# levi106/kvedge

Measured on AMD Instinct MI355X. Metric: images/sec ResNet-50 edge module at 1/2/4/8 MI355X; VM boot-to-ready sec, higher is better.
Workload: dtype bf16; 1 GPU; model=resnet50, global_batch=1280, per_gpu_batch=1280, image_size=224, parallelism=dp1, backend=none, hip_graph=True, streams=2, microbatch=0, mb_blocks=3

## Files before the change

### csrc/bindings/ops.cpp

```cpp
#include <ATen/ATen.h>
#include <c10/core/DeviceGuard.h>
#include <c10/hip/HIPStream.h>
#include <torch/library.h>

#include "../kernels/kvedge_kernels.h"

namespace {

hipStream_t cur_stream(const at::Tensor& t) {
  return c10::hip::getCurrentHIPStream(t.device().index()).stream();
}

void check_dev(const at::Tensor& t, const char* name) {
  TORCH_CHECK(t.is_cuda(), "kvedge: ", name, " must be a GPU tensor");
  TORCH_CHECK(t.is_contiguous(), "kvedge: ", name, " must be contiguous");
}

void check_bf16(const at::Tensor& t, const char* name) {
  check_dev(t, name);
  TORCH_CHECK(t.scalar_type() == at::kBFloat16, "kvedge: ", name, " must be bf16");
}

void set_splitk_ws(KvConvParams& p, const at::Tensor& ws) {
  p.ws = ws.data_ptr<float>();
  p.ws_elems = ws.numel();
}

void conv(const at::Tensor& x, const at::Tensor& w, const c10::optional<at::Tensor>& bias,
          const c10::optional<at::Tensor>& res, at::Tensor& y, int64_t N, int64_t H, int64_t W,
          int64_t Cin, int64_t ldx, int64_t x_coff, int64_t Ho, int64_t Wo, int64_t Cout,
          int64_t KH, int64_t KW, int64_t stride, int64_t pad, int64_t K, int64_t ldy,
          int64_t y_coff, int64_t ldr, int64_t r_coff, int64_t act, int64_t mode,
          int64_t tile, const c10::optional<at::Tensor>& ws) {
  check_bf16(x, "x");
  check_bf16(w, "w");
  check_bf16(y, "y");
  const c10::DeviceGuard g(x.device());
  KvConvParams p{};
  if (ws.has_value() && ws->defined()) {
    check_dev(*ws, "ws");
    TORCH_CHECK(ws->scalar_type() == at::kFloat, "kvedge: split-K workspace fp32");
    set_splitk_ws(p, *ws);
  }
  p.x = x.data_ptr();
  p.w = w.data_ptr();
  p.bias = nullptr;
  if (bias.has_value() && bias->defined()) {
    check_dev(*bias, "bias");
    TORCH_CHECK(bias->scalar_type() == at::kFloat && bias->numel() >= Cout, "kvedge: bias fp32[Cout]");
    p.bias = bias->data_ptr<float>();
  }
  p.res = nullptr;
  if (res.has_value() && res->defined()) {
    check_bf16(*res, "res");
    p.res = res->data_ptr();
  }
  p.y = y.data_ptr();
  p.N = (int)N; p.H = (int)H; p.W = (int)W; p.Cin = (int)Cin;
  p.ldx = (int)ldx; p.x_coff = (int)x_coff;
  p.Ho = (int)Ho; p.Wo = (int)Wo; p.Cout = (int)Cout;
  p.KH = (int)KH; p.KW = (int)KW; p.stride = (int)stride; p.pad = (int)pad;
  p.K = (int)K;
  TORCH_CHECK(w.dim() == 2 && w.size(0) == Cout, "kvedge: packed weight must be [Cout, Kpad]");
  p.Kpad = (int)w.size(1);
  p.M = (int)(N * Ho * Wo);
  p.ldy = (int)ldy; p.y_coff = (int)y_coff; p.ldr = (int)ldr; p.r_coff = (int)r_coff;
  p.act = (int)act; p.mode = (int)mode;
  TORCH_CHECK(N > 0 && H * W * ldx * 2 < (1ll << 31) && Ho * Wo * ldy * 2 < (1ll << 31),
              "kvedge: one image's activations exceed 2 GiB");
  TORCH_CHECK(x.numel() >= N * H * W * ldx, "kvedge: x smaller than N*H*W*ldx");
  TORCH_CHECK(x_coff >= 0 && x_coff + Cin <= ldx, "kvedge: x channel slice out of range");
  TORCH_CHECK(y.numel() >= (int64_t)p.M * ldy && y_coff + Cout <= ldy, "kvedge: y too small");
  if (p.res) TORCH_CHECK(res->numel() >= (int64_t)p.M * ldr && r_coff + Cout <= ldr, "kvedge: residual too small");
  const int rc = kv_conv2d(&p, (int)tile, cur_stream(x));
  TORCH_CHECK(rc == 0, "kvedge: kv_conv2d failed rc=", rc);
}

void conv_pair(const at::Tensor& x, const at::Tensor& w, const at::Tensor& bias,
               const at::Tensor& w2, const at::Tensor& b2, at::Tensor& z, int64_t Cin,
               int64_t x_coff, int64_t z_coff, int64_t act, int64_t tile) {
  check_bf16(x, "x");
  check_bf16(w, "w");
  check_bf16(w2, "w2");
  check_bf16(z, "z");
  check_dev(bias, "bias");
  check_dev(b2, "b2");
  TORCH_CHECK(x.dim() == 4 && z.dim() == 4 && w.dim() == 2 && w2.dim() == 2, "kvedge: conv_pair shapes");
  const int64_t N = x.size(0), H = x.size(1), W = x.size(2), ldx = x.size(3);
  const int64_t Cout = w.size(0), C2 = w2.size(0);
  TORCH_CHECK(w2.size(1) == Cout, "kvedge: conv_pair w2 must be [C2, Cout]");
  TORCH_CHECK(z.size(0) == N && z.size(1) == H && z.size(2) == W && z_coff + C2 <= z.size(3),
              "kvedge: conv_pair z [N, H, W, >= z_coff + C2]");
  TORCH_CHECK(x_coff + Cin <= ldx && w.size(1) == (9 * Cin + 63) / 64 * 64, "kvedge: conv_pair x / w");
  TORCH_CHECK(x_coff >= 0 && z_coff >= 0, "kvedge: conv_pair channel offsets must be >= 0");
  TORCH_CHECK(z_coff % 4 == 0 && z.size(3) % 4 == 0,
              "kvedge: conv_pair z_coff and the z row pitch must be multiples of 4 channels");
  TORCH_CHECK(bias.scalar_type() == at::kFloat && bias.numel() >= Cout && b2.scalar_type() == at::kFloat &&
              b2.numel() >= C2, "kvedge: conv_pair biases fp32");
  TORCH_CHECK(N * H * W * ldx * 2 < (1ll << 31) && N * H * W * z.size(3) * 2 < (1ll << 31),
              "kvedge: conv_pair operands exceed 2 GiB");
  const c10::DeviceGuard g(x.device());
  KvConvParams p{};
  p.x = x.data_ptr();
  p.w = w.data_ptr();
  p.bias = bias.data_ptr<float>();
  p.N = (int)N; p.H = (int)H; p.W = (int)W; p.Cin = (int)Cin;
  p.ldx = (int)ldx; p.x_coff = (int)x_coff;
  p.Ho = (int)H; p.Wo = (int)W; p.Cout = (int)Cout;
  p.KH = 3; p.KW = 3; p.stride = 1; p.pad = 1;
  p.K = (int)(9 * Cin); p.Kpad = (int)w.size(1);
  p.M = (int)(N * H * W);
  p.act = (int)act; p.mode = 0;
  p.w_t = w2.data_ptr(); p.bias_t = b2.data_ptr<float>(); p.z = z.data_ptr();
  p.n_t = (int)C2; p.ldz = (int)z.size(3); p.z_coff = (int)z_coff;
  p.pair_1x1 = 1;
  const int rc = kv_conv_pair(&p, (int)tile, cur_stream(x));
  TORCH_CHECK(rc == 0, "kvedge: conv_pair failed rc=", rc);
}

void conv_dual(const at::Tensor& x1, const at::Tensor& x2, const at::Tensor& w,
               const c10::optional<at::Tensor>& bias, at::Tensor& y, int64_t stride2,
               int64_t act, int64_t tile, const c10::optional<at::Tensor>& ws) {
  check_bf16(x1, "x1");
  check_bf16(x2, "x2");
  check_bf16(w, "w");
  check_bf16(y, "y");
  TORCH_CHECK(x1.dim() == 4 && x2.dim() == 4 && y.dim() == 4, "kvedge: NHWC tensors");
  const int64_t N = x1.size(0), Ho = x1.size(1), Wo = x1.size(2), K1 = x1.size(3);
  const int64_t K2 = x2.size(3), Cout = y.size(3);
  TORCH_CHECK(x2.size(0) == N && (x2.size(1) + stride2 - 1) / stride2 == Ho &&
                  (x2.size(2) + stride2 - 1) / stride2 == Wo, "kvedge: x2 geometry vs stride");
  TORCH_CHECK(y.size(0) == N && y.size(1) == Ho && y.size(2) == Wo, "kvedge: y shape");
  TORCH_CHECK(w.dim() == 2 && w.size(0) == Cout && w.size(1) == K1 + K2, "kvedge: w [Cout, K1+K2]");
  TORCH_CHECK(K1 % 64 == 0 && K2 % 64 == 0, "kvedge: K1, K2 multiples of 64");
  const c10::DeviceGuard g(x1.device());
  KvConvParams p{};
  p.x = x1.data_ptr();
  p.w = w.data_ptr();
  p.bias = nullptr;
  if (bias.has_value() && bias->defined()) {
    check_dev(*bias, "bias");
    TORCH_CHECK(bias->scalar_type() == at::kFloat && bias->numel() >= Cout, "kvedge: bias fp32[Cout]");
    p.bias = bias->data_ptr<float>();
  }
  p.res = nullptr;
  p.y = y.data_ptr();
  p.N = (int)N; p.H = (int)Ho; p.W = (int)Wo; p.Cin = (int)K1; p.ldx = (int)K1; p.x_coff = 0;
  p.Ho = (int)Ho; p.Wo = (int)Wo; p.Cout = (int)Cout;
  p.KH = 1; p.KW = 1; p.stride = 1; p.pad = 0;
  p.K = (int)(K1 + K2); p.Kpad = (int)(K1 + K2);
  p.M = (int)(N * Ho * Wo);
  p.ldy = (int)Cout; p.y_coff = 0; p.ldr = 0; p.r_coff = 0;
  p.act = (int)act; p.mode = 4;
  p.x2 = x2.data_ptr(); p.K1 = (int)K1; p.H2 = (int)x2.size(1); p.W2 = (int)x2.size(2);
  p.ldx2 = (int)K2; p.stride2 = (int)stride2;
  if (ws.has_value() && ws->defined()) {
    check_dev(*ws, "ws");
    TORCH_CHECK(ws->scalar_type() == at::kFloat, "kvedge: split-K workspace fp32");
    set_splitk_ws(p, *ws);
  }
  const int rc = kv_conv2d(&p, (int)tile, cur_stream(x1));
  TORCH_CHECK(rc == 0, "kvedge: conv_dual failed rc=", rc);
}

void conv_dual2(const at::Tensor& x, int64_t x_coff, int64_t K1, const at::Tensor& x2,
                int64_t x2_coff, const at::Tensor& w, const c10::optional<at::Tensor>& bias,
                at::Tensor& y, int64_t y_coff, int64_t stride2, int64_t up2, int64_t act,
                int64_t tile, const c10::optional<at::Tensor>& ws) {
  check_bf16(x, "x");
  check_bf16(x2, "x2");
  check_bf16(w, "w");
  check_bf16(y, "y");
  TORCH_CHECK(x.dim() == 4 && x2.dim() == 4 && y.dim() == 4 && w.dim() == 2, "kvedge: NHWC tensors");
  const int64_t N = x.size(0), Ho = x.size(1), Wo = x.size(2);
  const int64_t Cout = w.size(0), K2 = w.size(1) - K1;
  TORCH_CHECK(K1 > 0 && K2 > 0 && K1 % 64 == 0 && K2 % 64 == 0, "kvedge: K1, K2 multiples of 64");
  TORCH_CHECK(x_coff >= 0 && x_coff % 8 == 0 && x_coff + K1 <= x.size(3), "kvedge: x slice");
  TORCH_CHECK(x2_coff >= 0 && x2_coff % 8 == 0 && x2_coff + K2 <= x2.size(3), "kvedge: x2 slice");
  TORCH_CHECK(y_coff >= 0 && y_coff % 8 == 0 && y_coff + Cout <= y.size(3), "kvedge: y slice");
  TORCH_CHECK(x.size(3) % 8 == 0 && x2.size(3) % 8 == 0 && y.size(3) % 8 == 0, "kvedge: pitches");
  TORCH_CHECK(y.size(0) == N && y.size(1) == Ho && y.size(2) == Wo && x2.size(0) == N, "kvedge: y shape");
  if (up2) {
    TORCH_CHECK(x2.size(1) * 2 == Ho && x2.size(2) * 2 == Wo, "kvedge: up2 needs x2 at half size");
  } else {
    TORCH_CHECK(stride2 >= 1 && (x2.size(1) + stride2 - 1) / stride2 == Ho &&
                    (x2.size(2) + stride2 - 1) / stride2 == Wo,
                "kvedge: x2 geometry vs stride");
  }
  const c10::DeviceGuard g(x.device());
  KvConvParams p{};
  p.x = x.data_ptr();
  p.w = w.data_ptr();
  p.bias = nullptr;
  if (bias.has_value() && bias->defined()) {
    check_dev(*bias, "bias");
    TORCH_CHECK(bias->scalar_type() == at::kFloat && bias->numel() >= Cout, "kvedge: bias fp32[Cout]");
    p.bias = bias->data_ptr<float>();
  }
  p.y = y.data_ptr();
  p.N = (int)N; p.H = (int)Ho; p.W = (int)Wo; p.Cin = (int)K1; p.ldx = (int)x.size(3);
  p.x_coff = (int)x_coff;
  p.Ho = (int)Ho; p.Wo = (int)Wo; p.Cout = (int)Cout;
  p.KH = 1; p.KW = 1; p.stride = 1; p.pad = 0;
  p.K = (int)(K1 + K2); p.Kpad = (int)(K1 + K2);
  p.M = (int)(N * Ho * Wo);
  p.ldy = (int)y.size(3); p.y_coff = (int)y_coff; p.ldr = 0; p.r_coff = 0;
  p.act = (int)act; p.mode = 4;
  p.x2 = x2.data_ptr(); p.K1 = (int)K1; p.H2 = (int)x2.size(1); p.W2 = (int)x2.size(2);
  p.ldx2 = (int)x2.size(3); p.stride2 = (int)stride2; p.x2_coff = (int)x2_coff; p.up2 = (int)up2;
  if (ws.has_value() && ws->defined()) {
    check_dev(*ws, "ws");
    TORCH_CHECK(ws->scalar_type() == at::kFloat, "kvedge: split-K workspace fp32");
    set_splitk_ws(p, *ws);
  }
  const int rc = kv_conv2d(&p, (int)tile, cur_stream(x));
  TORCH_CHECK(rc == 0, "kvedge: conv_dual2 failed rc=", rc);
}

void conv_tail(const at::Tensor& x, const c10::optional<at::Tensor>& x2, const at::Tensor& w,
               const c10::optional<at::Tensor>& bias, const c10::optional<at::Tensor>& res,
               at::Tensor& y, const at::Tensor& w1, const c10::optional<at::Tensor>& b1,
               at::Tensor& z, int64_t stride2, int64_t act, int64_t tile) {
  check_bf16(x, "x");
  check_bf16(w, "w");
  check_bf16(y, "y");
  check_bf16(w1, "w1");
  check_bf16(z, "z");
  TORCH_CHECK(x.dim() == 4 && y.dim() == 4 && z.dim() == 4, "kvedge: NHWC tensors");
  const int64_t N = x.size(0), H = x.size(1), W = x.size(2), K1 = x.size(3);
  const int64_t Cout = y.size(3), Nt = w1.size(0);
  TORCH_CHECK(y.size(0) == N && y.size(1) == H && y.size(2) == W, "kvedge: y shape");
  TORCH_CHECK(z.size(0) == N && z.size(1) == H && z.size(2) == W && z.size(3) == Nt,
              "kvedge: z shape");
  TORCH_CHECK(w1.dim() == 2 && w1.size(1) == Cout, "kvedge: w1 must be [n_t, Cout]");
  TORCH_CHECK(K1 % 64 == 0, "kvedge: conv_tail K1 multiple of 64");
  const c10::DeviceGuard g(x.device());
  KvConvParams p{};
  p.x = x.data_ptr();
  p.w = w.data_ptr();
  p.bias = nullptr;
  if (bias.has_value() && bias->defined()) {
    check_dev(*bias, "bias");
    TORCH_CHECK(bias->scalar_type() == at::kFloat && bias->numel() >= Cout, "kvedge: bias fp32[Cout]");
    p.bias = bias->data_ptr<float>();
  }
  p.y = y.data_ptr();
  p.N = (int)N; p.H = (int)H; p.W = (int)W; p.Cin = (int)K1; p.ldx = (int)K1; p.x_coff = 0;
  p.Ho = (int)H; p.Wo = (int)W; p.Cout = (int)Cout;
  p.KH = 1; p.KW = 1; p.stride = 1; p.pad = 0;
  p.M = (int)(N * H * W);
  p.ldy = (int)Cout; p.y_coff = 0; p.r_coff = 0;
  p.act = (int)act;
  if (x2.has_value() && x2->defined()) {
    check_bf16(*x2, "x2");
    TORCH_CHECK(!(res.has_value() && res->defined()), "kvedge: conv_tail dual form takes no res");
    const int64_t K2 = x2->size(3);
    TORCH_CHECK(x2->dim() == 4 && x2->size(0) == N && (x2->size(1) + stride2 - 1) / stride2 == H &&
                    (x2->size(2) + stride2 - 1) / stride2 == W && K2 % 64 == 0,
                "kvedge: x2 geometry vs stride");
    TORCH_CHECK(w.dim() == 2 && w.size(0) == Cout && w.size(1) == K1 + K2, "kvedge: w [Cout, K1+K2]");
    p.mode = 4; p.K = (int)(K1 + K2); p.Kpad = (int)(K1 + K2);
    p.x2 = x2->data_ptr(); p.K1 = (int)K1; p.H2 = (int)x2->size(1); p.W2 = (int)x2->size(2);
    p.ldx2 = (int)K2; p.stride2 = (int)stride2;
    p.res = nullptr; p.ldr = 0;
  } else {
    TORCH_CHECK(res.has_value() && res->defined(), "kvedge: conv_tail plain form needs res");
    check_bf16(*res, "res");
    TORCH_CHECK(res->sizes() == y.sizes(), "kvedge: res shape");
    TORCH_CHECK(w.dim() == 2 && w.size(0) == Cout && w.size(1) == K1, "kvedge: w [Cout, K1]");
    p.mode = 1; p.K = (int)K1; p.Kpad = (int)K1;
    p.res = res->data_ptr(); p.ldr = (int)Cout;
  }
  p.w_t = w1.data_ptr();
  p.bias_t = nullptr;
  if (b1.has_value() && b1->defined()) {
    check_dev(*b1, "b1");
    TORCH_CHECK(b1->scalar_type() == at::kFloat && b1->numel() >= Nt, "kvedge: b1 fp32[n_t]");
    p.bias_t = b1->data_ptr<float>();
  }
  p.z = z.data_ptr(); p.n_t = (int)Nt; p.ldz = (int)Nt; p.z_coff = 0; p.act_t = 1;
  const int rc = kv_conv2d(&p, (int)tile, cur_stream(x));
  TORCH_CHECK(rc == 0, "kvedge: conv_tail failed rc=", rc);
}

void conv_frames_s2d(const at::Tensor& frames, const at::Tensor& w,
                     const c10::optional<at::Tensor>& bias, at::Tensor& y, int64_t act,
                     int64_t tile) {
  check_dev(frames, "frames");
  TORCH_CHECK(frames.scalar_type() == at::kByte && frames.dim() == 4 && frames.size(3) == 3 &&
                  frames.size(1) % 2 == 0 && frames.size(2) % 2 == 0,
              "kvedge: frames must be uint8 [N, H, W, 3] with even H, W");
  check_bf16(w, "w");
  check_bf16(y, "y");
  const int64_t N = frames.size(0), H = frames.size(1) / 2, W = frames.size(2) / 2;
  const int64_t Cout = w.size(0);
  TORCH_CHECK(w.dim() == 2 && w.size(1) == 64, "kvedge: s2d stem weight must be [Cout, 64]");
  TORCH_CHECK(y.dim() == 4 && y.size(0) == N && y.size(1) == H && y.size(2) == W &&
                  y.size(3) == Cout, "kvedge: y must be [N, H/2, W/2, Cout]");
  const c10::DeviceGuard g(frames.device());
  KvConvParams p{};
  p.x = frames.data_ptr();
  p.w = w.data_ptr();
  p.bias = nullptr;
  if (bias.has_value() && bias->defined()) {
    check_dev(*bias, "bias");
    TORCH_CHECK(bias->scalar_type() == at::kFloat && bias->numel() >= Cout, "kvedge: bias fp32[Cout]");
    p.bias = bias->data_ptr<float>();
  }
  p.res = nullptr;
  p.y = y.data_ptr();
  p.N = (int)N; p.H = (int)H; p.W = (int)W; p.Cin = 16; p.ldx = 16; p.x_coff = 0;
  p.Ho = (int)H; p.Wo = (int)W; p.Cout = (int)Cout;
  p.KH = 2; p.KW = 2; p.stride = 1; p.pad = 1; p.K = 64; p.Kpad = 64;
  p.M = (int)(N * H * W);
  p.ldy = (int)Cout; p.y_coff = 0; p.ldr = 0; p.r_coff = 0;
  p.act = (int)act; p.mode = 0; p.in_u8 = 1;
  const int rc = kv_conv2d(&p, (int)tile, cur_stream(frames));
  TORCH_CHECK(rc == 0, "kvedge: conv_frames_s2d failed rc=", rc);
}

void maxpool2d(const at::Tensor& x, at::Tensor& y, int64_t N, int64_t H, int64_t W, int64_t C,
               int64_t ldx, int64_t x_coff, int64_t ldy, int64_t y_coff, int64_t k, int64_t stride, int64_t pad,
               int64_t Ho, int64_t Wo) {
  check_bf16(x, "x");
  check_bf16(y, "y");
  TORCH_CHECK(x.numel() >= N * H * W * ldx && y.numel() >= N * Ho * Wo * ldy, "kvedge: maxpool sizes");
  const c10::DeviceGuard g(x.device());
  const int rc = kv_maxpool2d(x.data_ptr(), y.data_ptr(), (int)N, (int)H, (int)W, (int)C, (int)ldx,
                              (int)x_coff, (int)ldy, (int)y_coff, (int)k, (int)stride, (int)pad, (int)Ho,
                              (int)Wo, cur_stream(x));
  TORCH_CHECK(rc == 0, "kvedge: maxpool2d failed rc=", rc);
}

void stem_pool(const at::Tensor& x, const at::Tensor& w, const at::Tensor& bias, at::Tensor& y,
               int64_t y_coff) {
  check_bf16(x, "x");
  check_bf16(w, "w");
  check_bf16(y, "y");
  TORCH_CHECK(x.dim() == 4 && x.size(3) == 16, "kvedge: stem_pool x must be [N,H,W,16] (s2d)");
  TORCH_CHECK(w.numel() == 64 * 256, "kvedge: stem_pool w must be [64][256]");
  TORCH_CHECK(bias.is_cuda() && bias.scalar_type() == at::kFloat && bias.numel() == 64 &&
                  bias.is_contiguous(), "kvedge: stem_pool bias");
  const int64_t N = x.size(0), H = x.size(1), W = x.size(2);
  TORCH_CHECK(y.dim() == 4 && y.size(0) == N && y.size(1) == (H - 1) / 2 + 1 &&
                  y.size(2) == (W - 1) / 2 + 1 && y.size(3) >= y_coff + 64,
              "kvedge: stem_pool y shape");
  const c10::DeviceGuard g(x.device());
  const int rc = kv_stem_pool(x.data_ptr(), w.data_ptr(), bias.data_ptr<float>(), y.data_ptr(),
                              (int)N, (int)H, (int)W, (int)y.size(3), (int)y_coff, cur_stream(x));
  TORCH_CHECK(rc == 0, "kvedge: stem_pool failed rc=", rc);
}

void sppf_pool(at::Tensor& buf, int64_t N, int64_t H, int64_t W, int64_t C) {
  check_bf16(buf, "buf");
  TORCH_CHECK(buf.numel() == N * H * W * 4 * C, "kvedge: sppf buffer must be [N,H,W,4C]");
  const c10::DeviceGuard g(buf.device());
  const int rc = kv_sppf_pool(buf.data_ptr(), (int)N, (int)H, (int)W, (int)C, cur_stream(buf));
  TORCH_CHECK(rc == 0, "kvedge: sppf failed rc=", rc);
}

void global_avgpool(const at::Tensor& x, at::Tensor& y, int64_t N, int64_t HW, int64_t C) {
  check_bf16(x, "x");
  check_bf16(y, "y");
  TORCH_CHECK(x.numel() == N * HW * C && y.numel() == N * C, "kvedge: avgpool sizes");
  const c10::DeviceGuard g(x.device());
  const int rc = kv_global_avgpool(x.data_ptr(), y.data_ptr(), (int)N, (int)HW, (int)C, cur_stream(x));
  TORCH_CHECK(rc == 0, "kvedge: avgpool failed rc=", rc);
}

void pooled_fc(const at::Tensor& x, const at::Tensor& w, const c10::optional<at::Tensor>& bias,
               at::Tensor& y) {
  check_bf16(x, "x");
  check_bf16(w, "w");
  check_bf16(y, "y");
  TORCH_CHECK(x.dim() == 4 && w.dim() == 2 && y.dim() == 2, "kvedge: pooled_fc shapes");
  const int64_t N = x.size(0), HW = x.size(1) * x.size(2), C = x.size(3), ncls = w.size(0);
  TORCH_CHECK(w.size(1) >= C && y.size(0) == N && y.size(1) == ncls, "kvedge: pooled_fc w / y");
  const float* bp = nullptr;
  if (bias.has_value() && bias->defined()) {
    check_dev(*bias, "bias");
    TORCH_CHECK(bias->scalar_type() == at::kFloat && bias->numel() >= ncls, "kvedge: pooled_fc bias");
    bp = bias->data_ptr<float>();
  }
  const c10::DeviceGuard g(x.device());
  const int rc = kv_pooled_fc(x.data_ptr(), (int)N, (int)HW, (int)C, w.data_ptr(), (int)w.size(1),
                              bp, y.data_ptr(), (int)ncls, cur_stream(x));
  TORCH_CHECK(rc == 0, "kvedge: pooled_fc failed rc=", rc);
}

void softmax_rows(const at::Tensor& x, at::Tensor& y, at::Tensor& argmax) {
  check_bf16(x, "x");
  check_dev(y, "y");
  check_dev(argmax, "argmax");
  TORCH_CHECK(x.dim() == 2 && y.sizes() == x.sizes() && y.scalar_type() == at::kFloat, "kvedge: softmax y");
  TORCH_CHECK(argmax.scalar_type() == at::kLong && argmax.numel() == x.size(0), "kvedge: argmax");
  const c10::DeviceGuard g(x.device());
  const int rc = kv_softmax_rows(x.data_ptr(), y.data_ptr<float>(), argmax.data_ptr<int64_t>(),
                                 (int)x.size(0), (int)x.size(1), cur_stream(x));
  TORCH_CHECK(rc == 0, "kvedge: softmax failed rc=", rc);
}

void upsample2x(const at::Tensor& x, at::Tensor& y, int64_t N, int64_t H, int64_t W, int64_t C,
                int64_t ldx, int64_t x_coff, int64_t ldy, int64_t y_coff) {
  check_bf16(x, "x");
  check_bf16(y, "y");
  TORCH_CHECK(x.numel() >= N * H * W * ldx && y.numel() >= N * 4 * H * W * ldy, "kvedge: upsample sizes");
  const c10::DeviceGuard g(x.device());
  const int rc = kv_upsample2x(x.data_ptr(), y.data_ptr(), (int)N, (int)H, (int)W, (int)C, (int)ldx,
                               (int)x_coff, (int)ldy, (int)y_coff, cur_stream(x));
  TORCH_CHECK(rc == 0, "kvedge: upsample2x failed rc=", rc);
}

void yolo_decode(const at::Tensor& f0, const at::Tensor& f1, const at::Tensor& f2, int64_t h0,
                 int64_t w0, int64_t h1, int64_t w1, int64_t h2, int64_t w2, int64_t s0,
                 int64_t s1, int64_t s2, int64_t nc, at::Tensor& boxes, at::Tensor& scores,
                 at::Tensor& cls) {
  check_bf16(f0, "f0");
  check_bf16(f1, "f1");
  check_bf16(f2, "f2");
  const int64_t N = f0.size(0);
  const int64_t A = h0 * w0 + h1 * w1 + h2 * w2;
  const int64_t ch = 64 + nc;
  TORCH_CHECK(f0.numel() == N * h0 * w0 * ch && f1.numel() == N * h1 * w1 * ch &&
                  f2.numel() == N * h2 * w2 * ch, "kvedge: decode feature sizes");
  TORCH_CHECK(boxes.numel() == N * A * 4 && boxes.scalar_type() == at::kFloat, "kvedge: boxes");
  TORCH_CHECK(scores.numel() == N * A && scores.scalar_type() == at::kFloat, "kvedge: scores");
  TORCH_CHECK(cls.numel() == N * A && cls.scalar_type() == at::kInt, "kvedge: cls");
  const c10::DeviceGuard g(f0.device());
  const int rc = kv_yolo_decode(f0.data_ptr(), f1.data_ptr(), f2.data_ptr(), (int)h0, (int)w0,
                                (int)h1, (int)w1, (int)h2, (int)w2, (int)s0, (int)s1, (int)s2,
                                (int)N, (int)nc, boxes.data_ptr<float>(), scores.data_ptr<float>(),
                                cls.data_ptr<int>(), cur_stream(f0));
  TORCH_CHECK(rc == 0, "kvedge: yolo_decode failed rc=", rc);
}

void nms(const at::Tensor& boxes, const at::Tensor& scores, const at::Tensor& cls, double conf,
         double iou, int64_t max_det, at::Tensor& out, at::Tensor& count) {
  check_dev(boxes, "boxes");
  check_dev(scores, "scores");
  check_dev(cls, "cls");
  TORCH_CHECK(scores.dim() == 2, "kvedge: scores [N, A]");
  const int64_t N = scores.size(0), A = scores.size(1);
  TORCH_CHECK(boxes.numel() == N * A * 4 && cls.numel() == N * A, "kvedge: nms inputs");
  TORCH_CHECK(out.numel() == N * max_det * 6 && out.scalar_type() == at::kFloat, "kvedge: nms out");
  TORCH_CHECK(count.numel() == N && count.scalar_type() == at::kInt, "kvedge: nms count");
  const c10::DeviceGuard g(scores.device());
  const int rc = kv_nms(boxes.data_ptr<float>(), scores.data_ptr<float>(), cls.data_ptr<int>(),
                        (int)N, (int)A, (float)conf, (float)iou, (int)max_det,
                        out.data_ptr<float>(), count.data_ptr<int>(), cur_stream(scores));
  TORCH_CHECK(rc == 0, "kvedge: nms failed rc=", rc);
}

void synth_frames(at::Tensor& y, int64_t seed, int64_t step) {
  check_dev(y, "y");
  TORCH_CHECK(y.scalar_type() == at::kByte && y.dim() == 4 && y.size(3) == 3, "kvedge: frames u8 [N,H,W,3]");
  const c10::DeviceGuard g(y.device());
  const int rc = kv_synth_frames(y.data_ptr<uint8_t>(), (int)y.size(0), (int)y.size(1),
                                 (int)y.size(2), (uint64_t)seed, (uint64_t)step, cur_stream(y));
  TORCH_CHECK(rc == 0, "kvedge: synth_frames failed rc=", rc);
}

void synth_frames_dev(at::Tensor& y, at::Tensor& step, int64_t seed) {
  check_dev(y, "y");
  check_dev(step, "step");
  TORCH_CHECK(y.scalar_type() == at::kByte && y.dim() == 4 && y.size(3) == 3, "kvedge: frames u8 [N,H,W,3]");
  TORCH_CHECK(step.scalar_type() == at::kLong && (step.numel() == 1 || step.numel() == 2),
              "kvedge: step int64[1] or int64[2]");
  const c10::DeviceGuard g(y.device());
  const int rc = kv_synth_frames_dev(y.data_ptr<uint8_t>(), (int)y.size(0), (int)y.size(1),
                                     (int)y.size(2), (uint64_t)seed,
                                     reinterpret_cast<uint64_t*>(step.data_ptr<int64_t>()),
                                     step.numel() == 2 ? 1 : 0, cur_stream(y));
  TORCH_CHECK(rc == 0, "kvedge: synth_frames_dev failed rc=", rc);
}

void stem12_pool_frames(const at::Tensor& x, const at::Tensor& w, const at::Tensor& bias,
                        at::Tensor& y, at::ArrayRef<double> mean, at::ArrayRef<double> stdv,
                        int64_t y_coff) {
  check_dev(x, "x");
  check_bf16(w, "w");
  check_bf16(y, "y");
  TORCH_CHECK(x.scalar_type() == at::kByte && x.dim() == 4 && x.size(3) == 3 && x.is_contiguous(),
              "kvedge: stem12_pool_frames x must be contiguous u8 [N,H,W,3]");
  TORCH_CHECK(x.size(1) % 2 == 0 && x.size(2) % 4 == 0, "kvedge: stem12_pool_frames H even, W % 4");
  TORCH_CHECK(w.numel() == 64 * 192 && w.is_contiguous(), "kvedge: stem12 w must be [64][192]");
  TORCH_CHECK(bias.is_cuda() && bias.scalar_type() == at::kFloat && bias.numel() == 64 &&
                  bias.is_contiguous(), "kvedge: stem12 bias");
  TORCH_CHECK(mean.size() == 3 && stdv.size() == 3, "kvedge: mean/std of 3");
  const int64_t N = x.size(0), H = x.size(1) / 2, W = x.size(2) / 2;
  TORCH_CHECK(y.dim() == 4 && y.size(0) == N && y.size(1) == (H - 1) / 2 + 1 &&
                  y.size(2) == (W - 1) / 2 + 1 && y.size(3) >= y_coff + 64 && y.is_contiguous(),
              "kvedge: stem12_pool_frames y shape");
  float m[3], is[3];
  for (int i = 0; i < 3; ++i) {
    m[i] = (float)mean[i];
    is[i] = (float)(1.0 / stdv[i]);
  }
  const c10::DeviceGuard g(x.device());
  const int rc = kv_stem12_pool_frames(x.data_ptr(), w.data_ptr(), bias.data_ptr<float>(),
                                       y.data_ptr(), (int)N, (int)x.size(1), (int)x.size(2), m, is,
                                       (int)y.size(3), (int)y_coff, cur_stream(x));
  TORCH_CHECK(rc == 0, "kvedge: stem12_pool_frames failed rc=", rc);
}

void yolo_stem2(const at::Tensor& x, const at::Tensor& w0, const at::Tensor& b0,
                const at::Tensor& w1, const at::Tensor& b1, at::Tensor& y) {
  check_dev(x, "x");
  check_bf16(w0, "w0");
  check_bf16(w1, "w1");
  check_bf16(y, "y");
  TORCH_CHECK(x.scalar_type() == at::kByte && x.dim() == 4 && x.size(3) == 3 && x.is_contiguous(),
              "kvedge: yolo_stem2 x must be contiguous u8 [N,H,W,3]");
  TORCH_CHECK(x.size(1) % 4 == 0 && x.size(2) % 32 == 0 && x.size(2) <= 640,
              "kvedge: yolo_stem2 needs H % 4 == 0, W % 32 == 0, W <= 640");
  TORCH_CHECK(w0.dim() == 2 && w0.size(0) == 16 && w0.size(1) == 64 && w0.is_contiguous(),
              "kvedge: yolo_stem2 w0 must be [16][64]");
  TORCH_CHECK(w1.dim() == 2 && w1.size(0) == 32 && w1.size(1) >= 144 && w1.size(1) % 8 == 0 &&
                  w1.is_contiguous(), "kvedge: yolo_stem2 w1 must be [32][>= 144]");
  for (const at::Tensor* b : {&b0, &b1}) {
    check_dev(*b, "bias");
    TORCH_CHECK(b->scalar_type() == at::kFloat && b->is_contiguous(), "kvedge: fp32 biases");
  }
  TORCH_CHECK(b0.numel() >= 16 && b1.numel() >= 32, "kvedge: bias sizes");
  const int64_t N = x.size(0), H0 = x.size(1), W0 = x.size(2);
  TORCH_CHECK(y.dim() == 4 && y.size(0) == N && y.size(1) == H0 / 4 && y.size(2) == W0 / 4 &&
                  y.size(3) == 32 && y.is_contiguous(), "kvedge: yolo_stem2 y must be [N,H/4,W/4,32]");
  const c10::DeviceGuard g(x.device());
  const int rc = kv_yolo_stem2(x.data_ptr(), w0.data_ptr(), b0.data_ptr<float>(), w1.data_ptr(),
                               (int)w1.size(1), b1.data_ptr<float>(), y.data_ptr(), (int)N,
                               (int)H0, (int)W0, cur_stream(x));
  TORCH_CHECK(rc == 0, "kvedge: yolo_stem2 failed rc=", rc);
}

void stem_pool_frames(const at::Tensor& x, const at::Tensor& w, const at::Tensor& bias,
                      at::Tensor& y, at::ArrayRef<double> mean, at::ArrayRef<double> stdv,
                      int64_t y_coff) {
  check_dev(x, "x");
  check_bf16(w, "w");
  check_bf16(y, "y");
  TORCH_CHECK(x.scalar_type() == at::kByte && x.dim() == 4 && x.size(3) == 3 && x.is_contiguous(),
              "kvedge: stem_pool_frames x must be contiguous u8 [N,H,W,3]");
  TORCH_CHECK(x.size(1) % 2 == 0 && x.size(2) % 4 == 0, "kvedge: stem_pool_frames H even, W % 4");
  TORCH_CHECK(w.numel() == 64 * 256, "kvedge: stem_pool w must be [64][256]");
  TORCH_CHECK(bias.is_cuda() && bias.scalar_type() == at::kFloat && bias.numel() == 64 &&
                  bias.is_contiguous(), "kvedge: stem_pool bias");
  TORCH_CHECK(mean.size() == 3 && stdv.size() == 3, "kvedge: mean/std of 3");
  const int64_t N = x.size(0), H = x.size(1) / 2, W = x.size(2) / 2;
  TORCH_CHECK(y.dim() == 4 && y.size(0) == N && y.size(1) == (H - 1) / 2 + 1 &&
                  y.size(2) == (W - 1) / 2 + 1 && y.size(3) >= y_coff + 64,
              "kvedge: stem_pool_frames y shape");
  float m[3], is[3];
  for (int i = 0; i < 3; ++i) {
    m[i] = (float)mean[i];
    is[i] = (float)(1.0 / stdv[i]);
  }
  const c10::DeviceGuard g(x.device());
  const int rc = kv_stem_pool_frames(x.data_ptr(), w.data_ptr(), bias.data_ptr<float>(),
                                     y.data_ptr(), (int)N, (int)x.size(1), (int)x.size(2), m, is,
                                     (int)y.size(3), (int)y_coff, cur_stream(x));
  TORCH_CHECK(rc == 0, "kvedge: stem_pool_frames failed rc=", rc);
}

void preprocess(const at::Tensor& x, at::Tensor& y, at::ArrayRef<double> mean,
                at::ArrayRef<double> stdv) {
  check_dev(x, "x");
  check_bf16(y, "y");
  TORCH_CHECK(x.scalar_type() == at::kByte && x.dim() == 4 && x.size(3) == 3, "kvedge: x u8 [N,H,W,3]");
  TORCH_CHECK(y.dim() == 4 && y.size(0) == x.size(0), "kvedge: y batch");
  const bool s2d = y.size(3) == 16;
  if (s2d) {
    TORCH_CHECK(y.size(1) * 2 == x.size(1) && y.size(2) * 2 == x.size(2), "kvedge: y bf16 [N,H/2,W/2,16]");
  } else {
    TORCH_CHECK(y.size(1) == x.size(1) && y.size(2) == x.size(2) && y.size(3) == 4,
                "kvedge: y bf16 [N,H,W,4] or [N,H/2,W/2,16]");
  }
  TORCH_CHECK(mean.size() == 3 && stdv.size() == 3, "kvedge: mean/std of 3");
  float m[3], is[3];
  for (int i = 0; i < 3; ++i) {
    m[i] = (float)mean[i];
    is[i] = (float)(1.0 / stdv[i]);
  }
  const c10::DeviceGuard g(x.device());
  const int rc = s2d ? kv_preprocess_s2d(x.data_ptr<uint8_t>(), y.data_ptr(), (int)x.size(0),
                                         (int)x.size(1), (int)x.size(2), m, is, cur_stream(x))
                     : kv_preprocess(x.data_ptr<uint8_t>(), y.data_ptr(), (int)x.size(0),
                                     (int)x.size(1), (int)x.size(2), m, is, cur_stream(x));
  TORCH_CHECK(rc == 0, "kvedge: preprocess failed rc=", rc);
}

void frame_resize(const at::Tensor& src, at::Tensor& dst, at::IntArrayRef axis_y,
                  at::IntArrayRef axis_x, int64_t pad) {
  check_dev(src, "src");
  check_dev(dst, "dst");
  TORCH_CHECK(src.scalar_type() == at::kByte && src.dim() == 4 && src.size(3) == 3,
              "kvedge: src u8 [N,Hs,Ws,3]");
  TORCH_CHECK(dst.scalar_type() == at::kByte && dst.dim() == 4 && dst.size(3) == 3 &&
                  dst.size(0) == src.size(0), "kvedge: dst u8 [N,Hd,Wd,3]");
  TORCH_CHECK(axis_y.size() == 5 && axis_x.size() == 5, "kvedge: axis_y / axis_x of 5 ints");
  TORCH_CHECK(src.size(1) <= 8192 && src.size(2) <= 8192 && dst.size(1) <= 8192 &&
                  dst.size(2) <= 8192, "kvedge: frame_resize extents are 1..8192");
  TORCH_CHECK(src.device() == dst.device(), "kvedge: src / dst on different devices");
  int ay[5], ax[5];
  for (int i = 0; i < 5; ++i) {
    TORCH_CHECK(axis_y[i] >= 0 && axis_y[i] <= 8192 && axis_x[i] >= 0 && axis_x[i] <= 8192,
                "kvedge: frame_resize axis values are 0..8192");
    ay[i] = (int)axis_y[i];
    ax[i] = (int)axis_x[i];
  }
  const c10::DeviceGuard g(src.device());
  const int rc = kv_frame_resize(src.data_ptr<uint8_t>(), dst.data_ptr<uint8_t>(), (int)src.size(0),
                                 (int)src.size(1), (int)src.size(2), (int)dst.size(1),
                                 (int)dst.size(2), ay, ax, (int)pad, cur_stream(src));
  TORCH_CHECK(rc == 0, "kvedge: frame_resize failed rc=", rc);
}

void det_to_source(at::Tensor& det, const at::Tensor& count, at::ArrayRef<double> map, int64_t Hs,
                   int64_t Ws) {
  check_dev(det, "det");
  check_dev(count, "count");
  TORCH_CHECK(det.scalar_type() == at::kFloat && det.dim() == 3 && det.size(2) == 6,
              "kvedge: det fp32 [N,max_det,6]");
  TORCH_CHECK(count.scalar_type() == at::kInt && count.numel() == det.size(0),
              "kvedge: count int32 [N]");
  TORCH_CHECK(map.size() == 4, "kvedge: map = {cy, sy, cx, sx}");
  TORCH_CHECK(Hs >= 1 && Ws >= 1 && Hs <= 8192 && Ws <= 8192, "kvedge: source size 1..8192");
  TORCH_CHECK(det.device() == count.device(), "kvedge: det / count on different devices");
  const c10::DeviceGuard g(det.device());
  const int rc = kv_det_to_source(det.data_ptr<float>(), count.data_ptr<int>(), (int)det.size(0),
                                  (int)det.size(1), (float)map[0], (float)map[1], (float)map[2],
                                  (float)map[3], (int)Hs, (int)Ws, cur_stream(det));
  TORCH_CHECK(rc == 0, "kvedge: det_to_source failed rc=", rc);
}

void roi_crop_band(const at::Tensor& src, const at::Tensor& det, const at::Tensor& count,
                   at::Tensor& dst, int64_t pad, int64_t band) {
  check_dev(src, "src");
  check_dev(det, "det");
  check_dev(count, "count");
  check_dev(dst, "dst");
  TORCH_CHECK(src.scalar_type() == at::kByte && src.dim() == 4 && src.size(3) == 3,
              "kvedge: src u8 [N,Hs,Ws,3]");
  TORCH_CHECK(det.scalar_type() == at::kFloat && det.dim() == 3 && det.size(2) == 6 &&
                  det.size(0) == src.size(0), "kvedge: det fp32 [N,max_det,6]");
  TORCH_CHECK(count.scalar_type() == at::kInt && count.dim() == 1 &&
                  count.size(0) == src.size(0), "kvedge: count int32 [N]");
  TORCH_CHECK(dst.scalar_type() == at::kByte && dst.dim() == 4 && dst.size(3) == 3 &&
                  dst.size(1) == dst.size(2), "kvedge: dst u8 [N*K,D,D,3]");
  const int64_t N = src.size(0);
  TORCH_CHECK(N ? dst.size(0) >= N && dst.size(0) % N == 0 : dst.size(0) == 0,
              "kvedge: dst holds N*K crops, K >= 1");
  const int64_t K = N ? dst.size(0) / N : 1;
  TORCH_CHECK(K <= det.size(1), "kvedge: roi_crop K ", K, " > max_det ", det.size(1));
  TORCH_CHECK(src.size(1) <= 8192 && src.size(2) <= 8192 && dst.size(1) <= 8192,
              "kvedge: roi_crop extents are 1..8192");
  TORCH_CHECK(N * det.size(1) < (1ll << 31) && dst.size(0) < (1ll << 31),
              "kvedge: roi_crop batch too large");
  TORCH_CHECK(src.device() == det.device() && src.device() == count.device() &&
                  src.device() == dst.device(), "kvedge: roi_crop operands on different devices");
  TORCH_CHECK(band >= 0 && band <= 32, "kvedge: roi_crop band is 0, 4, 8, 16 or 32");
  const c10::DeviceGuard g(src.device());
  const int rc = kv_roi_crop_band(src.data_ptr<uint8_t>(), det.data_ptr<float>(),
                                  count.data_ptr<int>(), dst.data_ptr<uint8_t>(), (int)N,
                                  (int)src.size(1), (int)src.size(2), (int)det.size(1), (int)K,
                                  (int)dst.size(1), (int)pad, (int)band, cur_stream(src));
  TORCH_CHECK(rc == 0, "kvedge: roi_crop failed rc=", rc);
}

void roi_crop(const at::Tensor& src, const at::Tensor& det, const at::Tensor& count,
              at::Tensor& dst, int64_t pad) {
  roi_crop_band(src, det, count, dst, pad, 0);
}

void batchnorm_nhwc(const at::Tensor& x, at::Tensor& y, const at::Tensor& scale,
                    const at::Tensor& shift, bool relu) {
  check_bf16(x, "x");
  check_bf16(y, "y");
  check_dev(scale, "scale");
  check_dev(shift, "shift");
  const int64_t C = x.size(-1);
  TORCH_CHECK(scale.numel() == C && shift.numel() == C && scale.scalar_type() == at::kFloat &&
                  shift.scalar_type() == at::kFloat, "kvedge: bn scale/shift fp32[C]");
  TORCH_CHECK(y.sizes() == x.sizes(), "kvedge: bn y shape");
  const c10::DeviceGuard g(x.device());
  const int rc = kv_batchnorm_nhwc(x.data_ptr(), y.data_ptr(), scale.data_ptr<float>(),
                                   shift.data_ptr<float>(), x.numel() / C, (int)C, relu ? 1 : 0,
                                   cur_stream(x));
  TORCH_CHECK(rc == 0, "kvedge: batchnorm failed rc=", rc);
}

int64_t conv_num_tiles() { return kv_conv_num_tiles(); }
int64_t conv_splitk_base() { return kv_conv_splitk_base(); }
int64_t conv_splitk_num_tiles() { return kv_conv_splitk_num_tiles(); }
int64_t nloop_sched_check() { return kv_nloop_sched_check(); }
int64_t conv_seam_num_tiles() { return kv_conv_seam_num_tiles(); }
int64_t set_conv_chunk_bytes(int64_t b) { return kv_set_conv_chunk_bytes(b); }

void c2f16_fused(const at::Tensor& x, int64_t x_coff, const at::Tensor& w1, const at::Tensor& b1,
                 const at::Tensor& wm1, const at::Tensor& bm1, const at::Tensor& wm2,
                 const at::Tensor& bm2, const at::Tensor& w2, const at::Tensor& b2, at::Tensor& y,
                 int64_t y_coff, int64_t S) {
  check_bf16(x, "x");
  check_bf16(y, "y");
  for (const at::Tensor* w : {&w1, &wm1, &wm2, &w2}) check_bf16(*w, "w");
  for (const at::Tensor* b : {&b1, &bm1, &bm2, &b2}) {
    check_dev(*b, "bias");
    TORCH_CHECK(b->scalar_type() == at::kFloat && b->is_contiguous(), "kvedge: c2f16 biases fp32");
  }
  TORCH_CHECK(x.dim() == 4 && y.dim() == 4 && x.size(0) == y.size(0) && x.size(1) == y.size(1) &&
                  x.size(2) == y.size(2), "kvedge: c2f16 x / y [N, H, W, C]");
  const int64_t N = x.size(0), H = x.size(1), W = x.size(2);
  TORCH_CHECK(x_coff >= 0 && x_coff + 32 <= x.size(3) && y_coff >= 0 && y_coff + 32 <= y.size(3),
              "kvedge: c2f16 channel slices");
  TORCH_CHECK(w1.dim() == 2 && w1.size(0) == 32 && w1.size(1) >= 32 && wm1.dim() == 2 &&
                  wm1.size(0) == 16 && wm1.size(1) >= 144 && wm2.sizes() == wm1.sizes() &&
                  w2.dim() == 2 && w2.size(0) == 32 && w2.size(1) >= 48,
              "kvedge: c2f16 weights w1 [32, >=32], wm [16, >=144], w2 [32, >=48]");
  TORCH_CHECK(b1.numel() == 32 && bm1.numel() == 16 && bm2.numel() == 16 && b2.numel() == 32,
              "kvedge: c2f16 bias sizes");
  TORCH_CHECK(kv_c2f16_supported((int)H, (int)W, (int)S), "kvedge: c2f16 has no form for H=", H,
              " W=", W, " S=", S);
  TORCH_CHECK(x.numel() * 2 < (1ll << 31) - (1 << 20) && y.numel() * 2 < (1ll << 31) - (1 << 20),
              "kvedge: c2f16 operands exceed 2 GiB");
  TORCH_CHECK(x.data_ptr() != y.data_ptr(), "kvedge: c2f16 cannot run in place");
  const c10::DeviceGuard g(x.device());
  KvC2fParams p{};
  p.x = x.data_ptr();
  p.y = y.data_ptr();
  p.w1 = w1.data_ptr();
  p.b1 = b1.data_ptr<float>();
  p.wm1 = wm1.data_ptr();
  p.bm1 = bm1.data_ptr<float>();
  p.wm2 = wm2.data_ptr();
  p.bm2 = bm2.data_ptr<float>();
  p.w2 = w2.data_ptr();
  p.b2 = b2.data_ptr<float>();
  p.N = (int)N; p.H = (int)H; p.W = (int)W;
  p.ldx = (int)x.size(3); p.x_coff = (int)x_coff;
  p.ldy = (int)y.size(3); p.y_coff = (int)y_coff;
  p.ldw1 = (int)w1.size(1); p.ldwm = (int)wm1.size(1); p.ldw2 = (int)w2.size(1);
  p.S = (int)S;
  const int rc = kv_c2f16_fused(&p, cur_stream(x));
  TORCH_CHECK(rc == 0, "kvedge: c2f16_fused failed rc=", rc);
}

int64_t c2f16_supported(int64_t H, int64_t W, int64_t S) {
  return kv_c2f16_supported((int)H, (int)W, (int)S);
}

}

TORCH_LIBRARY(kvedge, m) {
  m.def("conv(Tensor x, Tensor w, Tensor? bias, Tensor? res, Tensor(a!) y, int N, int H, int W, "
        "int Cin, int ldx, int x_coff, int Ho, int Wo, int Cout, int KH, int KW, int stride, "
        "int pad, int K, int ldy, int y_coff, int ldr, int r_coff, int act, int mode, int tile, "
        "Tensor(b!)? ws=None) -> ()");
  m.def("conv_pair(Tensor x, Tensor w, Tensor bias, Tensor w2, Tensor b2, Tensor(a!) z, int Cin, "
        "int x_coff, int z_coff, int act, int tile) -> ()");
  m.def("conv_dual(Tensor x1, Tensor x2, Tensor w, Tensor? bias, Tensor(a!) y, int stride2, int act, "
        "int tile, Tensor(b!)? ws=None) -> ()");
  m.def("conv_tail(Tensor x, Tensor? x2, Tensor w, Tensor? bias, Tensor? res, Tensor(a!) y, "
        "Tensor w1, Tensor? b1, Tensor(b!) z, int stride2, int act, int tile) -> ()");
  m.def("conv_frames_s2d(Tensor frames, Tensor w, Tensor? bias, Tensor(a!) y, int act, "
        "int tile) -> ()");
  m.def("stem_pool(Tensor x, Tensor w, Tensor bias, Tensor(a!) y, int y_coff) -> ()");
  m.def("maxpool2d(Tensor x, Tensor(a!) y, int N, int H, int W, int C, int ldx, int x_coff, int ldy, "
        "int y_coff, int k, int stride, int pad, int Ho, int Wo) -> ()");
  m.def("sppf_pool(Tensor(a!) buf, int N, int H, int W, int C) -> ()");
  m.def("global_avgpool(Tensor x, Tensor(a!) y, int N, int HW, int C) -> ()");
  m.def("softmax_rows(Tensor x, Tensor(a!) y, Tensor(b!) argmax) -> ()");
  m.def("pooled_fc(Tensor x, Tensor w, Tensor? bias, Tensor(a!) y) -> ()");
  m.def("upsample2x(Tensor x, Tensor(a!) y, int N, int H, int W, int C, int ldx, int x_coff, int ldy, "
        "int y_coff) -> ()");
  m.def("yolo_decode(Tensor f0, Tensor f1, Tensor f2, int h0, int w0, int h1, int w1, int h2, "
        "int w2, int s0, int s1, int s2, int nc, Tensor(a!) boxes, Tensor(b!) scores, "
        "Tensor(c!) cls) -> ()");
  m.def("nms(Tensor boxes, Tensor scores, Tensor cls, float conf, float iou, int max_det, "
        "Tensor(a!) out, Tensor(b!) count) -> ()");
  m.def("synth_frames(Tensor(a!) y, int seed, int step) -> ()");
  m.def("synth_frames_dev(Tensor(a!) y, Tensor(b!) step, int seed) -> ()");
  m.def("stem_pool_frames(Tensor x, Tensor w, Tensor bias, Tensor(a!) y, float[] mean, float[] std, int y_coff) -> ()");
  m.def("stem12_pool_frames(Tensor x, Tensor w, Tensor bias, Tensor(a!) y, float[] mean, float[] std, int y_coff) -> ()");
  m.def("yolo_stem2(Tensor x, Tensor w0, Tensor b0, Tensor w1, Tensor b1, Tensor(a!) y) -> ()");
  m.def("preprocess(Tensor x, Tensor(a!) y, float[] mean, float[] std) -> ()");
  m.def("frame_resize(Tensor src, Tensor(a!) dst, int[] axis_y, int[] axis_x, int pad) -> ()");
  m.def("det_to_source(Tensor(a!) det, Tensor count, float[] map, int Hs, int Ws) -> ()");
  m.def("roi_crop(Tensor src, Tensor det, Tensor count, Tensor(a!) dst, int pad) -> ()");
  m.def("roi_crop_band(Tensor src, Tensor det, Tensor count, Tensor(a!) dst, int pad, int band) -> ()");
  m.def("batchnorm_nhwc(Tensor x, Tensor(a!) y, Tensor scale, Tensor shift, bool relu) -> ()");
  m.def("conv_num_tiles() -> int", conv_num_tiles);
  m.def("conv_splitk_base() -> int", conv_splitk_base);
  m.def("conv_splitk_num_tiles() -> int", conv_splitk_num_tiles);
  m.def("nloop_sched_check() -> int", nloop_sched_check);
  m.def("conv_seam_num_tiles() -> int", conv_seam_num_tiles);
  m.def("c2f16_fused(Tensor x, int x_coff, Tensor w1, Tensor b1, Tensor wm1, Tensor bm1, "
        "Tensor wm2, Tensor bm2, Tensor w2, Tensor b2, Tensor(a!) y, int y_coff, int S) -> ()");
  m.def("c2f16_supported(int H, int W, int S) -> int", c2f16_supported);
  m.def("conv_dual2(Tensor x, int x_coff, int K1, Tensor x2, int x2_coff, Tensor w, Tensor? bias, "
        "Tensor(a!) y, int y_coff, int stride2, int up2, int act, int tile, Tensor(b!)? ws=None) -> ()");
  m.def("set_conv_chunk_bytes(int bytes) -> int", set_conv_chunk_bytes);
}

TORCH_LIBRARY_IMPL(kvedge, CUDA, m) {
  m.impl("conv", conv);
  m.impl("conv_dual", conv_dual);
  m.impl("maxpool2d", maxpool2d);
  m.impl("stem_pool", stem_pool);
  m.impl("conv_frames_s2d", conv_frames_s2d);
  m.impl("conv_tail", conv_tail);
  m.impl("conv_pair", conv_pair);
  m.impl("c2f16_fused", c2f16_fused);
  m.impl("conv_dual2", conv_dual2);
  m.impl("sppf_pool", sppf_pool);
  m.impl("global_avgpool", global_avgpool);
  m.impl("softmax_rows", softmax_rows);
  m.impl("pooled_fc", pooled_fc);
  m.impl("upsample2x", upsample2x);
  m.impl("yolo_decode", yolo_decode);
  m.impl("nms", nms);
  m.impl("synth_frames", synth_frames);
  m.impl("synth_frames_dev", synth_frames_dev);
  m.impl("preprocess", preprocess);
  m.impl("stem_pool_frames", stem_pool_frames);
  m.impl("stem12_pool_frames", stem12_pool_frames);
  m.impl("yolo_stem2", yolo_stem2);
  m.impl("frame_resize", frame_resize);
  m.impl("det_to_source", det_to_source);
  m.impl("roi_crop", roi_crop);
  m.impl("roi_crop_band", roi_crop_band);
  m.impl("batchnorm_nhwc", batchnorm_nhwc);
}
```

### csrc/kernels/conv_igemm.hip

```cpp
#include <algorithm>

#include "common.h"
#include "kvedge_kernels.h"

namespace kvedge {
namespace {

constexpr int BK = 64;

struct TileCfg {
  int bm, bn, wm, wn;
};

template <int BM, int BN, int WM, int WN, int MODE>
__global__ __launch_bounds__(256, 2) void conv_igemm_kernel(const KvConvParams p) {
  constexpr int WTM = BM / WM, WTN = BN / WN;
  constexpr int TM = WTM / 16, TN = WTN / 16;
  constexpr int AR = BM / 32;
  constexpr int BR = BN / 32;
  static_assert(WM * WN == 4, "4 waves per workgroup");
  static_assert(TM >= 1 && TN >= 1, "wave tile >= 16x16");

  __shared__ __attribute__((aligned(16))) bf16 smem[2 * (BM + BN) * BK];

  const int tid = threadIdx.x;
  const int lane = tid & 63;
  const int wv = tid >> 6;
  const int wm = wv / WN, wn = wv % WN;

  const int nbm = (p.M + BM - 1) / BM;
  const int nbn = (p.Cout + BN - 1) / BN;
  const int t = xcd_remap(blockIdx.x, nbm * nbn);
  const int m0 = (t / nbn) * BM;
  const int n0 = (t % nbn) * BN;
  static_assert(BN <= 256, "one bias value per thread");
  const float bias_r = (tid < BN && p.bias && n0 + tid < p.Cout) ? p.bias[n0 + tid] : 0.f;

  const bf16* __restrict__ X = reinterpret_cast<const bf16*>(p.x);
  const bf16* __restrict__ Wt = reinterpret_cast<const bf16*>(p.w);

  const int cc = tid & 7;
  const int rr = tid >> 3;

  int a_base[AR], a_h0[AR], a_w0[AR];
  const int HoWo = p.Ho * p.Wo;
#pragma unroll
  for (int i = 0; i < AR; ++i) {
    const int m = m0 + rr + 32 * i;
    if (m < p.M) {
      if (MODE == 1) {
        a_base[i] = m * p.ldx + p.x_coff;
        a_h0[i] = 0;
        a_w0[i] = 0;
      } else {
        const int img = m / HoWo;
        const int rem = m - img * HoWo;
        const int ho = rem / p.Wo;
        const int wo = rem - ho * p.Wo;
        a_base[i] = img * p.H * p.W * p.ldx + p.x_coff;
        a_h0[i] = ho * p.stride - p.pad;
        a_w0[i] = wo * p.stride - p.pad;
      }
    } else {
      a_base[i] = 0;
      a_h0[i] = -(1 << 28);
      a_w0[i] = -(1 << 28);
    }
  }

  int kr = 0, ksx = 0, kc = cc * 8;
  if (MODE == 0) {
    while (kc >= p.Cin) {
      kc -= p.Cin;
      if (++ksx == p.KW) { ksx = 0; ++kr; }
    }
  }
  const int kwp = (p.KW + 1) & ~1;
  const int kpr = kwp * 4;

  uint4 ra[AR], rb[BR];

  auto load_a = [&](int kt) {
#pragma unroll
    for (int i = 0; i < AR; ++i) {
      uint4 v = make_uint4(0, 0, 0, 0);
      if (MODE == 1) {
        const int k = kt * BK + cc * 8;
        if (a_h0[i] >= 0 && k < p.Cin)
          v = *reinterpret_cast<const uint4*>(X + a_base[i] + k);
      } else if (MODE == 0) {
        const int hi = a_h0[i] + kr, wi = a_w0[i] + ksx;
        if (kr < p.KH && (unsigned)hi < (unsigned)p.H && (unsigned)wi < (unsigned)p.W)
          v = *reinterpret_cast<const uint4*>(X + a_base[i] + (hi * p.W + wi) * p.ldx + kc);
      } else {
        const int k = kt * BK + cc * 8;
        const int r = k / kpr;
        const int s = ((k - r * kpr) >> 3) * 2;
        const int hi = a_h0[i] + r, wi = a_w0[i] + s;
        if (r < p.KH && (unsigned)hi < (unsigned)p.H) {
          const bf16* rowp = X + a_base[i] + hi * p.W * 4;
          uint2 lo = make_uint2(0, 0), hi2 = make_uint2(0, 0);
          if ((unsigned)wi < (unsigned)p.W) lo = *reinterpret_cast<const uint2*>(rowp + wi * 4);
          if ((unsigned)(wi + 1) < (unsigned)p.W)
            hi2 = *reinterpret_cast<const uint2*>(rowp + (wi + 1) * 4);
          v = make_uint4(lo.x, lo.y, hi2.x, hi2.y);
        }
      }
      ra[i] = v;
    }
  };
  auto advance_k = [&]() {
    if (MODE == 0) {
      kc += BK;
      while (kc >= p.Cin) {
        kc -= p.Cin;
        if (++ksx == p.KW) { ksx = 0; ++kr; }
      }
    }
  };
  auto load_b = [&](int kt) {
#pragma unroll
    for (int i = 0; i < BR; ++i) {
      const int n = n0 + rr + 32 * i;
      uint4 v = make_uint4(0, 0, 0, 0);
      if (n < p.Cout)
        v = *reinterpret_cast<const uint4*>(Wt + (size_t)n * p.Kpad + kt * BK + cc * 8);
      rb[i] = v;
    }
  };
  auto store_tiles = [&](int buf) {
    bf16* As = smem + buf * (BM + BN) * BK;
    bf16* Bs = As + BM * BK;
#pragma unroll
    for (int i = 0; i < AR; ++i) {
      const int row = rr + 32 * i;
      *reinterpret_cast<uint4*>(As + row * BK + ((cc ^ (row & 7)) << 3)) = ra[i];
    }
#pragma unroll
    for (int i = 0; i < BR; ++i) {
      const int row = rr + 32 * i;
      *reinterpret_cast<uint4*>(Bs + row * BK + ((cc ^ (row & 7)) << 3)) = rb[i];
    }
  };

  floatx4 acc[TN][TM];
#pragma unroll
  for (int a = 0; a < TN; ++a)
#pragma unroll
    for (int b = 0; b < TM; ++b) acc[a][b] = floatx4{0.f, 0.f, 0.f, 0.f};

  auto compute = [&](int buf) {
    const bf16* As = smem + buf * (BM + BN) * BK;
    const bf16* Bs = As + BM * BK;
    const int fr = lane & 15;
    const int sw = lane & 7;
#pragma unroll
    for (int ks = 0; ks < 2; ++ks) {
      const int q = ks * 4 + (lane >> 4);
      bf16x8 af[TM], bfg[TN];
#pragma unroll
      for (int tm = 0; tm < TM; ++tm) {
        const int row = wm * WTM + tm * 16 + fr;
        af[tm] = *reinterpret_cast<const bf16x8*>(As + row * BK + ((q ^ sw) << 3));
      }
#pragma unroll
      for (int tn = 0; tn < TN; ++tn) {
        const int row = wn * WTN + tn * 16 + fr;
        bfg[tn] = *reinterpret_cast<const bf16x8*>(Bs + row * BK + ((q ^ sw) << 3));
      }
#pragma unroll
      for (int tn = 0; tn < TN; ++tn)
#pragma unroll
        for (int tm = 0; tm < TM; ++tm)
          acc[tn][tm] = __builtin_amdgcn_mfma_f32_16x16x32_bf16(bfg[tn], af[tm], acc[tn][tm], 0, 0, 0);
    }
  };

  const int nk = p.Kpad / BK;
  load_a(0);
  load_b(0);
  store_tiles(0);
  __syncthreads();
  for (int kt = 0; kt < nk; ++kt) {
    const int cur = kt & 1;
    const bool more = kt + 1 < nk;
    if (more) {
      advance_k();
      load_a(kt + 1);
      load_b(kt + 1);
    }
    compute(cur);
    if (more) store_tiles(cur ^ 1);
    __syncthreads();
  }

  constexpr int CS = BN + 8;
  static_assert(BM * CS * 2 + BN * 4 <= 2 * (BM + BN) * BK * 2, "C tile + bias slot must fit");
  const bool has_res = p.res != nullptr;
  float* const lbias = reinterpret_cast<float*>(smem + 2 * (BM + BN) * BK) - BN;
  if (tid < BN) lbias[tid] = bias_r;
  __syncthreads();
  typedef unsigned int u32x4v __attribute__((ext_vector_type(4)));
  const __amdgpu_buffer_rsrc_t ry = __builtin_amdgcn_make_buffer_rsrc(p.y, (short)0, p.M * p.ldy * 2, 0x00020000);
  const __amdgpu_buffer_rsrc_t rres = __builtin_amdgcn_make_buffer_rsrc(
      const_cast<void*>(p.res), (short)0, has_res ? p.M * p.ldr * 2 : 0, 0x00020000);
  constexpr int kOOB1 = 0x7ffffff0;
  constexpr int CPR = BN / 8;
  constexpr int PER = BM * CPR / 256;
  dispatch_act(p.act, has_res, [&](auto A1, auto A2) __attribute__((always_inline)) {
    constexpr int act1 = decltype(A1)::value, act2 = decltype(A2)::value;
#pragma unroll
    for (int tn = 0; tn < TN; ++tn) {
      const int nl = wn * WTN + tn * 16 + (lane >> 4) * 4;
      const float4 bv = *reinterpret_cast<const float4*>(lbias + nl);
#pragma unroll
      for (int tm = 0; tm < TM; ++tm) {
        const int ml = wm * WTM + tm * 16 + (lane & 15);
        bf16x4 o;
        o[0] = f2bf(act_c<act1>(acc[tn][tm][0] + bv.x));
        o[1] = f2bf(act_c<act1>(acc[tn][tm][1] + bv.y));
        o[2] = f2bf(act_c<act1>(acc[tn][tm][2] + bv.z));
        o[3] = f2bf(act_c<act1>(acc[tn][tm][3] + bv.w));
        *reinterpret_cast<bf16x4*>(smem + ml * CS + nl) = o;
      }
    }
    u32x4v rv[PER];
    if (has_res) {
#pragma unroll
      for (int j = 0; j < PER; ++j) {
        const int idx = tid + 256 * j;
        const int m = m0 + idx / CPR, n = n0 + (idx % CPR) * 8;
        const int off = (m < p.M && n < p.Cout) ? (m * p.ldr + p.r_coff + n) * 2 : kOOB1;
        rv[j] = __builtin_amdgcn_raw_buffer_load_b128(rres, off, 0, 0);
      }
    }
    __syncthreads();
#pragma unroll
    for (int j = 0; j < PER; ++j) {
      const int idx = tid + 256 * j;
      const int ml = idx / CPR, ch = idx % CPR;
      const int m = m0 + ml, n = n0 + ch * 8;
      bf16x8 v = *reinterpret_cast<const bf16x8*>(smem + ml * CS + ch * 8);
      if (has_res) {
        const bf16x8 r8 = __builtin_bit_cast(bf16x8, rv[j]);
#pragma unroll
        for (int e = 0; e < 8; ++e) v[e] = f2bf(act_c<act2>((float)v[e] + (float)r8[e]));
      }
      const int off = (m < p.M && n < p.Cout) ? (m * p.ldy + p.y_coff + n) * 2 : kOOB1;
      __builtin_amdgcn_raw_buffer_store_b128(__builtin_bit_cast(u32x4v, v), ry, off, 0, 0);
    }
  });
}

typedef void (*ConvKernelFn)(const KvConvParams);

template <int BM, int BN, int WM, int WN>
struct TileInst {
  static ConvKernelFn get(int mode) {
    switch (mode) {
      case 0: return conv_igemm_kernel<BM, BN, WM, WN, 0>;
      case 1: return conv_igemm_kernel<BM, BN, WM, WN, 1>;
      default: return conv_igemm_kernel<BM, BN, WM, WN, 2>;
    }
  }
};

struct TileEntry {
  TileCfg cfg;
  ConvKernelFn (*get)(int);
};

const TileEntry kTiles[] = {
    {{128, 128, 2, 2}, &TileInst<128, 128, 2, 2>::get},
    {{128, 64, 2, 2}, &TileInst<128, 64, 2, 2>::get},
    {{64, 64, 2, 2}, &TileInst<64, 64, 2, 2>::get},
    {{256, 64, 4, 1}, &TileInst<256, 64, 4, 1>::get},
    {{64, 128, 2, 2}, &TileInst<64, 128, 2, 2>::get},
    {{256, 128, 2, 2}, &TileInst<256, 128, 2, 2>::get},
};
constexpr int kNumTiles = sizeof(kTiles) / sizeof(kTiles[0]);

}
}

using namespace kvedge;

namespace kvedge {
int glds_num_tiles();
int glds_launch(const KvConvParams* p, int tile, hipStream_t stream);
int glds_tile_bm(int tile);
int glds_tile_bn(int tile);
int stream_num_tiles();
int stream_launch(const KvConvParams* p, int tile, hipStream_t stream);
int stream_tail_tile(int n_t);
int direct_num_tiles();
int direct_launch(const KvConvParams* p, int tile, hipStream_t stream);
int nloop_num_tiles();
int nloop_launch(const KvConvParams* p, int tile, hipStream_t stream);
int nloop_sched_check();
int xp_num_tiles();
int xp_launch(const KvConvParams* p, int tile, hipStream_t stream);
int sk_num_tiles();
int sk_launch(const KvConvParams* p, int tile, hipStream_t stream);
int direct_de_num_tiles();
int direct_de_launch(const KvConvParams* p, int tile, hipStream_t stream);
int skinny_num_tiles();
int skinny_launch(const KvConvParams* p, int tile, hipStream_t stream);
int pp_num_tiles();
int pp_launch(const KvConvParams* p, int tile, hipStream_t stream);
int seam_num_tiles();
int seam_pick_tile(const KvConvParams* p);
int seam_launch(const KvConvParams* p, int tile, hipStream_t stream);
}

extern "C" int kv_conv_seam_num_tiles(void) { return kvedge::seam_num_tiles(); }

extern "C" int kv_nloop_sched_check(void) { return kvedge::nloop_sched_check(); }

extern "C" int kv_conv_num_tiles(void) {
  return kNumTiles + glds_num_tiles() + stream_num_tiles() + direct_num_tiles() +
         nloop_num_tiles() + xp_num_tiles() + sk_num_tiles() + direct_de_num_tiles() +
         skinny_num_tiles() + pp_num_tiles();
}

extern "C" int kv_conv_splitk_base(void) {
  return kNumTiles + glds_num_tiles() + stream_num_tiles() + direct_num_tiles() +
         nloop_num_tiles() + xp_num_tiles();
}
extern "C" int kv_conv_splitk_num_tiles(void) { return sk_num_tiles(); }

extern "C" int kv_conv_pick_tile(const KvConvParams* p) {
  const long long M = p->M, N = p->Cout;
  auto nwg = [&](int bm, int bn) { return ((M + bm - 1) / bm) * ((N + bn - 1) / bn); };
  if (N <= 64) {
    if (nwg(256, 64) >= 1024) return 3;
    if (nwg(128, 64) >= 512) return 1;
    return 2;
  }
  if (nwg(256, 128) >= 2048) return 5;
  if (nwg(128, 128) >= 512) return 0;
  if (nwg(64, 128) >= 256) return 4;
  return 2;
}

#ifdef KVEDGE_CHECKS
static bool kv_in_alloc(const void* ptr, long long bytes) {
  if (!ptr || bytes <= 0) return true;
  hipDeviceptr_t base = nullptr;
  size_t size = 0;
  if (hipMemGetAddressRange(&base, &size, (hipDeviceptr_t)ptr) != hipSuccess) {
    (void)hipGetLastError();
    return false;
  }
  const char* b = static_cast<const char*>(base);
  const char* q = static_cast<const char*>(ptr);
  return q >= b && q + bytes <= b + size;
}

static int kv_conv_check_extents(const KvConvParams* p) {
  const long long M = (long long)p->N * p->Ho * p->Wo;
  if (!kv_in_alloc(p->x, p->in_u8 ? (long long)p->N * p->H * p->W * 12
                                    : (long long)p->N * p->H * p->W * p->ldx * 2)) return -20;
  if (!kv_in_alloc(p->w, (long long)p->Cout * p->Kpad * 2)) return -21;
  if (!kv_in_alloc(p->bias, (long long)p->Cout * 4)) return -22;
  if (!kv_in_alloc(p->y, M * p->ldy * 2)) return -23;
  if (p->res && !kv_in_alloc(p->res, M * p->ldr * 2)) return -24;
  if (p->n_t && (!kv_in_alloc(p->z, M * p->ldz * 2) ||
                 !kv_in_alloc(p->w_t, (long long)p->n_t * p->Cout * 2) ||
                 !kv_in_alloc(p->bias_t, (long long)p->n_t * 4)))
    return -28;
  if (p->mode == 4 && !kv_in_alloc(p->x2, (long long)p->N * p->H2 * p->W2 * p->ldx2 * 2)) return -25;
  if (p->x_coff + p->Cin > p->ldx || p->y_coff + p->Cout > p->ldy) return -26;
  if (p->res && p->r_coff + p->Cout > p->ldr) return -27;
  return 0;
}
#endif

static int kv_conv2d_one(const KvConvParams* p, int tile, hipStream_t stream);

static long long kv_conv_max_image_bytes(const KvConvParams* p) {
  const long long hw = (long long)p->H * p->W, ohw = (long long)p->Ho * p->Wo;
  long long m = p->in_u8 ? hw * 12 : hw * p->ldx * 2;
  m = std::max(m, ohw * p->ldy * 2);
  if (p->res) m = std::max(m, ohw * p->ldr * 2);
  if (p->mode == 4) m = std::max(m, (long long)p->H2 * p->W2 * p->ldx2 * 2);
  if (p->n_t) m = std::max(m, ohw * p->ldz * 2);
  return m;
}

static long long g_chunk_bytes = 0x7f000000LL;

extern "C" long long kv_set_conv_chunk_bytes(long long bytes) {
  g_chunk_bytes = bytes > 0 ? std::min(bytes, 0x7f000000LL) : 0x7f000000LL;
  return g_chunk_bytes;
}

extern "C" int kv_conv2d(const KvConvParams* p, int tile, hipStream_t stream) {
#ifdef KVEDGE_CHECKS
  if (const int rc = kv_conv_check_extents(p)) return rc;
#endif
  const long long kChunkBytes = g_chunk_bytes;
  const long long per = kv_conv_max_image_bytes(p);
  if (per <= 0 || per >= kChunkBytes) return per <= 0 ? -1 : -9;
  const long long cap = kChunkBytes / per;
  if (p->N <= cap) return kv_conv2d_one(p, tile, stream);
  const long long hw = (long long)p->H * p->W, ohw = (long long)p->Ho * p->Wo;
  for (int n0 = 0; n0 < p->N; n0 += (int)cap) {
    KvConvParams q = *p;
    q.N = (int)std::min<long long>(cap, p->N - n0);
    q.M = (int)(q.N * ohw);
    auto adv = [&](const void* b, long long bytes_per_image) -> const char* {
      return b ? static_cast<const char*>(b) + (long long)n0 * bytes_per_image : nullptr;
    };
    q.x = adv(p->x, p->in_u8 ? hw * 12 : hw * p->ldx * 2);
    q.y = const_cast<char*>(adv(p->y, ohw * p->ldy * 2));
    if (p->res) q.res = adv(p->res, ohw * p->ldr * 2);
    if (p->mode == 4) q.x2 = adv(p->x2, (long long)p->H2 * p->W2 * p->ldx2 * 2);
    if (p->n_t) q.z = const_cast<char*>(adv(p->z, ohw * p->ldz * 2));
    if (const int rc = kv_conv2d_one(&q, tile, stream)) return rc;
  }
  return 0;
}

static int kv_conv2d_one(const KvConvParams* p, int tile, hipStream_t stream) {
  if (p->Kpad % BK != 0 || p->Cout % 8 != 0) return -1;
  if (p->n_t) {
    const int v3 = kNumTiles + glds_num_tiles();
    const int v9 = kv_conv_num_tiles();
    if (tile < 0) {
      if (p->Cout == 256) {
        tile = v3 + stream_tail_tile(p->n_t);
      } else {
        const int s = seam_pick_tile(p);
        if (s < 0) return -8;
        tile = v9 + s;
      }
    }
    if (tile >= v9) return seam_launch(p, tile - v9, stream);
    if (tile < v3 || tile >= v3 + stream_num_tiles()) return -8;
    return stream_launch(p, tile - v3, stream);
  }
  if (p->in_u8) {
    const int v4 = kNumTiles + glds_num_tiles() + stream_num_tiles();
    if (tile >= 0 && tile < v4) return -8;
    return direct_launch(p, tile < 0 ? 0 : tile - v4, stream);
  }
  if (p->mode == 2 && (p->Cin != 4 || p->ldx != 4)) return -2;
  if (p->mode != 2 && (p->Cin % 8 != 0 || p->ldx % 8 != 0 || p->x_coff % 8 != 0)) return -3;
  if (p->mode == 1 && (p->KH != 1 || p->KW != 1 || p->stride != 1 || p->pad != 0)) return -4;
  if ((p->ldy % 8) || (p->y_coff % 8) || (p->res && ((p->ldr % 8) || (p->r_coff % 8)))) return -5;
  if (p->mode == 4) {
    if (tile < 0) {
      const long long nwg128 = ((p->M + 127) / 128) * ((p->Cout + 127) / 128);
      tile = kNumTiles + (nwg128 >= 512 ? 0 : 4);
    }
    if (tile < kNumTiles) return -8;
  }
  if (tile < 0) tile = kv_conv_pick_tile(p);
  const int v3 = kNumTiles + glds_num_tiles();
  const int v4 = v3 + stream_num_tiles();
  const int v6 = v4 + direct_num_tiles();
  const int v7 = v6 + nloop_num_tiles();
  const int v8 = v7 + xp_num_tiles();
  const int v10 = v8 + sk_num_tiles();
  const int v12 = v10 + direct_de_num_tiles();
  const int v14 = v12 + skinny_num_tiles();
  if (tile >= v14 + pp_num_tiles()) return -6;
  if (tile >= v14) return pp_launch(p, tile - v14, stream);
  if (tile >= v12) return skinny_launch(p, tile - v12, stream);
  if (tile >= v10) return direct_de_launch(p, tile - v10, stream);
  if (tile >= v8) return sk_launch(p, tile - v8, stream);
  if (tile >= v7) return xp_launch(p, tile - v7, stream);
  if (tile >= v6) return nloop_launch(p, tile - v6, stream);
  if (tile >= v4) return direct_launch(p, tile - v4, stream);
  if (tile >= v3) return stream_launch(p, tile - v3, stream);
  if (tile >= kNumTiles) return glds_launch(p, tile - kNumTiles, stream);
  const TileEntry& e = kTiles[tile];
  const long long nwg = (long long)((p->M + e.cfg.bm - 1) / e.cfg.bm) *
                        ((p->Cout + e.cfg.bn - 1) / e.cfg.bn);
  if (nwg <= 0) return 0;
  ConvKernelFn fn = e.get(p->mode);
  hipLaunchKernelGGL(fn, dim3((unsigned)nwg), dim3(256), 0, stream, *p);
  return hipGetLastError() == hipSuccess ? 0 : -7;
}
```

### csrc/kernels/conv_seam.hip

```cpp
#include "common.h"
#include "kvedge_kernels.h"

namespace kvedge {
namespace {

constexpr int kSmOOB = 0x7ffffff0;
constexpr int kSmLdsMax = 160 * 1024;

template <int I>
struct SmIC {
  static constexpr int value = I;
};
template <int N, int I = 0, class F>
__device__ __forceinline__ void sm_static_for(F&& f) {
  if constexpr (I < N) {
    f(SmIC<I>{});
    sm_static_for<N, I + 1>(f);
  }
}

template <int N>
__device__ __forceinline__ void sm_wait_vm() {
  static_assert(N >= 0 && N <= 63, "vmcnt field");
  asm volatile("s_waitcnt vmcnt(%0)" ::"n"(N) : "memory");
}

template <int SY, int SZ, int D, int RD, int KB, int NA>
struct SmSched {
  static constexpr int SPT = SY + SZ;
  static constexpr int kB = KB, kR = 2, kS = 2, kA = NA;
  static constexpr int kFar = 12;
  static constexpr int kTiles = kFar + 2;
  static constexpr int wait(int kind, int idx) {
    long endB[kTiles * SPT + D + 2] = {};
    long endR[kTiles + RD + 2] = {};
    long pos = kA;
    for (int t = 0; t < RD - 1; ++t) endR[t] = (pos += kR);
    for (int s = 0; s < D - 1; ++s) endB[s] = (pos += kB);
    for (int t = 0; t < kTiles; ++t) {
      for (int j = 0; j < SPT; ++j) {
        const int s = t * SPT + j;
        if (j == SY) {
          if (kind == 1 && idx == t) return (int)(pos - endR[t]);
          pos += kS;
        }
        if (kind == 0 && idx == s) return (int)(pos - endB[s]);
        if (kind == 2 && idx == s) return D >= 3 ? (int)(pos - endB[s + 1]) : -1;
        endB[s + D - 1] = (pos += kB);
        if (j == 0) endR[t + RD - 1] = (pos += kR);
      }
    }
    return -1;
  }
  static constexpr int wB(int t, int j) { return wait(0, t * SPT + j); }
  static constexpr int wE(int t) { return wait(1, t); }
  static constexpr int wXB(int t, int j) { return wait(2, t * SPT + j); }
  static constexpr int steady_from() {
    int t0 = 0;
    for (int t = 0; t < kFar; ++t) {
      bool same = wE(t) == wE(kFar);
      for (int j = 0; j < SPT; ++j)
        same = same && wB(t, j) == wB(kFar, j) && wXB(t, j) == wXB(kFar, j);
      if (!same) t0 = t + 1;
    }
    return t0;
  }
  static constexpr int kSteady = steady_from();
  static constexpr int safe_B(int j) {
    int m = wB(kFar, j);
    for (int t = 0; t <= kSteady; ++t) m = wB(t, j) < m ? wB(t, j) : m;
    return m;
  }
  static constexpr int safe_XB(int j) {
    int m = wXB(kFar, j);
    for (int t = 0; t <= kSteady; ++t) m = wXB(t, j) < m ? wXB(t, j) : m;
    return m;
  }
  static constexpr int safe_E() {
    int m = wE(kFar);
    for (int t = 0; t <= kSteady; ++t) m = wE(t) < m ? wE(t) : m;
    return m;
  }
  static constexpr bool ok(bool xp = false) {
    for (int t = 0; t <= kFar; ++t) {
      if (wE(t) < 0 || wE(t) > 63) return false;
      for (int j = 0; j < SPT; ++j) {
        if (wB(t, j) < 0 || wB(t, j) > 63) return false;
        if (xp && (wXB(t, j) < 0 || wXB(t, j) > 63)) return false;
      }
    }
    return kSteady < kFar;
  }
};

__device__ __forceinline__ int sm_sw(int r) { return (r >> 1) & 7; }

__device__ __forceinline__ void sm_lds_barrier() {
  asm volatile("s_waitcnt lgkmcnt(0)" ::: "memory");
  __builtin_amdgcn_s_barrier();
  asm volatile("" ::: "memory");
}

template <int NC3, int NZC, int D, int RD, int NW = 8, int KS2 = 1, bool AREG = false,
          bool XP = false>
__global__ __launch_bounds__(64 * NW, NW == 4 ? 2 : 1) void conv_seam_kernel(const KvConvParams p, int ntiles) {
  static_assert(NW == 4 || NW == 8, "waves");
  static_assert(NC3 % KS2 == 0 && NZC % KS2 == 0, "whole chunks per ring stage");
  constexpr int SY = NC3 / KS2, SZ = NZC / KS2, BPW = 8 / NW;
  using S = SmSched<SY, SZ, D, RD, KS2 * BPW, AREG ? 0 : 2 * NC3>;
  static_assert(S::ok(XP), "counted-wait schedule out of range or not periodic");
  constexpr int SPT = S::SPT, BM = 16 * NW, NT = 64 * NW;
  static_assert(!XP || (AREG && D >= 3 && SPT % 2 == 0),
                "XP: A in VGPRs, stage s + 1 issued before step s, register sets by step parity");
  constexpr int A_BYTES = AREG ? 0 : NC3 * BM * 128, B_CHUNK = 64 * 128, B_STAGE = KS2 * B_CHUNK;
  constexpr int R_SLOT = BM * 64 * 2;
  constexpr int B_OFF = A_BYTES, R_OFF = B_OFF + D * B_STAGE, BIAS_OFF = R_OFF + RD * R_SLOT;
  constexpr int BIAS_ROUND = NW * 1024;
  extern __shared__ __attribute__((aligned(16))) char sm_smem[];
  char* const lds = sm_smem;

  const int tid = threadIdx.x, lane = tid & 63;
  const int wv = __builtin_amdgcn_readfirstlane(tid >> 6);
  const int wm = wv >> 1, wn = wv & 1;
  const int nbm = (p.M + BM - 1) / BM;
  const int m0 = xcd_remap(blockIdx.x, nbm) * BM;
  const int Cout = p.Cout, N1 = p.n_t;
  const int b1_off = BIAS_OFF + ((Cout * 4 + BIAS_ROUND - 1) / BIAS_ROUND) * BIAS_ROUND;

  const kv_i32x4 rx = kv_rsrc4(p.x, p.M * p.ldx * 2);
  const kv_i32x4 rw3 = kv_rsrc4(p.w, Cout * p.Kpad * 2);
  const kv_i32x4 rw1 = kv_rsrc4(p.w_t, N1 * Cout * 2);
  const kv_i32x4 rr = kv_rsrc4(p.res, p.M * p.ldr * 2);
  const kv_i32x4 rb3 = kv_rsrc4(p.bias, Cout * 4);
  const kv_i32x4 rb1 = kv_rsrc4(p.bias_t, N1 * 4);
  const __amdgpu_buffer_rsrc_t ry =
      __builtin_amdgcn_make_buffer_rsrc(p.y, (short)0, p.M * p.ldy * 2, 0x00020000);
  const __amdgpu_buffer_rsrc_t rz =
      __builtin_amdgcn_make_buffer_rsrc(p.z, (short)0, p.M * p.ldz * 2, 0x00020000);

  const int lrow = lane >> 3, pch = lane & 7;
  int arow_off[2], r_src[2], lc8[2];
#pragma unroll
  for (int i = 0; i < 2; ++i) {
    const int row = (wv * 2 + i) * 8 + lrow;
    const int lc = pch ^ sm_sw(row);
    lc8[i] = lc * 8;
    const int m = m0 + row;
    arow_off[i] = m < p.M ? (m * p.ldx + p.x_coff + lc * 8) * 2 : kSmOOB;
    r_src[i] = m < p.M ? (m * p.ldr + p.r_coff + lc * 8) * 2 : kSmOOB;
  }
  int w3_src[BPW], w1_src[BPW], brow[BPW];
#pragma unroll
  for (int i = 0; i < BPW; ++i) {
    brow[i] = (wv * BPW + i) * 8 + lrow;
    const int bch = (pch ^ sm_sw(brow[i])) * 8;
    w3_src[i] = (brow[i] * p.Kpad + bch) * 2;
    w1_src[i] = (brow[i] * Cout + bch) * 2;
  }

  auto issue_B = [&](int tt, auto JJ) __attribute__((always_inline)) {
    constexpr int jj = decltype(JJ)::value;
    const int s = tt * SPT + jj;
    char* dst = lds + B_OFF + (s % D) * B_STAGE;
#pragma unroll
    for (int c = 0; c < KS2; ++c)
#pragma unroll
      for (int i = 0; i < BPW; ++i) {
        char* d = dst + c * B_CHUNK + (wv * BPW + i) * 1024;
        if constexpr (jj < SY) {
          const int n = tt * 64 + brow[i];
          const int v = (tt < ntiles && n < Cout) ? w3_src[i] + (tt * 64 * p.Kpad + (jj * KS2 + c) * 64) * 2 : kSmOOB;
          kv_lds_dma16(rw3, d, v);
        } else {
          const int zc = (jj - SY) * KS2 + c;
          const int zr = zc * 64 + brow[i];
          const int v = (tt < ntiles && zr < N1) ? w1_src[i] + (zc * 64 * Cout + tt * 64) * 2 : kSmOOB;
          kv_lds_dma16(rw1, d, v);
        }
      }
  };
  auto issue_R = [&](int tt) __attribute__((always_inline)) {
    char* dst = lds + R_OFF + (tt % RD) * R_SLOT;
#pragma unroll
    for (int i = 0; i < 2; ++i) {
      const int n = tt * 64 + lc8[i];
      const int v = (tt < ntiles && n < Cout && r_src[i] != kSmOOB) ? r_src[i] + tt * 128 : kSmOOB;
      kv_lds_dma16_nt(rr, dst + (wv * 2 + i) * 1024, v);
    }
  };

  for (int i = 0; i < (Cout * 4 + BIAS_ROUND - 1) / BIAS_ROUND; ++i) {
    const int off = (i * NW + wv) * 1024;
    kv_lds_dma16(rb3, lds + BIAS_OFF + off, off + lane * 16);
  }
  for (int i = 0; i < (N1 * 4 + BIAS_ROUND - 1) / BIAS_ROUND; ++i) {
    const int off = (i * NW + wv) * 1024;
    kv_lds_dma16(rb1, lds + b1_off + off, off + lane * 16);
  }
  typedef unsigned int sm_u32x4 __attribute__((ext_vector_type(4)));
  sm_u32x4 araw[AREG ? NC3 : 1][2][2];
  const int fr = lane & 15, fh = lane >> 4;
  if constexpr (AREG) {
#pragma unroll
    for (int kc = 0; kc < NC3; ++kc)
#pragma unroll
      for (int ks = 0; ks < 2; ++ks)
#pragma unroll
        for (int tm = 0; tm < 2; ++tm) {
          const int m = m0 + wm * 32 + tm * 16 + fr;
          const int k = kc * 64 + ks * 32 + fh * 8;
          const int off = (m < p.M && k < p.Cin) ? (m * p.ldx + p.x_coff + k) * 2 : kSmOOB;
          asm volatile("buffer_load_dwordx4 %0, %1, %2, 0 offen"
                       : "=v"(araw[kc][ks][tm]) : "v"(off), "s"(rx) : "memory");
        }
  }
  if constexpr (!AREG) {
#pragma unroll
    for (int kc = 0; kc < NC3; ++kc)
#pragma unroll
      for (int i = 0; i < 2; ++i) {
        char* dst = lds + kc * (BM * 128) + (wv * 2 + i) * 1024;
        const int v = (arow_off[i] != kSmOOB && kc * 64 + lc8[i] < p.Cin) ? arow_off[i] + kc * 128 : kSmOOB;
        kv_lds_dma16_nt(rx, dst, v);
      }
  }
#pragma unroll
  for (int t = 0; t < RD - 1; ++t) issue_R(t);
  sm_static_for<D - 1>([&](auto JJ) __attribute__((always_inline)) {
    constexpr int s = decltype(JJ)::value;
    issue_B(s / SPT, SmIC<s % SPT>{});
  });
  bf16x8 areg[AREG ? NC3 : 1][2][2];
  if constexpr (AREG) {
    sm_wait_vm<(RD - 1) * S::kR + (D - 1) * S::kB>();
#pragma unroll
    for (int kc = 0; kc < NC3; ++kc)
#pragma unroll
      for (int ks = 0; ks < 2; ++ks)
#pragma unroll
        for (int tm = 0; tm < 2; ++tm) {
          asm volatile("" : "+v"(araw[kc][ks][tm]));
          areg[kc][ks][tm] = __builtin_bit_cast(bf16x8, araw[kc][ks][tm]);
        }
  }

  floatx4 acc[2][2];
  floatx4 accz[NZC][2][2];
#pragma unroll
  for (int zc = 0; zc < NZC; ++zc)
#pragma unroll
    for (int a = 0; a < 2; ++a)
#pragma unroll
      for (int b = 0; b < 2; ++b) accz[zc][a][b] = floatx4{0.f, 0.f, 0.f, 0.f};

  auto mma64 = [&](const char* As, const char* Bs, floatx4 (&c)[2][2]) __attribute__((always_inline)) {
#pragma unroll
    for (int ks = 0; ks < 2; ++ks) {
      const int q = ks * 4 + fh;
      bf16x8 af[2], bfg[2];
#pragma unroll
      for (int tm = 0; tm < 2; ++tm) {
        const int row = wm * 32 + tm * 16 + fr;
        af[tm] = *reinterpret_cast<const bf16x8*>(As + row * 128 + ((q ^ sm_sw(row)) << 4));
      }
#pragma unroll
      for (int tn = 0; tn < 2; ++tn) {
        const int row = wn * 32 + tn * 16 + fr;
        bfg[tn] = *reinterpret_cast<const bf16x8*>(Bs + row * 128 + ((q ^ sm_sw(row)) << 4));
      }
#pragma unroll
      for (int tn = 0; tn < 2; ++tn)
#pragma unroll
        for (int tm = 0; tm < 2; ++tm)
          c[tn][tm] = __builtin_amdgcn_mfma_f32_16x16x32_bf16(bfg[tn], af[tm], c[tn][tm], 0, 0, 0);
    }
  };

  auto mma64r = [&](int kc_unused, const bf16x8 (&a)[2][2], const char* Bs, floatx4 (&c)[2][2])
      __attribute__((always_inline)) {
#pragma unroll
    for (int ks = 0; ks < 2; ++ks) {
      const int q = ks * 4 + fh;
      bf16x8 bfg[2];
#pragma unroll
      for (int tn = 0; tn < 2; ++tn) {
        const int row = wn * 32 + tn * 16 + fr;
        bfg[tn] = *reinterpret_cast<const bf16x8*>(Bs + row * 128 + ((q ^ sm_sw(row)) << 4));
      }
#pragma unroll
      for (int tn = 0; tn < 2; ++tn)
#pragma unroll
        for (int tm = 0; tm < 2; ++tm)
          c[tn][tm] = __builtin_amdgcn_mfma_f32_16x16x32_bf16(bfg[tn], a[ks][tm], c[tn][tm], 0, 0, 0);
    }
  };

  bf16x8 bset[XP ? 2 : 1][XP ? KS2 : 1][2][2];
  auto read_B = [&](bf16x8 (&dst)[XP ? KS2 : 1][2][2], const char* Bs) __attribute__((always_inline)) {
#pragma unroll
    for (int c = 0; c < (XP ? KS2 : 1); ++c)
#pragma unroll
      for (int ks = 0; ks < 2; ++ks)
#pragma unroll
        for (int tn = 0; tn < 2; ++tn) {
          const int row = wn * 32 + tn * 16 + fr, q = ks * 4 + fh;
          dst[c][ks][tn] =
              *reinterpret_cast<const bf16x8*>(Bs + c * B_CHUNK + row * 128 + ((q ^ sm_sw(row)) << 4));
        }
  };
  auto mma_xr = [&](const bf16x8 (&b)[2][2], const bf16x8 (&a)[2][2], floatx4 (&c)[2][2])
      __attribute__((always_inline)) {
#pragma unroll
    for (int ks = 0; ks < 2; ++ks)
#pragma unroll
      for (int tn = 0; tn < 2; ++tn)
#pragma unroll
        for (int tm = 0; tm < 2; ++tm)
          c[tn][tm] = __builtin_amdgcn_mfma_f32_16x16x32_bf16(b[ks][tn], a[ks][tm], c[tn][tm], 0, 0, 0);
  };
  auto mma_xl = [&](const bf16x8 (&b)[2][2], const char* As, floatx4 (&c)[2][2])
      __attribute__((always_inline)) {
#pragma unroll
    for (int ks = 0; ks < 2; ++ks) {
      const int q = ks * 4 + fh;
      bf16x8 af[2];
#pragma unroll
      for (int tm = 0; tm < 2; ++tm) {
        const int row = wm * 32 + tm * 16 + fr;
        af[tm] = *reinterpret_cast<const bf16x8*>(As + row * 128 + ((q ^ sm_sw(row)) << 4));
      }
#pragma unroll
      for (int tn = 0; tn < 2; ++tn)
#pragma unroll
        for (int tm = 0; tm < 2; ++tm)
          c[tn][tm] = __builtin_amdgcn_mfma_f32_16x16x32_bf16(b[ks][tn], af[tm], c[tn][tm], 0, 0, 0);
    }
  };

  dispatch_act(p.act, true, [&](auto A1, auto A2) __attribute__((always_inline)) {
    constexpr int act1 = decltype(A1)::value, act2 = decltype(A2)::value;
    for (int t = 0; t < ntiles; ++t) {
      const bool warm = t < S::kSteady;
      char* Rs = lds + R_OFF + (t % RD) * R_SLOT;
      sm_static_for<SPT>([&](auto JC) __attribute__((always_inline)) {
        constexpr int j = decltype(JC)::value;
        const int s = t * SPT + j;
        if constexpr (j == SY) {
          if (warm) sm_wait_vm<S::safe_E()>();
          else sm_wait_vm<S::wE(S::kFar)>();
          sm_lds_barrier();
          const float* bias_t = reinterpret_cast<const float*>(lds + BIAS_OFF) + t * 64;
#pragma unroll
          for (int tn = 0; tn < 2; ++tn) {
            const int c0 = wn * 32 + tn * 16 + fh * 4;
            const float4 bv = *reinterpret_cast<const float4*>(bias_t + c0);
#pragma unroll
            for (int tm = 0; tm < 2; ++tm) {
              const int row = wm * 32 + tm * 16 + fr;
              bf16x4* ptr = reinterpret_cast<bf16x4*>(Rs + row * 128 + (((c0 >> 3) ^ sm_sw(row)) << 4) +
                                                      (c0 & 7) * 2);
              const bf16x4 rv = *ptr;
              bf16x4 o;
              o[0] = f2bf(act_c<act2>(act_c<act1>(acc[tn][tm][0] + bv.x) + (float)rv[0]));
              o[1] = f2bf(act_c<act2>(act_c<act1>(acc[tn][tm][1] + bv.y) + (float)rv[1]));
              o[2] = f2bf(act_c<act2>(act_c<act1>(acc[tn][tm][2] + bv.z) + (float)rv[2]));
              o[3] = f2bf(act_c<act2>(act_c<act1>(acc[tn][tm][3] + bv.w) + (float)rv[3]));
              *ptr = o;
            }
          }
          sm_lds_barrier();
#pragma unroll
          for (int i = 0; i < 2; ++i) {
            const int idx = tid + NT * i;
            const int row = idx >> 3, c = idx & 7;
            const bf16x8 v = *reinterpret_cast<const bf16x8*>(Rs + row * 128 + ((c ^ sm_sw(row)) << 4));
            const int m = m0 + row, n = t * 64 + c * 8;
            const int off = (m < p.M && n < Cout) ? (m * p.ldy + p.y_coff + n) * 2 : kSmOOB;
            __builtin_amdgcn_raw_buffer_store_b128(__builtin_bit_cast(kv_i32x4, v), ry, off, 0, 2);
          }
        }
        if constexpr (j == 0) {
#pragma unroll
          for (int a = 0; a < 2; ++a)
#pragma unroll
            for (int b = 0; b < 2; ++b) acc[a][b] = floatx4{0.f, 0.f, 0.f, 0.f};
        }
        if constexpr (XP) {
          if (warm) sm_wait_vm<S::safe_XB(j)>();
          else sm_wait_vm<S::wXB(S::kFar, j)>();
        } else {
          if (warm) sm_wait_vm<S::safe_B(j)>();
          else sm_wait_vm<S::wB(S::kFar, j)>();
        }
        sm_lds_barrier();
        constexpr int jn = (j + D - 1) % SPT, tadv = (j + D - 1) / SPT;
        issue_B(t + tadv, SmIC<jn>{});
        if constexpr (j == 0) issue_R(t + RD - 1);
        const char* Bs = lds + B_OFF + (s % D) * B_STAGE;
        if constexpr (XP) {
          constexpr int cur = j & 1, nxt = cur ^ 1;
          if constexpr (j == 0) {
            if (t == 0) read_B(bset[cur], Bs);
          }
          read_B(bset[nxt], lds + B_OFF + ((s + 1) % D) * B_STAGE);
#pragma unroll
          for (int c = 0; c < KS2; ++c) {
            if constexpr (j < SY) mma_xr(bset[cur][c], areg[j * KS2 + c], acc);
            else mma_xl(bset[cur][c], Rs, accz[(j - SY) * KS2 + c]);
          }
        } else {
#pragma unroll
          for (int c = 0; c < KS2; ++c) {
            if constexpr (j < SY && AREG) mma64r(0, areg[j * KS2 + c], Bs + c * B_CHUNK, acc);
            else if constexpr (j < SY) mma64(lds + (j * KS2 + c) * (BM * 128), Bs + c * B_CHUNK, acc);
            else mma64(Rs, Bs + c * B_CHUNK, accz[(j - SY) * KS2 + c]);
          }
        }
      });
    }
  });

  asm volatile("s_waitcnt vmcnt(0)" ::: "memory");
  __syncthreads();
  const float* b1 = reinterpret_cast<const float*>(lds + b1_off);
  const bool relu_z = p.act_t == 1;
  sm_static_for<NZC>([&](auto ZC) __attribute__((always_inline)) {
    constexpr int zc = decltype(ZC)::value;
    char* Zs = lds + R_OFF + (zc % RD) * R_SLOT;
    if constexpr (zc > 0 && zc % RD == 0) __syncthreads();
#pragma unroll
    for (int tn = 0; tn < 2; ++tn) {
      const int c0 = wn * 32 + tn * 16 + fh * 4;
      const float4 bv = *reinterpret_cast<const float4*>(b1 + zc * 64 + c0);
#pragma unroll
      for (int tm = 0; tm < 2; ++tm) {
        const int row = wm * 32 + tm * 16 + fr;
        float v0 = accz[zc][tn][tm][0] + bv.x, v1 = accz[zc][tn][tm][1] + bv.y;
        float v2 = accz[zc][tn][tm][2] + bv.z, v3 = accz[zc][tn][tm][3] + bv.w;
        if (relu_z) {
          v0 = fmaxf(v0, 0.f); v1 = fmaxf(v1, 0.f); v2 = fmaxf(v2, 0.f); v3 = fmaxf(v3, 0.f);
        }
        bf16x4 o;
        o[0] = f2bf(v0); o[1] = f2bf(v1); o[2] = f2bf(v2); o[3] = f2bf(v3);
        *reinterpret_cast<bf16x4*>(Zs + row * 128 + (((c0 >> 3) ^ sm_sw(row)) << 4) + (c0 & 7) * 2) = o;
      }
    }
    if constexpr (zc % RD == RD - 1 || zc == NZC - 1) {
      __syncthreads();
      constexpr int z0 = zc - zc % RD;
#pragma unroll
      for (int g = z0; g <= zc; ++g) {
        const char* Zg = lds + R_OFF + (g % RD) * R_SLOT;
#pragma unroll
        for (int i = 0; i < 2; ++i) {
          const int idx = tid + NT * i;
          const int row = idx >> 3, c = idx & 7;
          const bf16x8 v = *reinterpret_cast<const bf16x8*>(Zg + row * 128 + ((c ^ sm_sw(row)) << 4));
          const int m = m0 + row, n = g * 64 + c * 8;
          const int off = (m < p.M && n < N1) ? (m * p.ldz + p.z_coff + n) * 2 : kSmOOB;
          __builtin_amdgcn_raw_buffer_store_b128(__builtin_bit_cast(kv_i32x4, v), rz, off, 0, 0);
        }
      }
    }
  });
}

typedef void (*SmFn)(const KvConvParams, int);

struct SmTile {
  int nc3, nzc, d, rd, nw, ks2, areg;
  SmFn fn;
};

template <int NC3, int NZC, int D, int RD, int NW = 8, int KS2 = 1, bool AREG = false,
          bool XP = false>
constexpr SmTile sm_tile() {
  return SmTile{NC3, NZC, D, RD, NW, KS2, AREG ? 1 : 0,
                &conv_seam_kernel<NC3, NZC, D, RD, NW, KS2, AREG, XP>};
}

static const SmTile kSmTiles[] = {
    sm_tile<2, 2, 4, 3, 4>(),
    sm_tile<2, 2, 6, 3>(),
    sm_tile<2, 2, 4, 3, 8, 2>(),
    sm_tile<2, 2, 6, 3, 4, 1, true>(),
    sm_tile<2, 2, 6, 3, 8, 2, true>(),
    sm_tile<2, 4, 6, 3, 8, 2, true>(),
    sm_tile<2, 4, 6, 3>(),
    sm_tile<4, 4, 4, 4, 8, 2, true, true>(),
    sm_tile<4, 4, 4, 4, 8, 2, true>(),
    sm_tile<4, 4, 3, 2, 8, 2>(),
    sm_tile<4, 4, 5, 2>(),
    sm_tile<4, 4, 3, 2, 4>(),
    sm_tile<4, 4, 6, 2, 8, 2, true>(),
    sm_tile<4, 4, 8, 3, 8, 1, true>(),
    sm_tile<4, 4, 3, 5, 8, 2, true>(),
    sm_tile<4, 8, 4, 3>(),
};

int sm_lds_bytes(const SmTile& e, int cout, int n1) {
  const int bm = 16 * e.nw, round = e.nw * 1024;
  return (e.areg ? 0 : e.nc3 * bm * 128) + e.d * e.ks2 * 64 * 128 + e.rd * bm * 128 +
         ((cout * 4 + round - 1) / round) * round + ((n1 * 4 + round - 1) / round) * round;
}

}

int seam_num_tiles() { return (int)(sizeof(kSmTiles) / sizeof(kSmTiles[0])); }

int seam_pick_tile(const KvConvParams* p) {
  for (int i = 0; i < seam_num_tiles(); ++i) {
    const SmTile& e = kSmTiles[i];
    if (p->Kpad == e.nc3 * 64 && p->n_t == e.nzc * 64 && sm_lds_bytes(e, p->Cout, p->n_t) <= kSmLdsMax)
      return i;
  }
  return -1;
}

int seam_launch(const KvConvParams* p, int tile, hipStream_t stream) {
  if (tile < 0 || tile >= seam_num_tiles()) return -6;
  const SmTile& e = kSmTiles[tile];
  if (p->mode != 1 || !p->res || p->x2 || !p->w_t || !p->z || p->in_u8 || p->pair_1x1) return -8;
  if (p->Kpad != e.nc3 * 64 || p->Cin > p->Kpad || p->n_t != e.nzc * 64 || p->Cout % 64) return -8;
  if (p->ldx % 8 || p->x_coff % 8 || p->ldy % 8 || p->y_coff % 8 || p->ldr % 8 || p->r_coff % 8 ||
      p->ldz % 8 || p->z_coff % 8 || p->x_coff + p->Cin > p->ldx || p->y_coff + p->Cout > p->ldy ||
      p->r_coff + p->Cout > p->ldr || p->z_coff + p->n_t > p->ldz)
    return -8;
  if ((long long)p->M * p->ldy * 2 >= kSmOOB || (long long)p->M * p->ldr * 2 >= kSmOOB ||
      (long long)p->M * p->ldx * 2 >= kSmOOB || (long long)p->M * p->ldz * 2 >= kSmOOB ||
      (long long)p->Cout * p->Kpad * 2 >= kSmOOB || (long long)p->n_t * p->Cout * 2 >= kSmOOB)
    return -9;
  const int lds = sm_lds_bytes(e, p->Cout, p->n_t);
  if (lds > kSmLdsMax) return -11;
  const int nbm = (p->M + 16 * e.nw - 1) / (16 * e.nw), ntiles = p->Cout / 64;
  if (nbm <= 0 || ntiles <= 0) return 0;
  if (hipFuncSetAttribute(reinterpret_cast<const void*>(e.fn),
                          hipFuncAttributeMaxDynamicSharedMemorySize, lds) != hipSuccess)
    return -7;
  hipLaunchKernelGGL(e.fn, dim3((unsigned)nbm), dim3(64 * e.nw), (unsigned)lds, stream, *p, ntiles);
  return hipGetLastError() == hipSuccess ? 0 : -7;
}

}
```

### csrc/kernels/conv_stream.hip

```cpp
#include "common.h"
#include "kvedge_kernels.h"

#include <cstdlib>

typedef float floatx16 __attribute__((ext_vector_type(16)));
typedef float floatx4 __attribute__((ext_vector_type(4)));
typedef unsigned int u32x4 __attribute__((ext_vector_type(4)));

template <int MF>
struct SAccOf { typedef floatx16 type; static constexpr int n = 16; };
template <>
struct SAccOf<16> { typedef floatx4 type; static constexpr int n = 4; };

namespace kvedge {
namespace {

constexpr int BK = 64;
constexpr int kOOB = 0x7ffffff0;
constexpr int kLdsMax = 160 * 1024;

__device__ __forceinline__ __amdgpu_buffer_rsrc_t mk_rsrc(const void* base, int bytes) {
  return __builtin_amdgcn_make_buffer_rsrc(const_cast<void*>(base), (short)0, bytes, 0x00020000);
}

template <int AUX = 0>
__device__ __forceinline__ void dma16(__amdgpu_buffer_rsrc_t rs, bf16* lds, int voff, int soff) {
  __builtin_amdgcn_raw_ptr_buffer_load_lds(
      rs, (__attribute__((address_space(3))) void*)lds, 16, voff, soff, 0, AUX);
}

template <int N, int I = 0, class F>
__device__ __forceinline__ void static_for(F&& f) {
  if constexpr (I < N) {
    f(IC<I>{});
    static_for<N, I + 1>(f);
  }
}

template <int N>
__device__ __forceinline__ void wait_vm() {
  asm volatile("s_waitcnt vmcnt(%0)" ::"n"(N < 63 ? N : 63) : "memory");
}

__host__ __device__ constexpr int stream_lds_bytes(int bm, int bn, int d, bool res, bool bres,
                                                   int kpad, int nt1 = 0) {
  return 2 * (d * (bm * BK + (bres ? 0 : bn * BK)) + (bres ? bn * kpad : 0) + bm * (bn + 8) +
              nt1 * bn);
}

template <int BM, int BN, int D, int MODE, bool RES, bool BRES, int POL, int NT1 = 0, int MF = 32>
__global__ __launch_bounds__(256, (NT1 || (BM * BN >= 128 * 128 && BRES)) ? 1 : 2)
void conv_stream_kernel(const KvConvParams p) {
  constexpr int WM = 2, WN = 2;
  constexpr int WTM = BM / WM, WTN = BN / WN;
  constexpr int TM = WTM / MF, TN = WTN / MF;
  using Acc = typename SAccOf<MF>::type;
  constexpr int NACC = SAccOf<MF>::n;
  constexpr int A_INS = BM / 32, B_INS = BN / 32;
  constexpr int CS = BN + 8;
  constexpr int CPR = BN / 8;
  constexpr int PER = BM * CPR / 256;
  constexpr int SA = BM * BK, SB = BRES ? 0 : BN * BK;
  constexpr int SLOT = SA + SB;
  constexpr int SI = A_INS + (BRES ? 0 : B_INS) + (RES ? PER : 0);
  constexpr int PERZ = NT1 ? BM * NT1 / 8 / 256 : 0;
  constexpr int EPI = PER + PERZ;
  static_assert(NT1 == 0 || (BM == 64 && BRES && NT1 % 64 == 0 && PERZ >= 1), "tail tile");
  constexpr int SP = POL;
  constexpr int YP = NT1 > 0 ? 2 : SP;
  static_assert(TM >= 1 && TN >= 1 && PER >= 1 && D >= 2 && D <= 6, "tile");
  extern __shared__ __attribute__((aligned(16))) bf16 smem[];
  const int nk = p.Kpad / BK;
  bf16* const Bres = smem + D * SLOT;
  bf16* const Cs = Bres + (BRES ? BN * p.Kpad : 0);
  bf16* const W1s = Cs + BM * CS;

  const int tid = threadIdx.x, lane = tid & 63;
  const int wv = __builtin_amdgcn_readfirstlane(tid >> 6);
  const int wm = wv / WN, wn = wv % WN;
  const int nbm = (p.M + BM - 1) / BM, nbn = (p.Cout + BN - 1) / BN;
  const int logical = xcd_remap(blockIdx.x, gridDim.x);
  const int nb = logical % nbn;
  const int n0 = nb * BN;
  const int mstep = gridDim.x / nbn;
  const int mfirst = logical / nbn;
  const int ntiles = mfirst < nbm ? (nbm - 1 - mfirst) / mstep + 1 : 0;
  const int nstages = ntiles * nk;
  if (nstages == 0) return;

  const __amdgpu_buffer_rsrc_t rx = mk_rsrc(p.x, p.N * p.H * p.W * p.ldx * 2);
  const __amdgpu_buffer_rsrc_t rw = mk_rsrc(p.w, p.Cout * p.Kpad * 2);
  const __amdgpu_buffer_rsrc_t rx2 =
      mk_rsrc(MODE == 4 ? p.x2 : p.x, MODE == 4 ? p.N * p.H2 * p.W2 * p.ldx2 * 2 : 0);
  const __amdgpu_buffer_rsrc_t rr = mk_rsrc(RES ? p.res : p.x, RES ? p.M * p.ldr * 2 : 0);
  const __amdgpu_buffer_rsrc_t ry = mk_rsrc(p.y, p.M * p.ldy * 2);

  const int lrow = lane >> 3, pch = lane & 7;
  int b_off[B_INS];
#pragma unroll
  for (int i = 0; i < B_INS; ++i) {
    const int row = (wv * B_INS + i) * 8 + lrow;
    const int n = n0 + row;
    b_off[i] = n < p.Cout ? (n * p.Kpad + (pch ^ ((row >> 1) & 7)) * 8) * 2 : kOOB;
  }
  int a_lc[A_INS];
#pragma unroll
  for (int i = 0; i < A_INS; ++i) {
    const int row = (wv * A_INS + i) * 8 + lrow;
    a_lc[i] = pch ^ ((row >> 1) & 7);
  }
  const int HoWo = p.Ho * p.Wo;

  typedef u32x4 ResRegs[RES ? PER : 1];
  auto issue = [&](int s, int slot, ResRegs& rdst) __attribute__((always_inline)) {
    const int ti = s / nk, kt = s - ti * nk;
    const bool tv = ti < ntiles;
    const int m0 = (mfirst + ti * mstep) * BM;
    bf16* As = smem + slot * SLOT;
    const int kbase = kt * BK;
    if (MODE == 4 && kbase >= p.K1) {
#pragma unroll
      for (int i = 0; i < A_INS; ++i) {
        const int m = m0 + (wv * A_INS + i) * 8 + lrow;
        int v = kOOB;
        if (tv && m < p.M) {
          const int img = m / HoWo, rem = m - img * HoWo;
          const int ho = rem / p.Wo, wo = rem - ho * p.Wo;
          v = (((img * p.H2 + ho * p.stride2) * p.W2 + wo * p.stride2) * p.ldx2 + a_lc[i] * 8) * 2;
        }
        dma16<YP>(rx2, As + (wv * A_INS + i) * 512, v, (kbase - p.K1) * 2);
      }
    } else {
#pragma unroll
      for (int i = 0; i < A_INS; ++i) {
        const int m = m0 + (wv * A_INS + i) * 8 + lrow;
        const bool ok = tv && m < p.M && (MODE == 4 || kbase + a_lc[i] * 8 < p.Cin);
        const int v = ok ? (m * p.ldx + p.x_coff + a_lc[i] * 8) * 2 : kOOB;
        dma16<YP>(rx, As + (wv * A_INS + i) * 512, v, kbase * 2);
      }
    }
    if (!BRES) {
      bf16* Bs = As + SA;
#pragma unroll
      for (int i = 0; i < B_INS; ++i)
        dma16(rw, Bs + (wv * B_INS + i) * 512, tv ? b_off[i] : kOOB, kbase * 2);
    }
    if (RES) {
      const bool last = kt == nk - 1 && tv;
#pragma unroll
      for (int j = 0; j < PER; ++j) {
        const int idx = tid + 256 * j;
        const int m = m0 + idx / CPR, n = n0 + (idx % CPR) * 8;
        const int off = (last && m < p.M && n < p.Cout) ? (m * p.ldr + p.r_coff + n) * 2 : kOOB;
        rdst[j] = __builtin_amdgcn_raw_buffer_load_b128(rr, off, 0, YP);
      }
    }
  };

  Acc acc[TN][TM];
  auto zero_acc = [&]() __attribute__((always_inline)) {
#pragma unroll
    for (int a = 0; a < TN; ++a)
#pragma unroll
      for (int b = 0; b < TM; ++b)
#pragma unroll
        for (int e = 0; e < NACC; ++e) acc[a][b][e] = 0.f;
  };

  const int fr = lane & (MF - 1), fh = lane / MF;
  const int fr32 = lane & 31, fh32 = lane >> 5;
  auto compute = [&](int slot, int kt) __attribute__((always_inline)) {
    const bf16* As = smem + slot * SLOT;
    const bf16* Bs = BRES ? Bres + kt * BN * BK : As + SA;
    bf16x8 af[2][TM], bfg[2][TN];
    constexpr int KS = BK / (MF == 32 ? 16 : 32);
    auto load = [&](int buf, int ks) __attribute__((always_inline)) {
      const int q = ks * (64 / MF) + fh;
#pragma unroll
      for (int tm = 0; tm < TM; ++tm) {
        const int row = wm * WTM + tm * MF + fr;
        af[buf][tm] = *reinterpret_cast<const bf16x8*>(As + row * BK + ((q ^ ((row >> 1) & 7)) << 3));
      }
#pragma unroll
      for (int tn = 0; tn < TN; ++tn) {
        const int row = wn * WTN + tn * MF + fr;
        bfg[buf][tn] = *reinterpret_cast<const bf16x8*>(Bs + row * BK + ((q ^ ((row >> 1) & 7)) << 3));
      }
    };
    load(0, 0);
#pragma unroll
    for (int ks = 0; ks < KS; ++ks) {
      if (ks < KS - 1) load((ks + 1) & 1, ks + 1);
#pragma unroll
      for (int tn = 0; tn < TN; ++tn)
#pragma unroll
        for (int tm = 0; tm < TM; ++tm) {
          if constexpr (MF == 32)
            acc[tn][tm] = __builtin_amdgcn_mfma_f32_32x32x16_bf16(bfg[ks & 1][tn], af[ks & 1][tm],
                                                                  acc[tn][tm], 0, 0, 0);
          else
            acc[tn][tm] = __builtin_amdgcn_mfma_f32_16x16x32_bf16(bfg[ks & 1][tn], af[ks & 1][tm],
                                                                  acc[tn][tm], 0, 0, 0);
        }
    }
    __builtin_amdgcn_sched_group_barrier(0x100, TM + TN, 0);
#pragma unroll
    for (int ks = 0; ks < KS; ++ks) {
      if (ks < KS - 1) __builtin_amdgcn_sched_group_barrier(0x100, TM + TN, 0);
      __builtin_amdgcn_sched_group_barrier(0x008, TM * TN, 0);
    }
  };


  float4 bias_r[TN][NACC / 4];
#pragma unroll
  for (int tn = 0; tn < TN; ++tn)
#pragma unroll
    for (int g = 0; g < NACC / 4; ++g) {
      const int n = n0 + wn * WTN + tn * MF + g * 8 + fh * 4;
      bias_r[tn][g] = (p.bias && n < p.Cout) ? *reinterpret_cast<const float4*>(p.bias + n)
                                             : make_float4(0.f, 0.f, 0.f, 0.f);
    }

  constexpr int TN1 = NT1 ? NT1 / 64 : 1;
  float4 bias1_r[TN1][4];
  const __amdgpu_buffer_rsrc_t rz = mk_rsrc(NT1 ? p.z : p.y, NT1 ? p.M * p.ldz * 2 : 0);
  if constexpr (NT1 > 0) {
#pragma unroll
    for (int tn = 0; tn < TN1; ++tn)
#pragma unroll
      for (int g = 0; g < 4; ++g) {
        const int n = (wv & 1) * (NT1 / 2) + tn * 32 + g * 8 + fh32 * 4;
        bias1_r[tn][g] = p.bias_t ? *reinterpret_cast<const float4*>(p.bias_t + n)
                                  : make_float4(0.f, 0.f, 0.f, 0.f);
      }
  }

  auto tail = [&](int m0) __attribute__((always_inline)) {
    asm volatile("s_waitcnt lgkmcnt(0)" ::: "memory");
    __builtin_amdgcn_s_barrier();
    asm volatile("" ::: "memory");
    const int wm2 = wv >> 1, wn2 = wv & 1;
    floatx16 acc2[TN1];
#pragma unroll
    for (int tn = 0; tn < TN1; ++tn)
#pragma unroll
      for (int g = 0; g < 4; ++g) {
        acc2[tn][4 * g + 0] = bias1_r[tn][g].x;
        acc2[tn][4 * g + 1] = bias1_r[tn][g].y;
        acc2[tn][4 * g + 2] = bias1_r[tn][g].z;
        acc2[tn][4 * g + 3] = bias1_r[tn][g].w;
      }
#pragma unroll
    for (int kk = 0; kk < BN / 16; ++kk) {
      const bf16x8 a = *reinterpret_cast<const bf16x8*>(Cs + (wm2 * 32 + fr32) * CS + kk * 16 + fh32 * 8);
      const int kt = kk >> 2, q = (kk & 3) * 2 + fh32;
#pragma unroll
      for (int tn = 0; tn < TN1; ++tn) {
        const int row = wn2 * (NT1 / 2) + tn * 32 + fr32;
        const bf16x8 b = *reinterpret_cast<const bf16x8*>(
            W1s + kt * NT1 * BK + row * BK + ((q ^ ((row >> 1) & 7)) << 3));
        acc2[tn] = __builtin_amdgcn_mfma_f32_32x32x16_bf16(b, a, acc2[tn], 0, 0, 0);
      }
    }
    asm volatile("s_waitcnt lgkmcnt(0)" ::: "memory");
    __builtin_amdgcn_s_barrier();
    asm volatile("" ::: "memory");
    constexpr int CZ = NT1 + 8;
#pragma unroll
    for (int tn = 0; tn < TN1; ++tn)
#pragma unroll
      for (int g = 0; g < 4; ++g) {
        const int nl = wn2 * (NT1 / 2) + tn * 32 + g * 8 + fh32 * 4;
        bf16x4 o;
        o[0] = f2bf(fmaxf(acc2[tn][4 * g + 0], 0.f));
        o[1] = f2bf(fmaxf(acc2[tn][4 * g + 1], 0.f));
        o[2] = f2bf(fmaxf(acc2[tn][4 * g + 2], 0.f));
        o[3] = f2bf(fmaxf(acc2[tn][4 * g + 3], 0.f));
        *reinterpret_cast<bf16x4*>(Cs + (wm2 * 32 + fr32) * CZ + nl) = o;
      }
    asm volatile("s_waitcnt lgkmcnt(0)" ::: "memory");
    __builtin_amdgcn_s_barrier();
    asm volatile("" ::: "memory");
    constexpr int ZPR = NT1 ? NT1 / 8 : 1;
#pragma unroll
    for (int j = 0; j < PERZ; ++j) {
      const int idx = tid + 256 * j;
      const int ml = idx / ZPR, ch = idx % ZPR;
      const int m = m0 + ml;
      const bf16x8 v = *reinterpret_cast<const bf16x8*>(Cs + ml * CZ + ch * 8);
      const int off = m < p.M ? (m * p.ldz + p.z_coff + ch * 8) * 2 : kOOB;
      __builtin_amdgcn_raw_buffer_store_b128(__builtin_bit_cast(u32x4, v), rz, off, 0, SP);
    }
  };

  auto epilogue = [&](int ti, const ResRegs& rres, auto A1, auto A2) __attribute__((always_inline)) {
    constexpr int act1 = decltype(A1)::value, act2 = decltype(A2)::value;
    const int m0 = (mfirst + ti * mstep) * BM;
#pragma unroll
    for (int tn = 0; tn < TN; ++tn) {
#pragma unroll
      for (int g = 0; g < NACC / 4; ++g) {
        const int nl = wn * WTN + tn * MF + g * 8 + fh * 4;
        const float4 bv = bias_r[tn][g];
#pragma unroll
        for (int tm = 0; tm < TM; ++tm) {
          const int ml = wm * WTM + tm * MF + fr;
          bf16x4 o;
          o[0] = f2bf(act_c<act1>(acc[tn][tm][4 * g + 0] + bv.x));
          o[1] = f2bf(act_c<act1>(acc[tn][tm][4 * g + 1] + bv.y));
          o[2] = f2bf(act_c<act1>(acc[tn][tm][4 * g + 2] + bv.z));
          o[3] = f2bf(act_c<act1>(acc[tn][tm][4 * g + 3] + bv.w));
          *reinterpret_cast<bf16x4*>(Cs + ml * CS + nl) = o;
        }
      }
    }
    asm volatile("s_waitcnt lgkmcnt(0)" ::: "memory");
    __builtin_amdgcn_s_barrier();
    asm volatile("" ::: "memory");
#pragma unroll
    for (int j = 0; j < PER; ++j) {
      const int idx = tid + 256 * j;
      const int ml = idx / CPR, ch = idx % CPR;
      const int m = m0 + ml, n = n0 + ch * 8;
      bf16x8 v = *reinterpret_cast<const bf16x8*>(Cs + ml * CS + ch * 8);
      if (RES) {
        const bf16x8 rv = __builtin_bit_cast(bf16x8, rres[j]);
#pragma unroll
        for (int e = 0; e < 8; ++e) v[e] = f2bf(act_c<act2>((float)v[e] + (float)rv[e]));
      }
      const int off = (m < p.M && n < p.Cout) ? (m * p.ldy + p.y_coff + n) * 2 : kOOB;
      __builtin_amdgcn_raw_buffer_store_b128(__builtin_bit_cast(u32x4, v), ry, off, 0, YP);
      if constexpr (NT1 > 0) *reinterpret_cast<bf16x8*>(Cs + ml * CS + ch * 8) = v;
    }
    if constexpr (NT1 > 0) tail(m0);
  };

  if (BRES) {
    for (int kt = 0; kt < nk; ++kt)
#pragma unroll
      for (int i = 0; i < B_INS; ++i)
        dma16(rw, Bres + kt * BN * BK + (wv * B_INS + i) * 512, b_off[i], kt * BK * 2);
  }
  if constexpr (NT1 > 0) {
    const __amdgpu_buffer_rsrc_t rw1 = mk_rsrc(p.w_t, p.n_t * p.Cout * 2);
    constexpr int B1 = NT1 / 32;
#pragma unroll
    for (int kt = 0; kt < BN / BK; ++kt)
#pragma unroll
      for (int i = 0; i < B1; ++i) {
        const int row = (wv * B1 + i) * 8 + lrow;
        const int off = row < p.n_t ? (row * p.Cout + (pch ^ ((row >> 1) & 7)) * 8) * 2 : kOOB;
        dma16(rw1, W1s + kt * NT1 * BK + (wv * B1 + i) * 512, off, kt * BK * 2);
      }
  }
  ResRegs rres[D];
  static_for<D - 1>([&](auto S) __attribute__((always_inline)) {
    constexpr int i = decltype(S)::value;
    issue(i, i, rres[i]);
  });
  zero_acc();
  const int nround = (nstages + D - 1) / D * D;
  dispatch_act(p.act, RES, [&](auto A1, auto A2) __attribute__((always_inline)) {
  for (int j0 = 0; j0 < nround; j0 += D) {
    static_for<D>([&](auto U) __attribute__((always_inline)) {
      constexpr int u = decltype(U)::value;
      const int j = j0 + u;
      const int ti = j / nk, kt = j - ti * nk;
      const int lo = j - D + 1 > 0 ? j - D + 1 : 0;
      const int e = j / nk - lo / nk;
      if (e <= 0) wait_vm<(D - 2) * SI>();
      else if (e == 1) wait_vm<(D - 2) * SI + EPI>();
      else if (e == 2) wait_vm<(D - 2) * SI + 2 * EPI>();
      else if (e == 3) wait_vm<(D - 2) * SI + 3 * EPI>();
      else if (e == 4) wait_vm<(D - 2) * SI + 4 * EPI>();
      else wait_vm<(D - 2) * SI + 5 * EPI>();
      asm volatile("s_waitcnt lgkmcnt(0)" ::: "memory");
      __builtin_amdgcn_s_barrier();
      asm volatile("" ::: "memory");
      constexpr int un = (u + D - 1) % D;
      issue(j + D - 1, un, rres[un]);
      compute(u, kt);
      if (kt == nk - 1) {
        epilogue(ti, rres[u], A1, A2);
        zero_acc();
      }
    });
  }
  });
}

}

typedef void (*StreamFn)(const KvConvParams);

template <int BM, int BN, int D, bool BRES, int POL = 0, int MF = 32>
StreamFn stream_get(int mode, bool res, int nt) {
  if (nt) return nullptr;
  if (mode == 4) return conv_stream_kernel<BM, BN, D, 4, false, BRES, POL, 0, MF>;
  return res ? conv_stream_kernel<BM, BN, D, 1, true, BRES, POL, 0, MF>
             : conv_stream_kernel<BM, BN, D, 1, false, BRES, POL, 0, MF>;
}

template <int BM, int BN, int D, int MF = 32>
StreamFn stream_get_tail(int mode, bool res, int nt) {
  if (nt == 0) return stream_get<BM, BN, D, true, 0, MF>(mode, res, 0);
  if constexpr (D == 3) if (nt == 64) {
    if (mode == 4) return conv_stream_kernel<BM, BN, D, 4, false, true, 0, 64, MF>;
    return res ? conv_stream_kernel<BM, BN, D, 1, true, true, 0, 64, MF> : nullptr;
  }
  if constexpr (D == 2) if (nt == 128) {
    if (mode == 4) return conv_stream_kernel<BM, BN, D, 4, false, true, 0, 128, MF>;
    return res ? conv_stream_kernel<BM, BN, D, 1, true, true, 0, 128, MF> : nullptr;
  }
  return nullptr;
}

struct StreamTile {
  int bm, bn, d;
  bool bres;
  StreamFn (*get)(int, bool, int);
};

static const StreamTile kStreamTiles[] = {
    {64, 64, 4, true, &stream_get<64, 64, 4, true>},
    {64, 128, 4, true, &stream_get<64, 128, 4, true>},
    {128, 64, 4, true, &stream_get<128, 64, 4, true>},
    {64, 64, 6, true, &stream_get<64, 64, 6, true>},
    {64, 128, 3, true, &stream_get<64, 128, 3, true>},
    {64, 64, 4, false, &stream_get<64, 64, 4, false>},
    {128, 64, 4, false, &stream_get<128, 64, 4, false>},
    {128, 128, 3, false, &stream_get<128, 128, 3, false>},
    {64, 128, 4, false, &stream_get<64, 128, 4, false>},
    {64, 128, 3, true, &stream_get<64, 128, 3, true, 2>},
    {64, 64, 4, true, &stream_get<64, 64, 4, true, 2>},
    {128, 128, 3, false, &stream_get<128, 128, 3, false, 2>},
    {128, 128, 3, true, &stream_get<128, 128, 3, true>},
    {128, 128, 2, true, &stream_get<128, 128, 2, true>},
    {128, 128, 3, true, &stream_get<128, 128, 3, true, 2>},
    {64, 64, 4, true, &stream_get<64, 64, 4, true, 0, 16>},
    {64, 128, 3, true, &stream_get<64, 128, 3, true, 0, 16>},
    {128, 128, 3, false, &stream_get<128, 128, 3, false, 2, 16>},
    {64, 256, 3, true, &stream_get_tail<64, 256, 3, 16>},
    {64, 256, 2, true, &stream_get_tail<64, 256, 2, 16>},
    {64, 256, 3, true, &stream_get_tail<64, 256, 3>},
    {64, 256, 2, true, &stream_get_tail<64, 256, 2>},
};

}

namespace kvedge {

int stream_num_tiles() { return (int)(sizeof(kStreamTiles) / sizeof(kStreamTiles[0])); }
int stream_tail_tile(int n_t) {
  static const int mf16 = [] {
    const char* s = getenv("KVEDGE_TAIL_MF16");
    return s && s[0] == '1' ? 2 : 0;
  }();
  return stream_num_tiles() - (n_t > 64 ? 1 : 2) - mf16;
}

int stream_launch(const KvConvParams* p, int tile, hipStream_t stream) {
  if (tile < 0 || tile >= stream_num_tiles()) return -6;
  if (p->mode != 1 && p->mode != 4) return -8;
  if (p->mode == 4 && (p->res || p->up2 || p->x2_coff)) return -8;
  if ((long long)p->M * p->ldy * 2 >= kOOB || (p->res && (long long)p->M * p->ldr * 2 >= kOOB))
    return -9;
  const long long xb = (long long)p->N * p->H * p->W * p->ldx * 2;
  const long long wb = (long long)p->Cout * p->Kpad * 2;
  if (xb >= kOOB || wb >= kOOB) return -9;
  if (p->mode == 4) {
    const long long x2b = (long long)p->N * p->H2 * p->W2 * p->ldx2 * 2;
    if (!p->x2 || x2b >= kOOB || p->K1 % BK || (p->Kpad - p->K1) % BK) return -10;
  }
  const StreamTile& e = kStreamTiles[tile];
  const bool res = p->res != nullptr;
  if (p->n_t) {
    if ((p->n_t != 64 && p->n_t != 128) || e.bn != p->Cout || !p->z || !p->w_t ||
        p->act_t != 1 || p->ldz % 8 || p->z_coff % 8 || p->ldz < p->z_coff + p->n_t)
      return -8;
    if ((long long)p->M * p->ldz * 2 >= kOOB) return -9;
  }
  const int lds = stream_lds_bytes(e.bm, e.bn, e.d, res, e.bres, p->Kpad, p->n_t);
  if (lds > kLdsMax) return -11;
  const int nbm = (p->M + e.bm - 1) / e.bm, nbn = (p->Cout + e.bn - 1) / e.bn;
  if (nbm <= 0 || nbn <= 0) return 0;
  int per_cu = kLdsMax / lds;
  if (per_cu > 4) per_cu = 4;
  static const int per_cu_env = [] {
    const char* s = getenv("KVEDGE_STREAM_PER_CU");
    return s ? atoi(s) : 0;
  }();
  if (per_cu_env > 0 && per_cu_env < per_cu) per_cu = per_cu_env;
  int mgroups = (256 * per_cu + nbn - 1) / nbn;
  if (mgroups > nbm) mgroups = nbm;
  if (mgroups < 1) mgroups = 1;
  StreamFn fn = e.get(p->mode, res, p->n_t);
  if (!fn) return -8;
  if (hipFuncSetAttribute(reinterpret_cast<const void*>(fn),
                          hipFuncAttributeMaxDynamicSharedMemorySize, lds) != hipSuccess)
    return -7;
  hipLaunchKernelGGL(fn, dim3((unsigned)(mgroups * nbn)), dim3(256), (unsigned)lds, stream, *p);
  return hipGetLastError() == hipSuccess ? 0 : -7;
}

}
```

### csrc/kernels/kvedge_kernels.h

```cpp
#pragma once
#include <hip/hip_runtime.h>
#include <stdint.h>

#ifdef __cplusplus
extern "C" {
#endif

typedef struct KvConvParams {
  const void* x;
  const void* w;
  const float* bias;
  const void* res;
  void* y;
  int N, H, W, Cin;
  int ldx, x_coff;
  int Ho, Wo, Cout;
  int KH, KW, stride, pad;
  int K, Kpad;
  int M;
  int ldy, y_coff, ldr, r_coff;
  int act;
  int mode;
  const void* x2;
  int K1, H2, W2, ldx2, stride2;
  int in_u8;
  const void* w_t;
  const float* bias_t;
  void* z;
  int n_t, ldz, z_coff, act_t;
  int pair_1x1;
  float* ws;
  int ksplit;
  long long ws_elems;
  int x2_coff;
  int up2;
} KvConvParams;

int kv_conv2d(const KvConvParams* p, int tile, hipStream_t stream);
long long kv_set_conv_chunk_bytes(long long bytes);
int kv_conv_num_tiles(void);
int kv_conv_splitk_base(void);
int kv_conv_splitk_num_tiles(void);
int kv_nloop_sched_check(void);
int kv_conv_pick_tile(const KvConvParams* p);
int kv_conv_seam_num_tiles(void);
int kv_conv_pair(const KvConvParams* p, int tile, hipStream_t stream);
int kv_conv_pair_num_tiles(void);

int kv_stem_pool(const void* x, const void* w, const float* bias, void* y, int N, int H, int W,
                 int ldy, int y_coff, hipStream_t s);
int kv_stem_pool_lds_bytes(int W);
int kv_stem_pool_frames(const void* frames, const void* w, const float* bias, void* y, int N,
                        int H0, int W0, const float* mean3, const float* inv_std3, int ldy,
                        int y_coff, hipStream_t s);
int kv_stem12_pool_frames(const void* frames, const void* w, const float* bias, void* y, int N,
                          int H0, int W0, const float* mean3, const float* inv_std3, int ldy,
                          int y_coff, hipStream_t s);
int kv_stem12_lds_bytes(int Ws);
int kv_yolo_stem2(const void* frames, const void* w0, const float* bias0, const void* w1,
                  int w1_ld, const float* bias1, void* y, int N, int H0, int W0, hipStream_t s);
int kv_yolo_stem2_lds_bytes(int Ws);

int kv_maxpool2d(const void* x, void* y, int N, int H, int W, int C, int ldx, int x_coff,
                 int ldy, int y_coff, int k, int stride, int pad, int Ho, int Wo, hipStream_t s);
int kv_sppf_pool(void* buf, int N, int H, int W, int C, hipStream_t s);
int kv_global_avgpool(const void* x, void* y, int N, int HW, int C, hipStream_t s);
int kv_pooled_fc(const void* x, int N, int HW, int C, const void* w, int ldw, const float* bias,
                 void* y, int ncls, hipStream_t s);
int kv_softmax_rows(const void* x, float* y, int64_t* argmax, int rows, int cols, hipStream_t s);
int kv_upsample2x(const void* x, void* y, int N, int H, int W, int C, int ldx, int x_coff,
                  int ldy, int y_coff, hipStream_t s);
int kv_yolo_decode(const void* f0, const void* f1, const void* f2, int h0, int w0, int h1,
                   int w1, int h2, int w2, int s0, int s1, int s2, int N, int nc,
                   float* boxes, float* scores, int* cls, hipStream_t s);
int kv_nms(const float* boxes, const float* scores, const int* cls, int N, int A,
           float conf_thres, float iou_thres, int max_det, float* out, int* count,
           hipStream_t s);
int kv_synth_frames(uint8_t* y, int N, int H, int W, uint64_t seed, uint64_t step,
                    hipStream_t s);
int kv_synth_frames_dev(uint8_t* y, int N, int H, int W, uint64_t seed, uint64_t* step,
                        int bump_done, hipStream_t s);
int kv_preprocess(const uint8_t* x, void* y, int N, int H, int W, const float* mean3,
                  const float* inv_std3, hipStream_t s);
int kv_preprocess_s2d(const uint8_t* x, void* y, int N, int H, int W, const float* mean3,
                      const float* inv_std3, hipStream_t s);
int kv_frame_resize(const uint8_t* src, uint8_t* dst, int N, int Hs, int Ws, int Hd, int Wd,
                    const int* axis_y, const int* axis_x, int pad, hipStream_t s);
int kv_det_to_source(float* det, const int* count, int N, int max_det, float cy, float sy,
                     float cx, float sx, int Hs, int Ws, hipStream_t s);
int kv_roi_crop(const uint8_t* src, const float* det, const int* count, uint8_t* dst, int N,
                int Hs, int Ws, int max_det, int K, int D, int pad, hipStream_t s);
int kv_roi_crop_band(const uint8_t* src, const float* det, const int* count, uint8_t* dst, int N,
                     int Hs, int Ws, int max_det, int K, int D, int pad, int band, hipStream_t s);
int kv_batchnorm_nhwc(const void* x, void* y, const float* scale, const float* shift,
                      int64_t rows, int C, int relu, hipStream_t s);

typedef struct KvC2fParams {
  const void* x;
  void* y;
  const void* w1;
  const float* b1;
  const void* wm1;
  const float* bm1;
  const void* wm2;
  const float* bm2;
  const void* w2;
  const float* b2;
  int N, H, W, ldx, x_coff, ldy, y_coff;
  int ldw1, ldwm, ldw2;
  int S;
} KvC2fParams;
int kv_c2f16_supported(int H, int W, int S);
int kv_c2f16_fused(const KvC2fParams* p, hipStream_t stream);

#ifdef __cplusplus
}
#endif
```

### kvedge_amd/models/layers.py

```python
from __future__ import annotations

from dataclasses import dataclass
from typing import Optional

import torch
import torch.nn as nn

from .. import ops
from ..ops import ConvSpec


def fold_bn(conv: nn.Conv2d, bn: Optional[nn.BatchNorm2d]):
    w = conv.weight.detach().float()
    b = conv.bias.detach().float() if conv.bias is not None else torch.zeros(w.shape[0])
    if bn is None:
        return w.clone(), b.clone()
    inv = bn.weight.detach().float() / torch.sqrt(bn.running_var.detach().float() + bn.eps)
    wf = w * inv[:, None, None, None]
    bf = (b - bn.running_mean.detach().float()) * inv + bn.bias.detach().float()
    return wf, bf


_RECORDER: Optional[list] = None


class record_convs:

    def __enter__(self):
        global _RECORDER
        _RECORDER = []
        return _RECORDER

    def __exit__(self, *exc):
        global _RECORDER
        _RECORDER = None


def _recorder_active() -> bool:
    return _RECORDER is not None


def _record(layer, key, fn) -> None:
    _RECORDER.append((layer, key, fn))


@dataclass
class DeployedConv:
    spec: ConvSpec
    w: torch.Tensor
    b: torch.Tensor
    tile: int = -1

    @staticmethod
    def from_modules(conv: nn.Conv2d, bn: Optional[nn.BatchNorm2d], act: int,
                     device="cpu") -> "DeployedConv":
        wf, bf = fold_bn(conv, bn)
        cout, cin, kh, kw = wf.shape
        assert kh == kw and conv.stride[0] == conv.stride[1] and conv.padding[0] == conv.padding[1]
        spec = ConvSpec.auto(cin, cout, kh, conv.stride[0], conv.padding[0], act)
        return DeployedConv(spec, ops.pack_conv_weight(wf, spec).to(device),
                            bf.contiguous().to(device))

    @staticmethod
    def stem_s2d(conv: nn.Conv2d, bn: Optional[nn.BatchNorm2d], act: int,
                 device="cpu", in_scale: float = 1.0) -> "DeployedConv":
        wf, bf = fold_bn(conv, bn)
        wf = wf * in_scale
        cout, cin, k, _ = wf.shape
        p, s = conv.padding[0], conv.stride[0]
        assert s == 2 and cin <= 4 and conv.padding[0] == conv.padding[1]
        q = (p + 1) // 2
        ka = (k - 1 + 2 * q - p) // 2 + 1
        w2 = torch.zeros(cout, 16, ka, ka)
        for a in range(ka):
            for dy in range(2):
                r = 2 * a + dy + p - 2 * q
                if not 0 <= r < k:
                    continue
                for b in range(ka):
                    for dx in range(2):
                        t = 2 * b + dx + p - 2 * q
                        if not 0 <= t < k:
                            continue
                        ch = (dy * 2 + dx) * 4
                        w2[:, ch:ch + cin, a, b] = wf[:, :, r, t]
        spec = ConvSpec(16, cout, ka, ka, 1, q, act, ops.MODE_GENERAL, pad_b=ka - 1 - q)
        return DeployedConv(spec, ops.pack_conv_weight(w2, spec).to(device),
                            bf.contiguous().to(device))

    def to(self, device) -> "DeployedConv":
        return DeployedConv(self.spec, self.w.to(device), self.b.to(device), self.tile)

    def __call__(self, x, res=None, out=None, x_coff=0, y_coff=0, r_coff=0, tile=None):
        out = ops.conv2d(x, self.spec, self.w, self.b, res=res, out=out, x_coff=x_coff,
                         y_coff=y_coff, r_coff=r_coff, tile=self.tile if tile is None else tile)
        if _RECORDER is not None:
            s = self.spec
            key = ("conv", s.cin, s.cout, s.kh, s.kw, s.stride, s.pad, s.act, s.mode,
                   tuple(x.shape), x_coff, tuple(out.shape), res is not None)
            fn = lambda t, o=out: ops.conv2d(x, s, self.w, self.b, res=res, out=o,
                                             x_coff=x_coff, y_coff=y_coff, r_coff=r_coff, tile=t)
            _RECORDER.append((self, key, fn))
        return out

    @property
    def flops_per_pixel(self) -> int:
        s = self.spec
        return 2 * s.kh * s.kw * s.cin * s.cout


@dataclass
class DeployedDualConv:
    w: torch.Tensor
    b: torch.Tensor
    k1: int
    stride2: int
    act: int
    tile: int = -1

    @staticmethod
    def from_modules(conv3, bn3, down_conv, down_bn, act, device="cpu") -> "DeployedDualConv":
        w3, b3 = fold_bn(conv3, bn3)
        wd, bd = fold_bn(down_conv, down_bn)
        assert w3.shape[2:] == (1, 1) and wd.shape[2:] == (1, 1)
        w = torch.cat([w3[:, :, 0, 0], wd[:, :, 0, 0]], 1)
        return DeployedDualConv(w.to(torch.bfloat16).contiguous().to(device),
                                (b3 + bd).contiguous().to(device), w3.shape[1],
                                down_conv.stride[0], act)

    def __call__(self, y, x, out=None, tile=None):
        out = ops.conv_dual(y, x, self.w, self.b, self.act, self.stride2, out=out,
                            tile=self.tile if tile is None else tile)
        if _RECORDER is not None:
            key = ("dual", tuple(y.shape), tuple(x.shape), tuple(self.w.shape), self.stride2,
                   self.act)
            fn = lambda t, o=out: ops.conv_dual(y, x, self.w, self.b, self.act,
                                                self.stride2, out=o, tile=t)
            _RECORDER.append((self, key, fn))
        return out

    def flops_per_pixel(self) -> int:
        return 2 * self.w.shape[0] * self.w.shape[1]


@torch.no_grad()
def calibrate_bn(model: nn.Module, batches, momentum: Optional[float] = None) -> None:
    bns = [m for m in model.modules() if isinstance(m, nn.BatchNorm2d)]
    saved = [(m.momentum) for m in bns]
    for m in bns:
        m.reset_running_stats()
        m.momentum = momentum
    model.train()
    for x in batches:
        model(x)
    model.eval()
    for m, mo in zip(bns, saved):
        m.momentum = mo


def frames_to_nchw(frames_u8: torch.Tensor, mean=ops.IMAGENET_MEAN,
                   std=ops.IMAGENET_STD) -> torch.Tensor:
    x = frames_u8.float() / 255.0
    x = (x - torch.tensor(mean, device=x.device)) / torch.tensor(std, device=x.device)
    return x.permute(0, 3, 1, 2).contiguous()


def count_flops(module: nn.Module, input_shape) -> int:
    import copy

    m = copy.deepcopy(module).to("meta").eval()
    total = [0]

    def hook(mod, inp, out):
        if isinstance(mod, nn.Conv2d):
            kh, kw = mod.kernel_size
            total[0] += 2 * out.numel() * (mod.in_channels // mod.groups) * kh * kw
        elif isinstance(mod, nn.Linear):
            total[0] += 2 * out.numel() * mod.in_features

    hs = [x.register_forward_hook(hook) for x in m.modules()
          if isinstance(x, (nn.Conv2d, nn.Linear))]
    with torch.no_grad():
        m(torch.empty(*input_shape, device="meta"))
    for h in hs:
        h.remove()
    return total[0] // input_shape[0]
```

### kvedge_amd/models/resnet.py

```python
from __future__ import annotations

import os

from typing import List, Optional

import torch
import torch.nn as nn
import torch.nn.functional as F

from .. import ops
from .layers import (DeployedConv, DeployedDualConv, calibrate_bn, count_flops, fold_bn,
                     frames_to_nchw)

ACT_NONE, ACT_RELU = ops.ACT_NONE, ops.ACT_RELU
TAIL1_MIN_ROWS = int(os.environ.get("KVEDGE_TAIL1_MIN_ROWS", "32768"))


class Bottleneck(nn.Module):
    expansion = 4

    def __init__(self, cin: int, width: int, stride: int):
        super().__init__()
        cout = width * self.expansion
        self.conv1 = nn.Conv2d(cin, width, 1, bias=False)
        self.bn1 = nn.BatchNorm2d(width)
        self.conv2 = nn.Conv2d(width, width, 3, stride, 1, bias=False)
        self.bn2 = nn.BatchNorm2d(width)
        self.conv3 = nn.Conv2d(width, cout, 1, bias=False)
        self.bn3 = nn.BatchNorm2d(cout)
        self.downsample = None
        if stride != 1 or cin != cout:
            self.downsample = nn.Sequential(nn.Conv2d(cin, cout, 1, stride, bias=False),
                                            nn.BatchNorm2d(cout))

    def forward(self, x):
        idt = x if self.downsample is None else self.downsample(x)
        y = F.relu(self.bn1(self.conv1(x)))
        y = F.relu(self.bn2(self.conv2(y)))
        y = self.bn3(self.conv3(y))
        return F.relu(y + idt)


class ResNet50Ref(nn.Module):
    layers_cfg = ((64, 3, 1), (128, 4, 2), (256, 6, 2), (512, 3, 2))

    def __init__(self, num_classes: int = 1000):
        super().__init__()
        self.conv1 = nn.Conv2d(3, 64, 7, 2, 3, bias=False)
        self.bn1 = nn.BatchNorm2d(64)
        blocks: List[nn.Module] = []
        cin = 64
        for width, n, stride in self.layers_cfg:
            for i in range(n):
                blocks.append(Bottleneck(cin, width, stride if i == 0 else 1))
                cin = width * 4
        self.blocks = nn.Sequential(*blocks)
        self.fc = nn.Linear(2048, num_classes)
        self.num_classes = num_classes

    def forward(self, x):
        x = F.relu(self.bn1(self.conv1(x)))
        x = F.max_pool2d(x, 3, 2, 1)
        x = self.blocks(x)
        x = torch.flatten(F.adaptive_avg_pool2d(x, 1), 1)
        return self.fc(x)


def init_resnet50(seed: int = 0, num_classes: int = 1000, calibrate: bool = True,
                  calib_batch: int = 4, calib_hw: int = 224) -> ResNet50Ref:
    g = torch.Generator().manual_seed(seed)
    m = ResNet50Ref(num_classes)
    for mod in m.modules():
        if isinstance(mod, nn.Conv2d):
            fan_out = mod.out_channels * mod.kernel_size[0] * mod.kernel_size[1]
            with torch.no_grad():
                mod.weight.normal_(0.0, (2.0 / fan_out) ** 0.5, generator=g)
        elif isinstance(mod, nn.BatchNorm2d):
            nn.init.ones_(mod.weight)
            nn.init.zeros_(mod.bias)
        elif isinstance(mod, nn.Linear):
            bound = 1.0 / mod.in_features ** 0.5
            with torch.no_grad():
                mod.weight.uniform_(-bound, bound, generator=g)
                mod.bias.uniform_(-bound, bound, generator=g)
    if calibrate:
        frames = torch.randint(0, 256, (calib_batch, calib_hw, calib_hw, 3), generator=g,
                               dtype=torch.uint8)
        calibrate_bn(m, [frames_to_nchw(frames)])
    m.eval()
    return m


class DeployedBottleneck:

    def __init__(self, b: Bottleneck, device, fuse_down: bool = True):
        self.c1 = DeployedConv.from_modules(b.conv1, b.bn1, ACT_RELU, device)
        self.c2 = DeployedConv.from_modules(b.conv2, b.bn2, ACT_RELU, device)
        self.c3 = DeployedConv.from_modules(b.conv3, b.bn3, ACT_RELU, device)
        self.down = None
        self.dual = None
        if b.downsample is not None:
            self.down = DeployedConv.from_modules(b.downsample[0], b.downsample[1], ACT_NONE,
                                                  device)
            if fuse_down:
                self.dual = DeployedDualConv.from_modules(b.conv3, b.bn3, b.downsample[0],
                                                          b.downsample[1], ACT_RELU, device)

    def __call__(self, x, out=None, t1=None):
        y = self.c1(x) if t1 is None else t1
        y = self.c2(y)
        if self.dual is not None:
            return self.dual(y, x, out=out)
        idt = x if self.down is None else self.down(x)
        return self.c3(y, res=idt, out=out)

    def can_tail(self, nxt: "DeployedBottleneck") -> bool:
        c1 = nxt.c1.spec
        cout = self.c3.spec.cout
        if not (c1.kh == 1 and c1.stride == 1 and c1.pad == 0 and c1.cin == cout and
                c1.act == ACT_RELU and self.c3.spec.act == ACT_RELU):
            return False
        if cout != 256:
            k3 = self.c3.spec.cin
            return (ops.SEAM_ENABLED and self.down is None and self.dual is None and
                    (k3, cout, c1.cout) in ops.SEAM_SHAPES)
        k = self.c3.spec.cin + (self.dual.w.shape[1] - self.dual.k1 if self.dual is not None else 0)
        return (c1.cout in (64, 128) and (self.dual is not None or self.down is None) and
                (self.dual is None or c1.cout == 64) and k <= 128)

    def tail_fits(self, x: torch.Tensor, batch: int = 0) -> bool:
        N, Ho, Wo, _ = self.out_shape(x.shape)
        N = batch or N
        if self.c3.spec.cout == 256:
            return N * Ho * Wo >= TAIL1_MIN_ROWS
        return (N * Ho * Wo + 127) // 128 >= ops.SEAM_MIN_WGS

    def call_tail(self, x, nxt: "DeployedBottleneck", t1=None, out=None, z=None):
        y = self.c1(x) if t1 is None else t1
        y = self.c2(y)
        c1 = nxt.c1
        if self.dual is not None:
            d = self.dual
            return ops.conv_tail(y, d.w, d.b, d.act, c1.w, c1.b, x2=x, stride2=d.stride2,
                                 out=out, z=z)
        return ops.conv_tail(y, self.c3.w, self.c3.b, self.c3.spec.act, c1.w, c1.b, res=x,
                             out=out, z=z)

    def out_shape(self, x_shape):
        N, H, W, _ = x_shape
        Ho, Wo = self.c2.spec.out_hw(H, W)
        return (N, Ho, Wo, self.c3.spec.cout)

    def convs(self):
        return [c for c in (self.c1, self.c2, self.c3, self.down, self.dual) if c is not None]


class KvResNet50:

    image_size = 224

    def __init__(self, ref: ResNet50Ref, device="cuda"):
        self.device = torch.device(device)
        self.num_classes = ref.num_classes
        self.stem = DeployedConv.stem_s2d(ref.conv1, ref.bn1, ACT_RELU, self.device)
        wf, _ = fold_bn(ref.conv1, ref.bn1)
        self.stem12_w = ops.pack_stem12(wf).to(self.device)
        self._flops = {}
        self._ref = ref
        self.blocks = [DeployedBottleneck(b, self.device) for b in ref.blocks]
        fcw = ref.fc.weight.detach().float()[:, :, None, None]
        fc_conv = nn.Conv2d(2048, ref.num_classes, 1, bias=True)
        with torch.no_grad():
            fc_conv.weight.copy_(fcw)
            fc_conv.bias.copy_(ref.fc.bias.detach())
        self.fc = DeployedConv.from_modules(fc_conv, None, ACT_NONE, self.device)

    @staticmethod
    def build(seed: int = 0, device="cuda", calibrate: bool = True) -> "KvResNet50":
        return KvResNet50(init_resnet50(seed, calibrate=calibrate), device)

    def convs(self) -> List[DeployedConv]:
        out = [self.stem]
        for b in self.blocks:
            out += b.convs()
        return out + [self.fc]

    def flops_per_image(self, hw: int = 224) -> int:
        if hw not in self._flops:
            self._flops[hw] = count_flops(self._ref, (1, 3, hw, hw))
        return self._flops[hw]

    def frame_plan(self, src_hw, image_size: int = 0) -> "ops.ResizePlan":
        return ops.center_crop_plan(src_hw, image_size or self.image_size)

    def preprocess(self, frames_u8: torch.Tensor) -> torch.Tensor:
        return ops.preprocess(frames_u8, s2d=True)

    microbatch: int = 0
    microbatch_blocks: int = 3
    fuse_stem_pool: bool = True
    fuse_preprocess: bool = True
    fuse_tail: bool = True
    stem12: bool = True

    def stem_and_pool(self, x: torch.Tensor, frames_in: bool = False) -> torch.Tensor:
        if frames_in:
            if self.stem12:
                return ops.stem12_pool_frames(x, self.stem12_w, self.stem.b)
            return ops.stem_pool_frames(x, self.stem.spec, self.stem.w, self.stem.b)
        if self.fuse_stem_pool:
            return ops.stem_pool(x, self.stem.spec, self.stem.w, self.stem.b)
        return ops.maxpool2d(self.stem(x), 3, 2, 1)

    def features(self, x: torch.Tensor, frames_in: bool = False) -> torch.Tensor:
        B = x.shape[0]
        mb = self.microbatch
        nb = self.microbatch_blocks
        t1 = None
        if mb and B > mb and B % mb == 0 and 0 < nb < len(self.blocks):
            full = full_t1 = None
            for i in range(0, B, mb):
                y = self.stem_and_pool(x[i:i + mb], frames_in)
                z = None
                for j in range(nb):
                    b, nxt = self.blocks[j], self.blocks[j + 1]
                    last = j == nb - 1
                    if last and full is None:
                        shp = b.out_shape(y.shape)
                        full = ops.empty((B,) + shp[1:], dtype=y.dtype, device=y.device)
                    fuse = (self.fuse_tail and y.is_cuda and b.can_tail(nxt) and
                            b.tail_fits(y, batch=B))
                    if last and full_t1 is None and fuse:
                        full_t1 = ops.empty(full.shape[:3] + (nxt.c1.spec.cout,),
                                            dtype=y.dtype, device=y.device)
                    o = full[i:i + mb] if last else None
                    if fuse:
                        y, z = b.call_tail(y, nxt, t1=z, out=o,
                                           z=full_t1[i:i + mb] if last else None)
                    else:
                        y, z = b(y, t1=z, out=o), None
            x, t1 = full, full_t1
            rest = self.blocks[nb:]
        else:
            x = self.stem_and_pool(x, frames_in)
            rest = self.blocks
        for i, b in enumerate(rest):
            nxt = rest[i + 1] if i + 1 < len(rest) else None
            if (self.fuse_tail and x.is_cuda and nxt is not None and b.can_tail(nxt) and
                    b.tail_fits(x)):
                x, t1 = b.call_tail(x, nxt, t1=t1)
            else:
                x, t1 = b(x, t1=t1), None
        return x

    def logits(self, x: torch.Tensor, frames_in: bool = False) -> torch.Tensor:
        f = self.features(x, frames_in)
        B = f.shape[0]
        if f.is_cuda and B <= ops.POOLED_FC_MAX_BATCH and self.fuse_head:
            return ops.pooled_fc(f, self.fc.w, self.fc.b)
        pooled = ops.global_avgpool(f).view(B, 1, 1, 2048)
        return self.fc(pooled).view(B, self.num_classes)

    fuse_head: bool = os.environ.get("KVEDGE_FUSE_HEAD", "0") == "1"

    def raw_outputs(self, frames_u8: torch.Tensor) -> torch.Tensor:
        if self.fuse_preprocess and self.fuse_stem_pool and frames_u8.is_cuda:
            return self.logits(frames_u8, frames_in=True)
        return self.logits(self.preprocess(frames_u8))

    def __call__(self, frames_u8: torch.Tensor, out: Optional[dict] = None):
        lg = self.raw_outputs(frames_u8)
        probs, top1 = ops.softmax_rows(lg)
        return probs, top1
```

### kvedge_amd/ops/__init__.py

```python
from __future__ import annotations

import os
from dataclasses import dataclass
from typing import Optional, Sequence, Tuple

import torch

from . import reference as _ref

_LIB_PATH = os.path.join(os.path.dirname(os.path.dirname(os.path.abspath(__file__))),
                         "_C_checks.so" if os.environ.get("KVEDGE_CHECKS", "0") not in ("", "0")
                         else os.path.basename(os.environ.get("KVEDGE_LIB", "") or "_C.so"))
_loaded = False
_load_error: Optional[str] = None

ACT_NONE, ACT_RELU, ACT_SILU = 0, 1, 2
RES_AFTER_ACT = 4
MODE_GENERAL, MODE_GEMM, MODE_STEM = 0, 1, 2
BK = 64


def load(build_if_missing: bool = False) -> bool:
    global _loaded, _load_error
    if _loaded:
        return True
    if not os.path.exists(_LIB_PATH) and build_if_missing:
        from .. import _build

        _build.build()
    if not os.path.exists(_LIB_PATH):
        _load_error = f"{_LIB_PATH} not built (run `python -m kvedge_amd._build`)"
        return False
    try:
        torch.ops.load_library(_LIB_PATH)
    except Exception as e:
        _load_error = f"failed to load {_LIB_PATH}: {e}"
        return False
    _check_single_hip_runtime()
    global SPLITK0
    SPLITK0 = int(torch.ops.kvedge.conv_splitk_base())
    if int(torch.ops.kvedge.conv_splitk_num_tiles()) != N_SPLITK_TILES:
        _load_error = "split-K tile count differs from the native library (stale build?)"
        return False
    _loaded = True
    return True


def _check_single_hip_runtime() -> None:
    try:
        with open("/proc/self/maps") as f:
            libs = {ln.split()[-1] for ln in f if "libamdhip64" in ln}
    except OSError:
        return
    real = {os.path.realpath(p) for p in libs}
    if len(real) > 1:
        raise RuntimeError(f"kvedge: multiple HIP runtimes loaded: {sorted(real)}")


def native_available() -> bool:
    return load()


def library_path() -> str:
    return _LIB_PATH


_recorder = None


def empty(*shape, dtype=None, device=None) -> torch.Tensor:
    t = torch.empty(*shape, dtype=dtype, device=device)
    if _recorder is not None:
        _recorder(t)
    return t


def set_alloc_recorder(fn) -> None:
    global _recorder
    _recorder = fn


def _native():
    if not load():
        raise RuntimeError(
            "kvedge_amd native kernels are required for GPU tensors but unavailable: "
            f"{_load_error}")
    return torch.ops.kvedge


@dataclass
class ConvSpec:
    cin: int
    cout: int
    kh: int
    kw: int
    stride: int = 1
    pad: int = 0
    act: int = ACT_NONE
    mode: int = MODE_GENERAL
    pad_b: int = -1

    @property
    def pad_end(self) -> int:
        return self.pad if self.pad_b < 0 else self.pad_b

    @property
    def cin_eff(self) -> int:
        return 4 if self.mode == MODE_STEM else self.cin

    @property
    def kwp(self) -> int:
        return (self.kw + 1) // 2 * 2

    @property
    def K(self) -> int:
        if self.mode == MODE_STEM:
            return self.kh * self.kwp * 4
        return self.kh * self.kw * self.cin

    @property
    def Kpad(self) -> int:
        return (self.K + BK - 1) // BK * BK

    def out_hw(self, h: int, w: int):
        p = self.pad + self.pad_end
        return ((h + p - self.kh) // self.stride + 1, (w + p - self.kw) // self.stride + 1)

    @staticmethod
    def auto(cin, cout, k, stride=1, pad=None, act=ACT_NONE) -> "ConvSpec":
        if pad is None:
            pad = k // 2
        if cin < 8:
            mode = MODE_STEM
        elif k == 1 and stride == 1 and pad == 0:
            mode = MODE_GEMM
        else:
            mode = MODE_GENERAL
        return ConvSpec(cin, cout, k, k, stride, pad, act, mode)


def pack_conv_weight(w: torch.Tensor, spec: ConvSpec) -> torch.Tensor:
    assert w.shape == (spec.cout, spec.cin, spec.kh, spec.kw), (w.shape, spec)
    w = w.detach().float()
    if spec.mode == MODE_STEM:
        wp = torch.zeros(spec.cout, spec.kh, spec.kwp, 4, dtype=torch.float32, device=w.device)
        wp[:, :, :spec.kw, :spec.cin] = w.permute(0, 2, 3, 1)
        flat = wp.reshape(spec.cout, -1)
    else:
        flat = w.permute(0, 2, 3, 1).reshape(spec.cout, -1)
    out = torch.zeros(spec.cout, spec.Kpad, dtype=torch.float32, device=w.device)
    out[:, :flat.shape[1]] = flat
    return out.to(torch.bfloat16).contiguous()


def unpack_conv_weight(wp: torch.Tensor, spec: ConvSpec) -> torch.Tensor:
    wf = wp.float()[:, :spec.K]
    if spec.mode == MODE_STEM:
        w4 = wf.reshape(spec.cout, spec.kh, spec.kwp, 4)[:, :, :spec.kw, :spec.cin]
        return w4.permute(0, 3, 1, 2).contiguous()
    return wf.reshape(spec.cout, spec.kh, spec.kw, spec.cin).permute(0, 3, 1, 2).contiguous()


_WS: dict = {}
SPLITK_MAX_ELEMS = 32 << 20
SPLITK_MAX_SPLIT = 32
N_SPLITK_TILES = 19
N_DE_TILES = 3
N_SKINNY_TILES = 9
SPLITK0 = 1 << 30


def is_splitk(tile: int) -> bool:
    return SPLITK0 <= tile < SPLITK0 + N_SPLITK_TILES


def splitk_workspace(device: torch.device, elems: int) -> Optional[torch.Tensor]:
    if elems > SPLITK_MAX_ELEMS // 2:
        return None
    key = (device.index, torch.cuda.current_stream(device).cuda_stream)
    ws = _WS.get(key)
    if ws is None:
        ws = torch.empty(SPLITK_MAX_ELEMS, dtype=torch.float32, device=device)
        _WS[key] = ws
    return ws


def conv2d(x: torch.Tensor, spec: ConvSpec, w: torch.Tensor, bias: Optional[torch.Tensor],
           res: Optional[torch.Tensor] = None, out: Optional[torch.Tensor] = None,
           x_coff: int = 0, y_coff: int = 0, r_coff: int = 0, tile: int = -1) -> torch.Tensor:
    N, H, W, ldx = x.shape
    Ho, Wo = spec.out_hw(H, W)
    if out is None:
        out = empty(N, Ho, Wo, spec.cout, dtype=torch.bfloat16, device=x.device)
    assert out.shape[:3] == (N, Ho, Wo), (out.shape, (N, Ho, Wo))
    ldy = out.shape[3]
    ldr = res.shape[-1] if res is not None else 0
    if x.is_cuda:
        ws = splitk_workspace(x.device, N * Ho * Wo * spec.cout) if is_splitk(tile) else None
        _native().conv(x, w, bias, res, out, N, H, W, spec.cin_eff, ldx, x_coff, Ho, Wo,
                       spec.cout, spec.kh, spec.kw, spec.stride, spec.pad, spec.K, ldy, y_coff,
                       ldr, r_coff, spec.act, spec.mode, tile, ws)
    else:
        _ref.conv2d(x, spec, w, bias, res, out, x_coff, y_coff, r_coff)
    return out


def conv_pair(x: torch.Tensor, spec: ConvSpec, w: torch.Tensor, bias: torch.Tensor,
              w2: torch.Tensor, b2: torch.Tensor, out: torch.Tensor, x_coff: int = 0,
              z_coff: int = 0, tile: int = 0) -> torch.Tensor:
    assert spec.kh == 3 and spec.stride == 1 and spec.pad == 1 and spec.mode == MODE_GENERAL
    C2 = w2.shape[0]
    assert w2.shape[1] == spec.cout and out.shape[:3] == x.shape[:3]
    if x.is_cuda:
        _native().conv_pair(x, w, bias, w2, b2, out, spec.cin, x_coff, z_coff, spec.act, tile)
        return out
    t = torch.empty(*x.shape[:3], spec.cout, dtype=torch.bfloat16)
    _ref.conv2d(x, spec, w, bias, None, t, x_coff, 0, 0)
    z = t.float() @ w2.float().t() + b2.float()
    out[..., z_coff:z_coff + C2] = z.to(out.dtype)
    return out


def conv_dual(x1: torch.Tensor, x2: torch.Tensor, w: torch.Tensor, bias: Optional[torch.Tensor],
              act: int, stride2: int, out: Optional[torch.Tensor] = None,
              tile: int = -1) -> torch.Tensor:
    N, Ho, Wo, K1 = x1.shape
    cout = w.shape[0]
    if out is None:
        out = empty(N, Ho, Wo, cout, dtype=torch.bfloat16, device=x1.device)
    if x1.is_cuda:
        ws = splitk_workspace(x1.device, N * Ho * Wo * cout) if is_splitk(tile) else None
        _native().conv_dual(x1, x2, w, bias, out, stride2, act, tile, ws)
    else:
        _ref.conv_dual(x1, x2, w, bias, act, stride2, out)
    return out


def conv_dual2(x: torch.Tensor, K1: int, x2: torch.Tensor, w: torch.Tensor,
               bias: Optional[torch.Tensor], act: int, out: torch.Tensor, x_coff: int = 0,
               x2_coff: int = 0, y_coff: int = 0, stride2: int = 1, up2: bool = False,
               tile: int = -1) -> torch.Tensor:
    if x.is_cuda:
        N, Ho, Wo, _ = x.shape
        ws = splitk_workspace(x.device, N * Ho * Wo * w.shape[0]) if is_splitk(tile) else None
        _native().conv_dual2(x, x_coff, K1, x2, x2_coff, w, bias, out, y_coff, stride2,
                             1 if up2 else 0, act, tile, ws)
    else:
        _ref.conv_dual2(x, x_coff, K1, x2, x2_coff, w, bias, act, stride2, up2, out, y_coff)
    return out


def conv_tail(x: torch.Tensor, w: torch.Tensor, bias: Optional[torch.Tensor], act: int,
              w1: torch.Tensor, b1: Optional[torch.Tensor], res: Optional[torch.Tensor] = None,
              x2: Optional[torch.Tensor] = None, stride2: int = 1,
              out: Optional[torch.Tensor] = None, z: Optional[torch.Tensor] = None,
              tile: int = -1):
    N, H, W, _ = x.shape
    cout, nt = w.shape[0], w1.shape[0]
    if out is None:
        out = empty(N, H, W, cout, dtype=torch.bfloat16, device=x.device)
    if z is None:
        z = empty(N, H, W, nt, dtype=torch.bfloat16, device=x.device)
    if x.is_cuda:
        _native().conv_tail(x, x2, w, bias, res, out, w1, b1, z, stride2, act, tile)
        return out, z
    if x2 is not None:
        _ref.conv_dual(x, x2, w, bias, act, stride2, out)
    else:
        spec = ConvSpec.auto(x.shape[3], cout, 1, 1, 0, act)
        _ref.conv2d(x, spec, w, bias, res, out, 0, 0, 0)
    spec1 = ConvSpec.auto(cout, nt, 1, 1, 0, ACT_RELU)
    _ref.conv2d(out, spec1, w1, b1, None, z, 0, 0, 0)
    return out, z


SEAM_SHAPES = {(128, 512, 128), (128, 512, 256), (256, 1024, 256)}
SEAM_ENABLED = os.environ.get("KVEDGE_SEAM", "1") != "0"
SEAM_MIN_WGS = int(os.environ.get("KVEDGE_SEAM_MIN_WGS", "256"))


C2F_ENABLED = os.environ.get("KVEDGE_C2F", "1") != "0"


def c2f16_strip(H: int, W: int) -> int:
    for S in (40, 32, 20, 16, 8, 4):
        if H % S == 0 and W in (80, 160):
            return S
    return 0


def c2f16(x: torch.Tensor, w1: torch.Tensor, b1: torch.Tensor, wm1: torch.Tensor,
          bm1: torch.Tensor, wm2: torch.Tensor, bm2: torch.Tensor, w2: torch.Tensor,
          b2: torch.Tensor, out: Optional[torch.Tensor] = None, x_coff: int = 0,
          y_coff: int = 0, S: int = 0) -> torch.Tensor:
    N, H, W, _ = x.shape
    if out is None:
        out = empty(N, H, W, 32, dtype=torch.bfloat16, device=x.device)
    if x.is_cuda:
        _native().c2f16_fused(x, x_coff, w1, b1, wm1, bm1, wm2, bm2, w2, b2, out, y_coff,
                              S or c2f16_strip(H, W))
        return out
    s1 = ConvSpec.auto(32, 32, 1, 1, 0, ACT_SILU)
    sm1 = ConvSpec.auto(16, 16, 3, 1, 1, ACT_SILU)
    sm2 = ConvSpec.auto(16, 16, 3, 1, 1, ACT_SILU | RES_AFTER_ACT)
    s2 = ConvSpec.auto(48, 32, 1, 1, 0, ACT_SILU)
    cat = torch.empty(N, H, W, 48, dtype=torch.bfloat16)
    u = torch.empty(N, H, W, 16, dtype=torch.bfloat16)
    _ref.conv2d(x, s1, w1, b1, None, cat, x_coff, 0, 0)
    _ref.conv2d(cat, sm1, wm1, bm1, None, u, 16, 0, 0)
    _ref.conv2d(u, sm2, wm2, bm2, cat, cat, 0, 32, 16)
    _ref.conv2d(cat, s2, w2, b2, None, out, 0, y_coff, 0)
    return out


def stem_pool(x: torch.Tensor, spec: "ConvSpec", w: torch.Tensor, bias: torch.Tensor,
              out: Optional[torch.Tensor] = None, y_coff: int = 0) -> torch.Tensor:
    assert spec.cin == 16 and spec.cout == 64 and spec.kh == 4 and spec.stride == 1
    assert spec.pad == 2 and spec.pad_end == 1 and spec.act == ACT_RELU and spec.Kpad == 256
    N, H, W, _ = x.shape
    Hp, Wp = (H - 1) // 2 + 1, (W - 1) // 2 + 1
    if out is None:
        out = empty(N, Hp, Wp, 64, dtype=torch.bfloat16, device=x.device)
    if x.is_cuda:
        _native().stem_pool(x, w, bias, out, y_coff)
    else:
        y = conv2d(x, spec, w, bias)
        maxpool2d(y, 3, 2, 1, out=out, y_coff=y_coff)
    return out


def stem_pool_frames(frames: torch.Tensor, spec: "ConvSpec", w: torch.Tensor,
                     bias: torch.Tensor, out: Optional[torch.Tensor] = None, y_coff: int = 0,
                     mean=None, std=None) -> torch.Tensor:
    assert frames.dtype == torch.uint8 and frames.dim() == 4 and frames.shape[3] == 3
    mean = IMAGENET_MEAN if mean is None else mean
    std = IMAGENET_STD if std is None else std
    if not frames.is_cuda:
        return stem_pool(preprocess(frames, mean=mean, std=std, s2d=True), spec, w, bias,
                         out=out, y_coff=y_coff)
    assert spec.cin == 16 and spec.cout == 64 and spec.kh == 4 and spec.stride == 1
    assert spec.pad == 2 and spec.pad_end == 1 and spec.act == ACT_RELU and spec.Kpad == 256
    N, H0, W0, _ = frames.shape
    H, W = H0 // 2, W0 // 2
    if out is None:
        out = empty(N, (H - 1) // 2 + 1, (W - 1) // 2 + 1, 64, dtype=torch.bfloat16,
                    device=frames.device)
    _native().stem_pool_frames(frames, w, bias, out, list(mean), list(std), y_coff)
    return out


def pack_stem12(wf: torch.Tensor) -> torch.Tensor:
    cout, cin, k, _ = wf.shape
    assert cin == 3 and k == 7
    w = torch.zeros(cout, 4, 4, 2, 2, 3)
    for r in range(4):
        for dy in range(2):
            ky = 2 * r - 1 + dy
            if not 0 <= ky < 7:
                continue
            for s_ in range(4):
                for dx in range(2):
                    kx = 2 * s_ - 1 + dx
                    if 0 <= kx < 7:
                        w[:, r, s_, dy, dx, :] = wf[:, :, ky, kx].float()
    return w.reshape(cout, 192).to(torch.bfloat16).contiguous()


def stem12_reference(frames: torch.Tensor, w12: torch.Tensor, bias: torch.Tensor,
                     mean=None, std=None) -> torch.Tensor:
    mean = IMAGENET_MEAN if mean is None else mean
    std = IMAGENET_STD if std is None else std
    N, H0, W0, _ = frames.shape
    Hs, Ws = H0 // 2, W0 // 2
    m = torch.tensor(mean, dtype=torch.float32)
    inv = 1.0 / torch.tensor(std, dtype=torch.float32)
    x = (frames.float() * (inv / 255.0) + (-m * inv)).to(torch.bfloat16).float()
    x = x.view(N, Hs, 2, Ws, 2, 3).permute(0, 1, 3, 2, 4, 5).reshape(N, Hs, Ws, 12)
    xp = torch.nn.functional.pad(x, (0, 0, 2, 1, 2, 1))
    cols = xp.unfold(1, 4, 1).unfold(2, 4, 1)
    cols = cols.permute(0, 1, 2, 4, 5, 3).reshape(N, Hs, Ws, 192)
    y = cols @ w12.float().t() + bias.float()
    y = y.to(torch.bfloat16).float().relu()
    y = torch.nn.functional.max_pool2d(y.permute(0, 3, 1, 2), 3, 2, 1).permute(0, 2, 3, 1)
    return y.to(torch.bfloat16).contiguous()


def stem12_pool_frames(frames: torch.Tensor, w12: torch.Tensor, bias: torch.Tensor,
                       out: Optional[torch.Tensor] = None, y_coff: int = 0,
                       mean=None, std=None) -> torch.Tensor:
    assert frames.dtype == torch.uint8 and frames.dim() == 4 and frames.shape[3] == 3
    mean = IMAGENET_MEAN if mean is None else mean
    std = IMAGENET_STD if std is None else std
    N, H0, W0, _ = frames.shape
    Hs, Ws = H0 // 2, W0 // 2
    if out is None:
        out = empty(N, (Hs - 1) // 2 + 1, (Ws - 1) // 2 + 1, 64, dtype=torch.bfloat16,
                    device=frames.device)
    if not frames.is_cuda:
        out[..., y_coff:y_coff + 64] = stem12_reference(frames, w12, bias, mean, std)
        return out
    _native().stem12_pool_frames(frames, w12, bias, out, list(mean), list(std), y_coff)
    return out


def yolo_stem2_fits(frames_shape) -> bool:
    _, H, W, _ = frames_shape
    return H % 4 == 0 and W % 32 == 0 and 0 < W <= 640


def yolo_stem2(frames: torch.Tensor, spec0: "ConvSpec", w0: torch.Tensor, b0: torch.Tensor,
               spec1: "ConvSpec", w1: torch.Tensor, b1: torch.Tensor,
               out: Optional[torch.Tensor] = None) -> torch.Tensor:
    assert spec0.kh == 2 and spec0.cin == 16 and spec0.cout == 16, spec0
    assert (spec1.kh, spec1.stride, spec1.cin, spec1.cout) == (3, 2, 16, 32), spec1
    assert spec0.act == ACT_SILU and spec1.act == ACT_SILU
    N, H, W, _ = frames.shape
    if out is None:
        out = empty(N, H // 4, W // 4, 32, dtype=torch.bfloat16, device=frames.device)
    if not frames.is_cuda:
        x = stem_from_frames(frames, spec0, w0, b0)
        return conv2d(x, spec1, w1, b1, out=out)
    _native().yolo_stem2(frames, w0, b0, w1, b1, out)
    return out


def stem_from_frames(frames: torch.Tensor, spec: "ConvSpec", w: torch.Tensor,
                     bias: Optional[torch.Tensor], out: Optional[torch.Tensor] = None,
                     tile: int = -1) -> torch.Tensor:
    assert spec.kh == 2 and spec.stride == 1 and spec.cin == 16, spec
    N, H, W, _ = frames.shape
    if out is None:
        out = empty(N, H // 2, W // 2, spec.cout, dtype=torch.bfloat16, device=frames.device)
    if frames.is_cuda:
        _native().conv_frames_s2d(frames, w, bias, out, spec.act, tile)
        return out
    x = preprocess(frames, mean=(0.0, 0.0, 0.0), std=(1.0 / 255,) * 3, s2d=True)
    return conv2d(x, spec, w, bias, out=out)


def maxpool2d(x: torch.Tensor, k: int, stride: int, pad: int, out: Optional[torch.Tensor] = None,
              C: Optional[int] = None, x_coff: int = 0, y_coff: int = 0) -> torch.Tensor:
    N, H, W, ldx = x.shape
    C = C or (ldx - x_coff)
    Ho = (H + 2 * pad - k) // stride + 1
    Wo = (W + 2 * pad - k) // stride + 1
    if out is None:
        out = empty(N, Ho, Wo, C, dtype=x.dtype, device=x.device)
    if x.is_cuda:
        _native().maxpool2d(x, out, N, H, W, C, ldx, x_coff, out.shape[3], y_coff, k, stride, pad,
                            Ho, Wo)
    else:
        _ref.maxpool2d(x[..., x_coff:x_coff + C], out, C, k, stride, pad, y_coff)
    return out


def sppf_pool(buf: torch.Tensor, C: int) -> torch.Tensor:
    N, H, W, ld = buf.shape
    assert ld == 4 * C
    if buf.is_cuda:
        _native().sppf_pool(buf, N, H, W, C)
    else:
        _ref.sppf_pool(buf, C)
    return buf


def global_avgpool(x: torch.Tensor, out: Optional[torch.Tensor] = None) -> torch.Tensor:
    N, H, W, C = x.shape
    if out is None:
        out = empty(N, C, dtype=x.dtype, device=x.device)
    if x.is_cuda:
        _native().global_avgpool(x, out, N, H * W, C)
    else:
        out.copy_(x.float().mean(dim=(1, 2)).to(out.dtype))
    return out


POOLED_FC_MAX_BATCH = 16


def pooled_fc(x: torch.Tensor, w: torch.Tensor, bias: Optional[torch.Tensor],
              out: Optional[torch.Tensor] = None) -> torch.Tensor:
    N, H, W, C = x.shape
    ncls = w.shape[0]
    if out is None:
        out = empty(N, ncls, dtype=torch.bfloat16, device=x.device)
    if x.is_cuda:
        _native().pooled_fc(x, w, bias, out)
        return out
    pooled = global_avgpool(x).view(N, 1, 1, C)
    spec = ConvSpec(C, ncls, 1, 1, 1, 0, ACT_NONE, MODE_GEMM)
    _ref.conv2d(pooled, spec, w, bias, None, out.view(N, 1, 1, ncls))
    return out


def softmax_rows(x: torch.Tensor, out: Optional[torch.Tensor] = None,
                 argmax: Optional[torch.Tensor] = None):
    if out is None:
        out = empty(x.shape, dtype=torch.float32, device=x.device)
    if argmax is None:
        argmax = empty(x.shape[0], dtype=torch.int64, device=x.device)
    if x.is_cuda:
        _native().softmax_rows(x, out, argmax)
    else:
        xf = x.float()
        out.copy_(torch.softmax(xf, dim=1))
        argmax.copy_(xf.argmax(dim=1))
    return out, argmax


def upsample2x(x: torch.Tensor, out: torch.Tensor, C: Optional[int] = None, x_coff: int = 0,
               y_coff: int = 0):
    N, H, W, ldx = x.shape
    C = C or (ldx - x_coff)
    if x.is_cuda:
        _native().upsample2x(x, out, N, H, W, C, ldx, x_coff, out.shape[3], y_coff)
    else:
        up = x[..., x_coff:x_coff + C].repeat_interleave(2, dim=1).repeat_interleave(2, dim=2)
        out[..., y_coff:y_coff + C] = up
    return out


def yolo_decode(feats: Sequence[torch.Tensor], strides: Sequence[int], nc: int,
                boxes=None, scores=None, cls=None):
    f0, f1, f2 = feats
    N = f0.shape[0]
    hw = [(f.shape[1], f.shape[2]) for f in feats]
    A = sum(h * w for h, w in hw)
    dev = f0.device
    if boxes is None:
        boxes = empty(N, A, 4, dtype=torch.float32, device=dev)
        scores = empty(N, A, dtype=torch.float32, device=dev)
        cls = empty(N, A, dtype=torch.int32, device=dev)
    if f0.is_cuda:
        _native().yolo_decode(f0, f1, f2, hw[0][0], hw[0][1], hw[1][0], hw[1][1], hw[2][0],
                              hw[2][1], strides[0], strides[1], strides[2], nc, boxes, scores, cls)
    else:
        _ref.yolo_decode(feats, strides, nc, boxes, scores, cls)
    return boxes, scores, cls


def nms(boxes, scores, cls, conf: float = 0.25, iou: float = 0.7, max_det: int = 300,
        out=None, count=None):
    N = scores.shape[0]
    if out is None:
        out = empty(N, max_det, 6, dtype=torch.float32, device=scores.device)
        count = empty(N, dtype=torch.int32, device=scores.device)
    if scores.is_cuda:
        _native().nms(boxes, scores, cls, conf, iou, max_det, out, count)
    else:
        _ref.nms(boxes, scores, cls, conf, iou, max_det, out, count)
    return out, count


def synth_frames(out: torch.Tensor, seed: int, step) -> torch.Tensor:
    if out.is_cuda:
        if isinstance(step, torch.Tensor):
            _native().synth_frames_dev(out, step, seed)
        else:
            _native().synth_frames(out, seed, int(step))
    else:
        _ref.synth_frames(out, seed, step)
    return out


IMAGENET_MEAN = (0.485, 0.456, 0.406)
IMAGENET_STD = (0.229, 0.224, 0.225)


def preprocess(x: torch.Tensor, out: Optional[torch.Tensor] = None, mean=IMAGENET_MEAN,
               std=IMAGENET_STD, s2d: bool = False) -> torch.Tensor:
    N, H, W, _ = x.shape
    if out is None:
        shape = (N, H // 2, W // 2, 16) if s2d else (N, H, W, 4)
        out = empty(shape, dtype=torch.bfloat16, device=x.device)
    if x.is_cuda:
        _native().preprocess(x, out, list(mean), list(std))
    else:
        _ref.preprocess(x, out, mean, std)
    return out


RESIZE_MAX_EXTENT = 8192
LETTERBOX_PAD = 114


@dataclass(frozen=True)
class ResizePlan:
    axis_y: Tuple[int, int, int, int, int]
    axis_x: Tuple[int, int, int, int, int]
    pad: int
    src_hw: Tuple[int, int]
    dst_hw: Tuple[int, int]

    def box_map(self) -> Tuple[float, float, float, float]:
        (sy_, ry, oy, c0y, _), (sx_, rx, ox, c0x, _) = self.axis_y, self.axis_x
        return float(c0y - oy), float(sy_ / ry), float(c0x - ox), float(sx_ / rx)


def _check_src_hw(src_hw, dst: int) -> Tuple[int, int]:
    hs, ws = int(src_hw[0]), int(src_hw[1])
    if not (1 <= hs <= RESIZE_MAX_EXTENT and 1 <= ws <= RESIZE_MAX_EXTENT):
        raise ValueError(f"frame size {hs}x{ws} outside 1..{RESIZE_MAX_EXTENT}")
    if not 1 <= dst <= RESIZE_MAX_EXTENT:
        raise ValueError(f"model size {dst} outside 1..{RESIZE_MAX_EXTENT}")
    return hs, ws


def letterbox_plan(src_hw, dst: int) -> ResizePlan:
    hs, ws = _check_src_hw(src_hw, dst)
    r = min(dst / hs, dst / ws)
    nw = min(dst, max(1, int(round(ws * r))))
    nh = min(dst, max(1, int(round(hs * r))))
    left = int(round((dst - nw) / 2 - 0.1))
    top = int(round((dst - nh) / 2 - 0.1))
    return ResizePlan((hs, nh, 0, top, nh), (ws, nw, 0, left, nw), LETTERBOX_PAD, (hs, ws),
                      (dst, dst))


def center_crop_plan(src_hw, dst: int) -> ResizePlan:
    hs, ws = _check_src_hw(src_hw, dst)
    short = dst * 8 // 7
    if hs <= ws:
        rh, rw = short, int(short * ws / hs)
    else:
        rh, rw = int(short * hs / ws), short
    if max(rh, rw) > RESIZE_MAX_EXTENT:
        raise ValueError(f"resized frame {rh}x{rw} exceeds {RESIZE_MAX_EXTENT}")
    oy, ox = int(round((rh - dst) / 2)), int(round((rw - dst) / 2))
    return ResizePlan((hs, rh, oy, 0, dst), (ws, rw, ox, 0, dst), 0, (hs, ws), (dst, dst))


def frame_resize(src: torch.Tensor, plan: ResizePlan,
                 out: Optional[torch.Tensor] = None) -> torch.Tensor:
    assert src.dtype == torch.uint8 and src.dim() == 4 and src.shape[3] == 3
    assert tuple(src.shape[1:3]) == tuple(plan.src_hw), (src.shape, plan.src_hw)
    hd, wd = plan.dst_hw
    if wd % 4:
        raise ValueError(f"frame_resize needs a destination width % 4 == 0, got {wd}")
    if out is None:
        out = torch.empty(src.shape[0], hd, wd, 3, dtype=torch.uint8, device=src.device)
    assert out.shape == (src.shape[0], hd, wd, 3), (out.shape, plan.dst_hw)
    if src.is_cuda:
        _native().frame_resize(src, out, list(plan.axis_y), list(plan.axis_x), plan.pad)
    else:
        _ref.frame_resize(src, plan, out)
    return out


def det_to_source(det: torch.Tensor, count: torch.Tensor, plan: ResizePlan) -> torch.Tensor:
    cy, sy, cx, sx = plan.box_map()
    hs, ws = plan.src_hw
    if det.is_cuda:
        _native().det_to_source(det, count, [cy, sy, cx, sx], hs, ws)
    else:
        _ref.det_to_source(det, count, (cy, sy, cx, sx), hs, ws)
    return det


def roi_crop(src: torch.Tensor, det: torch.Tensor, count: torch.Tensor, k: int, size: int,
             pad: int = 0, out: Optional[torch.Tensor] = None, band: int = 0) -> torch.Tensor:
    assert src.dtype == torch.uint8 and src.dim() == 4 and src.shape[3] == 3
    n = src.shape[0]
    if size % 4:
        raise ValueError(f"roi_crop needs a crop size % 4 == 0, got {size}")
    if not 1 <= size <= RESIZE_MAX_EXTENT:
        raise ValueError(f"crop size {size} outside 1..{RESIZE_MAX_EXTENT}")
    if det.dim() != 3 or det.shape[0] != n or det.shape[2] != 6:
        raise ValueError(f"det must be [N, max_det, 6] for N = {n}, got {tuple(det.shape)}")
    if not 1 <= k <= det.shape[1]:
        raise ValueError(f"roi_crop needs 1 <= k <= max_det = {det.shape[1]}, got {k}")
    if not 0 <= pad <= 255:
        raise ValueError(f"pad {pad} outside 0..255")
    if out is None:
        out = empty(n * k, size, size, 3, dtype=torch.uint8, device=src.device)
    assert out.shape == (n * k, size, size, 3), (out.shape, (n * k, size, size, 3))
    if src.is_cuda:
        if band:
            _native().roi_crop_band(src, det, count, out, pad, band)
        else:
            _native().roi_crop(src, det, count, out, pad)
    else:
        _ref.roi_crop(src, det, count, k, size, pad, out)
    return out


def batchnorm_nhwc(x, scale, shift, relu=False, out=None):
    if out is None:
        out = torch.empty_like(x)
    if x.is_cuda:
        _native().batchnorm_nhwc(x, out, scale, shift, relu)
    else:
        y = x.float() * scale + shift
        out.copy_((y.clamp_min(0) if relu else y).to(out.dtype))
    return out
```

Baseline: 90840 images/sec.

## Store only stride-2 subsampled tail output when next block downsamples

Adds a y_sub=2 mode to the fused tail conv kernels (seam and stream). The residual output y is written only at even (h,w) positions into a quarter-size tensor, because the next block's stride-2 downsample branch reads only those positions. That next block's dual conv then uses stride2=1 on the compacted input. This cuts y write traffic and the strided reads, at the cost of extra index division in the epilogue, new template instantiations and more plumbing through the Python model.

```diff
diff --git a/csrc/bindings/ops.cpp b/csrc/bindings/ops.cpp
--- a/csrc/bindings/ops.cpp
+++ b/csrc/bindings/ops.cpp
@@ -220,7 +220,7 @@
 void conv_tail(const at::Tensor& x, const c10::optional<at::Tensor>& x2, const at::Tensor& w,
                const c10::optional<at::Tensor>& bias, const c10::optional<at::Tensor>& res,
                at::Tensor& y, const at::Tensor& w1, const c10::optional<at::Tensor>& b1,
-               at::Tensor& z, int64_t stride2, int64_t act, int64_t tile) {
+               at::Tensor& z, int64_t stride2, int64_t act, int64_t tile, int64_t y_sub) {
   check_bf16(x, "x");
   check_bf16(w, "w");
   check_bf16(y, "y");
@@ -229,7 +229,13 @@
   TORCH_CHECK(x.dim() == 4 && y.dim() == 4 && z.dim() == 4, "kvedge: NHWC tensors");
   const int64_t N = x.size(0), H = x.size(1), W = x.size(2), K1 = x.size(3);
   const int64_t Cout = y.size(3), Nt = w1.size(0);
-  TORCH_CHECK(y.size(0) == N && y.size(1) == H && y.size(2) == W, "kvedge: y shape");
+  TORCH_CHECK(y_sub >= 0 && y_sub <= 2, "kvedge: conv_tail y_sub must be 0, 1 or 2");
+  if (y_sub == 2) {
+    TORCH_CHECK(y.size(0) == N && y.size(1) == (H + 1) / 2 && y.size(2) == (W + 1) / 2,
+                "kvedge: y_sub = 2 takes y [N, (H+1)/2, (W+1)/2, Cout]");
+  } else {
+    TORCH_CHECK(y.size(0) == N && y.size(1) == H && y.size(2) == W, "kvedge: y shape");
+  }
   TORCH_CHECK(z.size(0) == N && z.size(1) == H && z.size(2) == W && z.size(3) == Nt,
               "kvedge: z shape");
   TORCH_CHECK(w1.dim() == 2 && w1.size(1) == Cout, "kvedge: w1 must be [n_t, Cout]");
@@ -266,7 +272,8 @@
   } else {
     TORCH_CHECK(res.has_value() && res->defined(), "kvedge: conv_tail plain form needs res");
     check_bf16(*res, "res");
-    TORCH_CHECK(res->sizes() == y.sizes(), "kvedge: res shape");
+    TORCH_CHECK(res->dim() == 4 && res->size(0) == N && res->size(1) == H && res->size(2) == W &&
+                    res->size(3) == Cout, "kvedge: res shape");
     TORCH_CHECK(w.dim() == 2 && w.size(0) == Cout && w.size(1) == K1, "kvedge: w [Cout, K1]");
     p.mode = 1; p.K = (int)K1; p.Kpad = (int)K1;
     p.res = res->data_ptr(); p.ldr = (int)Cout;
@@ -279,6 +286,7 @@
     p.bias_t = b1->data_ptr<float>();
   }
   p.z = z.data_ptr(); p.n_t = (int)Nt; p.ldz = (int)Nt; p.z_coff = 0; p.act_t = 1;
+  p.y_sub = (int)y_sub;
   const int rc = kv_conv2d(&p, (int)tile, cur_stream(x));
   TORCH_CHECK(rc == 0, "kvedge: conv_tail failed rc=", rc);
 }
@@ -759,7 +767,7 @@
   m.def("conv_dual(Tensor x1, Tensor x2, Tensor w, Tensor? bias, Tensor(a!) y, int stride2, int act, "
         "int tile, Tensor(b!)? ws=None) -> ()");
   m.def("conv_tail(Tensor x, Tensor? x2, Tensor w, Tensor? bias, Tensor? res, Tensor(a!) y, "
-        "Tensor w1, Tensor? b1, Tensor(b!) z, int stride2, int act, int tile) -> ()");
+        "Tensor w1, Tensor? b1, Tensor(b!) z, int stride2, int act, int tile, int y_sub=1) -> ()");
   m.def("conv_frames_s2d(Tensor frames, Tensor w, Tensor? bias, Tensor(a!) y, int act, "
         "int tile) -> ()");
   m.def("stem_pool(Tensor x, Tensor w, Tensor bias, Tensor(a!) y, int y_coff) -> ()");
diff --git a/csrc/kernels/conv_igemm.hip b/csrc/kernels/conv_igemm.hip
--- a/csrc/kernels/conv_igemm.hip
+++ b/csrc/kernels/conv_igemm.hip
@@ -363,7 +363,7 @@
                                     : (long long)p->N * p->H * p->W * p->ldx * 2)) return -20;
   if (!kv_in_alloc(p->w, (long long)p->Cout * p->Kpad * 2)) return -21;
   if (!kv_in_alloc(p->bias, (long long)p->Cout * 4)) return -22;
-  if (!kv_in_alloc(p->y, M * p->ldy * 2)) return -23;
+  if (!kv_in_alloc(p->y, p->N * kv_conv_y_image_rows(p) * p->ldy * 2)) return -23;
   if (p->res && !kv_in_alloc(p->res, M * p->ldr * 2)) return -24;
   if (p->n_t && (!kv_in_alloc(p->z, M * p->ldz * 2) ||
                  !kv_in_alloc(p->w_t, (long long)p->n_t * p->Cout * 2) ||
@@ -381,7 +381,7 @@
 static long long kv_conv_max_image_bytes(const KvConvParams* p) {
   const long long hw = (long long)p->H * p->W, ohw = (long long)p->Ho * p->Wo;
   long long m = p->in_u8 ? hw * 12 : hw * p->ldx * 2;
-  m = std::max(m, ohw * p->ldy * 2);
+  m = std::max(m, kv_conv_y_image_rows(p) * p->ldy * 2);
   if (p->res) m = std::max(m, ohw * p->ldr * 2);
   if (p->mode == 4) m = std::max(m, (long long)p->H2 * p->W2 * p->ldx2 * 2);
   if (p->n_t) m = std::max(m, ohw * p->ldz * 2);
@@ -413,7 +413,7 @@
       return b ? static_cast<const char*>(b) + (long long)n0 * bytes_per_image : nullptr;
     };
     q.x = adv(p->x, p->in_u8 ? hw * 12 : hw * p->ldx * 2);
-    q.y = const_cast<char*>(adv(p->y, ohw * p->ldy * 2));
+    q.y = const_cast<char*>(adv(p->y, kv_conv_y_image_rows(p) * p->ldy * 2));
     if (p->res) q.res = adv(p->res, ohw * p->ldr * 2);
     if (p->mode == 4) q.x2 = adv(p->x2, (long long)p->H2 * p->W2 * p->ldx2 * 2);
     if (p->n_t) q.z = const_cast<char*>(adv(p->z, ohw * p->ldz * 2));
@@ -424,6 +424,7 @@
 
 static int kv_conv2d_one(const KvConvParams* p, int tile, hipStream_t stream) {
   if (p->Kpad % BK != 0 || p->Cout % 8 != 0) return -1;
+  if (p->y_sub < 0 || p->y_sub > 2 || (p->y_sub == 2 && !p->n_t)) return -8;
   if (p->n_t) {
     const int v3 = kNumTiles + glds_num_tiles();
     const int v9 = kv_conv_num_tiles();
diff --git a/csrc/kernels/conv_seam.hip b/csrc/kernels/conv_seam.hip
--- a/csrc/kernels/conv_seam.hip
+++ b/csrc/kernels/conv_seam.hip
@@ -102,7 +102,7 @@
 }
 
 template <int NC3, int NZC, int D, int RD, int NW = 8, int KS2 = 1, bool AREG = false,
-          bool XP = false>
+          bool XP = false, int YS = 1>
 __global__ __launch_bounds__(64 * NW, NW == 4 ? 2 : 1) void conv_seam_kernel(const KvConvParams p, int ntiles) {
   static_assert(NW == 4 || NW == 8, "waves");
   static_assert(NC3 % KS2 == 0 && NZC % KS2 == 0, "whole chunks per ring stage");
@@ -133,8 +133,9 @@
   const kv_i32x4 rr = kv_rsrc4(p.res, p.M * p.ldr * 2);
   const kv_i32x4 rb3 = kv_rsrc4(p.bias, Cout * 4);
   const kv_i32x4 rb1 = kv_rsrc4(p.bias_t, N1 * 4);
-  const __amdgpu_buffer_rsrc_t ry =
-      __builtin_amdgcn_make_buffer_rsrc(p.y, (short)0, p.M * p.ldy * 2, 0x00020000);
+  const int Hc = (p.Ho + 1) >> 1, Wc = (p.Wo + 1) >> 1;
+  const __amdgpu_buffer_rsrc_t ry = __builtin_amdgcn_make_buffer_rsrc(
+      p.y, (short)0, YS == 2 ? p.N * Hc * Wc * p.ldy * 2 : p.M * p.ldy * 2, 0x00020000);
   const __amdgpu_buffer_rsrc_t rz =
       __builtin_amdgcn_make_buffer_rsrc(p.z, (short)0, p.M * p.ldz * 2, 0x00020000);
 
@@ -148,6 +149,22 @@
     const int m = m0 + row;
     arow_off[i] = m < p.M ? (m * p.ldx + p.x_coff + lc * 8) * 2 : kSmOOB;
     r_src[i] = m < p.M ? (m * p.ldr + p.r_coff + lc * 8) * 2 : kSmOOB;
+  }
+  int ysub_row[2] = {kSmOOB, kSmOOB};
+  if constexpr (YS == 2) {
+    const int HoWo = p.Ho * p.Wo;
+    const FastDiv fHW{0xffffffffu / (unsigned)HoWo + 1u, HoWo};
+    const FastDiv fWo{0xffffffffu / (unsigned)p.Wo + 1u, p.Wo};
+    const int img0 = (int)((unsigned)m0 / (unsigned)HoWo), rem0 = m0 - img0 * HoWo;
+#pragma unroll
+    for (int i = 0; i < 2; ++i) {
+      const int row = (tid + 64 * NW * i) >> 3;
+      const int r = rem0 + row, io = fdiv(r, fHW), rr = fmod_(r, io, fHW);
+      const int ho = fdiv(rr, fWo), wo = fmod_(rr, ho, fWo);
+      const bool keep = m0 + row < p.M && ((ho | wo) & 1) == 0;
+      const int crow = ((img0 + io) * Hc + (ho >> 1)) * Wc + (wo >> 1);
+      ysub_row[i] = keep ? (crow * p.ldy + p.y_coff) * 2 : kSmOOB;
+    }
   }
   int w3_src[BPW], w1_src[BPW], brow[BPW];
 #pragma unroll
@@ -375,7 +392,9 @@
             const int row = idx >> 3, c = idx & 7;
             const bf16x8 v = *reinterpret_cast<const bf16x8*>(Rs + row * 128 + ((c ^ sm_sw(row)) << 4));
             const int m = m0 + row, n = t * 64 + c * 8;
-            const int off = (m < p.M && n < Cout) ? (m * p.ldy + p.y_coff + n) * 2 : kSmOOB;
+            int off;
+            if constexpr (YS == 2) off = (ysub_row[i] != kSmOOB && n < Cout) ? ysub_row[i] + n * 2 : kSmOOB;
+            else off = (m < p.M && n < Cout) ? (m * p.ldy + p.y_coff + n) * 2 : kSmOOB;
             __builtin_amdgcn_raw_buffer_store_b128(__builtin_bit_cast(kv_i32x4, v), ry, off, 0, 2);
           }
         }
@@ -470,13 +489,16 @@
 struct SmTile {
   int nc3, nzc, d, rd, nw, ks2, areg;
   SmFn fn;
+  SmFn fn_ysub;
 };
 
 template <int NC3, int NZC, int D, int RD, int NW = 8, int KS2 = 1, bool AREG = false,
           bool XP = false>
 constexpr SmTile sm_tile() {
+  SmFn ysub = nullptr;
+  if constexpr (NC3 == 2 && NZC == 4) ysub = &conv_seam_kernel<NC3, NZC, D, RD, NW, KS2, AREG, XP, 2>;
   return SmTile{NC3, NZC, D, RD, NW, KS2, AREG ? 1 : 0,
-                &conv_seam_kernel<NC3, NZC, D, RD, NW, KS2, AREG, XP>};
+                &conv_seam_kernel<NC3, NZC, D, RD, NW, KS2, AREG, XP>, ysub};
 }
 
 static const SmTile kSmTiles[] = {
@@ -526,7 +548,14 @@
       p->ldz % 8 || p->z_coff % 8 || p->x_coff + p->Cin > p->ldx || p->y_coff + p->Cout > p->ldy ||
       p->r_coff + p->Cout > p->ldr || p->z_coff + p->n_t > p->ldz)
     return -8;
-  if ((long long)p->M * p->ldy * 2 >= kSmOOB || (long long)p->M * p->ldr * 2 >= kSmOOB ||
+  if (p->y_sub < 0 || p->y_sub > 2) return -8;
+  if (p->y_sub == 2) {
+    if (!e.fn_ysub || p->Wo < 2 || (long long)p->Ho * p->Wo + 128 >= (1 << 16) ||
+        (long long)p->N * p->Ho * p->Wo != p->M)
+      return -8;
+  }
+  const long long yrows = p->y_sub == 2 ? p->N * kv_conv_y_image_rows(p) : (long long)p->M;
+  if (yrows * p->ldy * 2 >= kSmOOB || (long long)p->M * p->ldr * 2 >= kSmOOB ||
       (long long)p->M * p->ldx * 2 >= kSmOOB || (long long)p->M * p->ldz * 2 >= kSmOOB ||
       (long long)p->Cout * p->Kpad * 2 >= kSmOOB || (long long)p->n_t * p->Cout * 2 >= kSmOOB)
     return -9;
@@ -534,10 +563,11 @@
   if (lds > kSmLdsMax) return -11;
   const int nbm = (p->M + 16 * e.nw - 1) / (16 * e.nw), ntiles = p->Cout / 64;
   if (nbm <= 0 || ntiles <= 0) return 0;
-  if (hipFuncSetAttribute(reinterpret_cast<const void*>(e.fn),
+  const SmFn fn = p->y_sub == 2 ? e.fn_ysub : e.fn;
+  if (hipFuncSetAttribute(reinterpret_cast<const void*>(fn),
                           hipFuncAttributeMaxDynamicSharedMemorySize, lds) != hipSuccess)
     return -7;
-  hipLaunchKernelGGL(e.fn, dim3((unsigned)nbm), dim3(64 * e.nw), (unsigned)lds, stream, *p, ntiles);
+  hipLaunchKernelGGL(fn, dim3((unsigned)nbm), dim3(64 * e.nw), (unsigned)lds, stream, *p, ntiles);
   return hipGetLastError() == hipSuccess ? 0 : -7;
 }
 
diff --git a/csrc/kernels/conv_stream.hip b/csrc/kernels/conv_stream.hip
--- a/csrc/kernels/conv_stream.hip
+++ b/csrc/kernels/conv_stream.hip
@@ -48,9 +48,11 @@
               nt1 * bn);
 }
 
-template <int BM, int BN, int D, int MODE, bool RES, bool BRES, int POL, int NT1 = 0, int MF = 32>
+template <int BM, int BN, int D, int MODE, bool RES, bool BRES, int POL, int NT1 = 0, int MF = 32,
+          int YS = 1>
 __global__ __launch_bounds__(256, (NT1 || (BM * BN >= 128 * 128 && BRES)) ? 1 : 2)
 void conv_stream_kernel(const KvConvParams p) {
+  static_assert(YS == 1 || (YS == 2 && NT1 > 0), "subsampled y store: tail tiles only");
   constexpr int WM = 2, WN = 2;
   constexpr int WTM = BM / WM, WTN = BN / WN;
   constexpr int TM = WTM / MF, TN = WTN / MF;
@@ -93,7 +95,12 @@
   const __amdgpu_buffer_rsrc_t rx2 =
       mk_rsrc(MODE == 4 ? p.x2 : p.x, MODE == 4 ? p.N * p.H2 * p.W2 * p.ldx2 * 2 : 0);
   const __amdgpu_buffer_rsrc_t rr = mk_rsrc(RES ? p.res : p.x, RES ? p.M * p.ldr * 2 : 0);
-  const __amdgpu_buffer_rsrc_t ry = mk_rsrc(p.y, p.M * p.ldy * 2);
+  const int Hc = (p.Ho + 1) >> 1, Wc = (p.Wo + 1) >> 1;
+  const __amdgpu_buffer_rsrc_t ry =
+      mk_rsrc(p.y, YS == 2 ? p.N * Hc * Wc * p.ldy * 2 : p.M * p.ldy * 2);
+  const int dHW = YS == 2 ? p.Ho * p.Wo : 2, dWo = YS == 2 ? p.Wo : 2;
+  const FastDiv fHW{0xffffffffu / (unsigned)dHW + 1u, dHW};
+  const FastDiv fWo{0xffffffffu / (unsigned)dWo + 1u, dWo};
 
   const int lrow = lane >> 3, pch = lane & 7;
   int b_off[B_INS];
@@ -297,6 +304,20 @@
   auto epilogue = [&](int ti, const ResRegs& rres, auto A1, auto A2) __attribute__((always_inline)) {
     constexpr int act1 = decltype(A1)::value, act2 = decltype(A2)::value;
     const int m0 = (mfirst + ti * mstep) * BM;
+    int ysub_off[YS == 2 ? PER : 1];
+    if constexpr (YS == 2) {
+      const int img0 = (int)((unsigned)m0 / (unsigned)HoWo), rem0 = m0 - img0 * HoWo;
+#pragma unroll
+      for (int j = 0; j < PER; ++j) {
+        const int idx = tid + 256 * j;
+        const int ml = idx / CPR, n = n0 + (idx % CPR) * 8;
+        const int r = rem0 + ml, io = fdiv(r, fHW), rr = fmod_(r, io, fHW);
+        const int ho = fdiv(rr, fWo), wo = fmod_(rr, ho, fWo);
+        const bool keep = m0 + ml < p.M && n < p.Cout && ((ho | wo) & 1) == 0;
+        const int row = ((img0 + io) * Hc + (ho >> 1)) * Wc + (wo >> 1);
+        ysub_off[j] = keep ? (row * p.ldy + p.y_coff + n) * 2 : kOOB;
+      }
+    }
 #pragma unroll
     for (int tn = 0; tn < TN; ++tn) {
 #pragma unroll
@@ -329,7 +350,9 @@
 #pragma unroll
         for (int e = 0; e < 8; ++e) v[e] = f2bf(act_c<act2>((float)v[e] + (float)rv[e]));
       }
-      const int off = (m < p.M && n < p.Cout) ? (m * p.ldy + p.y_coff + n) * 2 : kOOB;
+      int off;
+      if constexpr (YS == 2) off = ysub_off[j];
+      else off = (m < p.M && n < p.Cout) ? (m * p.ldy + p.y_coff + n) * 2 : kOOB;
       __builtin_amdgcn_raw_buffer_store_b128(__builtin_bit_cast(u32x4, v), ry, off, 0, YP);
       if constexpr (NT1 > 0) *reinterpret_cast<bf16x8*>(Cs + ml * CS + ch * 8) = v;
     }
@@ -395,16 +418,22 @@
 typedef void (*StreamFn)(const KvConvParams);
 
 template <int BM, int BN, int D, bool BRES, int POL = 0, int MF = 32>
-StreamFn stream_get(int mode, bool res, int nt) {
-  if (nt) return nullptr;
+StreamFn stream_get(int mode, bool res, int nt, int ysub) {
+  if (nt || ysub == 2) return nullptr;
   if (mode == 4) return conv_stream_kernel<BM, BN, D, 4, false, BRES, POL, 0, MF>;
   return res ? conv_stream_kernel<BM, BN, D, 1, true, BRES, POL, 0, MF>
              : conv_stream_kernel<BM, BN, D, 1, false, BRES, POL, 0, MF>;
 }
 
 template <int BM, int BN, int D, int MF = 32>
-StreamFn stream_get_tail(int mode, bool res, int nt) {
-  if (nt == 0) return stream_get<BM, BN, D, true, 0, MF>(mode, res, 0);
+StreamFn stream_get_tail(int mode, bool res, int nt, int ysub) {
+  if (nt == 0) return stream_get<BM, BN, D, true, 0, MF>(mode, res, 0, ysub);
+  if (ysub == 2) {
+    if constexpr (D == 2)
+      if (nt == 128 && mode == 1 && res)
+        return conv_stream_kernel<BM, BN, D, 1, true, true, 0, 128, MF, 2>;
+    return nullptr;
+  }
   if constexpr (D == 3) if (nt == 64) {
     if (mode == 4) return conv_stream_kernel<BM, BN, D, 4, false, true, 0, 64, MF>;
     return res ? conv_stream_kernel<BM, BN, D, 1, true, true, 0, 64, MF> : nullptr;
@@ -419,7 +448,7 @@
 struct StreamTile {
   int bm, bn, d;
   bool bres;
-  StreamFn (*get)(int, bool, int);
+  StreamFn (*get)(int, bool, int, int);
 };
 
 static const StreamTile kStreamTiles[] = {
@@ -464,7 +493,14 @@
   if (tile < 0 || tile >= stream_num_tiles()) return -6;
   if (p->mode != 1 && p->mode != 4) return -8;
   if (p->mode == 4 && (p->res || p->up2 || p->x2_coff)) return -8;
-  if ((long long)p->M * p->ldy * 2 >= kOOB || (p->res && (long long)p->M * p->ldr * 2 >= kOOB))
+  if (p->y_sub < 0 || p->y_sub > 2) return -8;
+  if (p->y_sub == 2) {
+    if (!p->n_t || p->mode != 1 || !p->res || p->Wo < 2 || (long long)p->Ho * p->Wo + 128 >= (1 << 16) ||
+        (long long)p->N * p->Ho * p->Wo != p->M)
+      return -8;
+  }
+  const long long yrows = p->y_sub == 2 ? p->N * kv_conv_y_image_rows(p) : (long long)p->M;
+  if (yrows * p->ldy * 2 >= kOOB || (p->res && (long long)p->M * p->ldr * 2 >= kOOB))
     return -9;
   const long long xb = (long long)p->N * p->H * p->W * p->ldx * 2;
   const long long wb = (long long)p->Cout * p->Kpad * 2;
@@ -495,7 +531,7 @@
   int mgroups = (256 * per_cu + nbn - 1) / nbn;
   if (mgroups > nbm) mgroups = nbm;
   if (mgroups < 1) mgroups = 1;
-  StreamFn fn = e.get(p->mode, res, p->n_t);
+  StreamFn fn = e.get(p->mode, res, p->n_t, p->y_sub);
   if (!fn) return -8;
   if (hipFuncSetAttribute(reinterpret_cast<const void*>(fn),
                           hipFuncAttributeMaxDynamicSharedMemorySize, lds) != hipSuccess)
diff --git a/csrc/kernels/kvedge_kernels.h b/csrc/kernels/kvedge_kernels.h
--- a/csrc/kernels/kvedge_kernels.h
+++ b/csrc/kernels/kvedge_kernels.h
@@ -34,7 +34,13 @@
   long long ws_elems;
   int x2_coff;
   int up2;
+  int y_sub;
 } KvConvParams;
+
+static inline long long kv_conv_y_image_rows(const KvConvParams* p) {
+  return p->y_sub == 2 ? (long long)((p->Ho + 1) / 2) * ((p->Wo + 1) / 2)
+                       : (long long)p->Ho * p->Wo;
+}
 
 int kv_conv2d(const KvConvParams* p, int tile, hipStream_t stream);
 long long kv_set_conv_chunk_bytes(long long bytes);
diff --git a/kvedge_amd/models/layers.py b/kvedge_amd/models/layers.py
--- a/kvedge_amd/models/layers.py
+++ b/kvedge_amd/models/layers.py
@@ -128,14 +128,14 @@
                                 (b3 + bd).contiguous().to(device), w3.shape[1],
                                 down_conv.stride[0], act)
 
-    def __call__(self, y, x, out=None, tile=None):
-        out = ops.conv_dual(y, x, self.w, self.b, self.act, self.stride2, out=out,
+    def __call__(self, y, x, out=None, tile=None, stride2=None):
+        s2 = self.stride2 if stride2 is None else stride2
+        out = ops.conv_dual(y, x, self.w, self.b, self.act, s2, out=out,
                             tile=self.tile if tile is None else tile)
         if _RECORDER is not None:
-            key = ("dual", tuple(y.shape), tuple(x.shape), tuple(self.w.shape), self.stride2,
-                   self.act)
+            key = ("dual", tuple(y.shape), tuple(x.shape), tuple(self.w.shape), s2, self.act)
             fn = lambda t, o=out: ops.conv_dual(y, x, self.w, self.b, self.act,
-                                                self.stride2, out=o, tile=t)
+                                                s2, out=o, tile=t)
             _RECORDER.append((self, key, fn))
         return out
 
diff --git a/kvedge_amd/models/resnet.py b/kvedge_amd/models/resnet.py
--- a/kvedge_amd/models/resnet.py
+++ b/kvedge_amd/models/resnet.py
@@ -14,6 +14,7 @@
 
 ACT_NONE, ACT_RELU = ops.ACT_NONE, ops.ACT_RELU
 TAIL1_MIN_ROWS = int(os.environ.get("KVEDGE_TAIL1_MIN_ROWS", "32768"))
+TAIL1_YSUB = os.environ.get("KVEDGE_TAIL1_YSUB", "0") == "1"
 
 
 class Bottleneck(nn.Module):
@@ -106,11 +107,12 @@
                 self.dual = DeployedDualConv.from_modules(b.conv3, b.bn3, b.downsample[0],
                                                           b.downsample[1], ACT_RELU, device)
 
-    def __call__(self, x, out=None, t1=None):
+    def __call__(self, x, out=None, t1=None, x_sub=False):
+        assert not x_sub or (t1 is not None and self.dual is not None and self.dual.stride2 == 2)
         y = self.c1(x) if t1 is None else t1
         y = self.c2(y)
         if self.dual is not None:
-            return self.dual(y, x, out=out)
+            return self.dual(y, x, out=out, stride2=1 if x_sub else None)
         idt = x if self.down is None else self.down(x)
         return self.c3(y, res=idt, out=out)
 
@@ -128,23 +130,26 @@
         return (c1.cout in (64, 128) and (self.dual is not None or self.down is None) and
                 (self.dual is None or c1.cout == 64) and k <= 128)
 
-    def tail_fits(self, x: torch.Tensor, batch: int = 0) -> bool:
-        N, Ho, Wo, _ = self.out_shape(x.shape)
+    def tail_fits(self, x: torch.Tensor, batch: int = 0, t1=None) -> bool:
+        N, Ho, Wo, _ = self.out_shape(x.shape if t1 is None else t1.shape)
         N = batch or N
         if self.c3.spec.cout == 256:
             return N * Ho * Wo >= TAIL1_MIN_ROWS
         return (N * Ho * Wo + 127) // 128 >= ops.SEAM_MIN_WGS
 
-    def call_tail(self, x, nxt: "DeployedBottleneck", t1=None, out=None, z=None):
+    def call_tail(self, x, nxt: "DeployedBottleneck", t1=None, out=None, z=None, y_sub=1,
+                  x_sub=False):
+        assert not x_sub or (t1 is not None and self.dual is not None and self.dual.stride2 == 2)
         y = self.c1(x) if t1 is None else t1
         y = self.c2(y)
         c1 = nxt.c1
         if self.dual is not None:
             d = self.dual
-            return ops.conv_tail(y, d.w, d.b, d.act, c1.w, c1.b, x2=x, stride2=d.stride2,
-                                 out=out, z=z)
+            return ops.conv_tail(y, d.w, d.b, d.act, c1.w, c1.b, x2=x,
+                                 stride2=1 if x_sub else d.stride2,
+                                 out=out, z=z, y_sub=y_sub)
         return ops.conv_tail(y, self.c3.w, self.c3.b, self.c3.spec.act, c1.w, c1.b, res=x,
-                             out=out, z=z)
+                             out=out, z=z, y_sub=y_sub)
 
     def out_shape(self, x_shape):
         N, H, W, _ = x_shape
@@ -201,6 +206,7 @@
     fuse_stem_pool: bool = True
     fuse_preprocess: bool = True
     fuse_tail: bool = True
+    fuse_tail_cpu: bool = False
     stem12: bool = True
 
     def stem_and_pool(self, x: torch.Tensor, frames_in: bool = False) -> torch.Tensor:
@@ -244,13 +250,17 @@
         else:
             x = self.stem_and_pool(x, frames_in)
             rest = self.blocks
+        x_sub = False
         for i, b in enumerate(rest):
             nxt = rest[i + 1] if i + 1 < len(rest) else None
-            if (self.fuse_tail and x.is_cuda and nxt is not None and b.can_tail(nxt) and
-                    b.tail_fits(x)):
-                x, t1 = b.call_tail(x, nxt, t1=t1)
+            if (self.fuse_tail and (x.is_cuda or self.fuse_tail_cpu) and nxt is not None and
+                    b.can_tail(nxt) and b.tail_fits(x, t1=t1)):
+                sub = (ops.TAIL_YSUB and nxt.dual is not None and nxt.dual.stride2 == 2 and
+                       (b.c3.spec.cout != 256 or TAIL1_YSUB))
+                x, t1 = b.call_tail(x, nxt, t1=t1, y_sub=2 if sub else 1, x_sub=x_sub)
+                x_sub = sub
             else:
-                x, t1 = b(x, t1=t1), None
+                x, t1, x_sub = b(x, t1=t1, x_sub=x_sub), None, False
         return x
 
     def logits(self, x: torch.Tensor, frames_in: bool = False) -> torch.Tensor:
diff --git a/kvedge_amd/ops/__init__.py b/kvedge_amd/ops/__init__.py
--- a/kvedge_amd/ops/__init__.py
+++ b/kvedge_amd/ops/__init__.py
@@ -254,29 +254,40 @@
               w1: torch.Tensor, b1: Optional[torch.Tensor], res: Optional[torch.Tensor] = None,
               x2: Optional[torch.Tensor] = None, stride2: int = 1,
               out: Optional[torch.Tensor] = None, z: Optional[torch.Tensor] = None,
-              tile: int = -1):
+              tile: int = -1, y_sub: int = 1):
     N, H, W, _ = x.shape
     cout, nt = w.shape[0], w1.shape[0]
-    if out is None:
-        out = empty(N, H, W, cout, dtype=torch.bfloat16, device=x.device)
+    assert y_sub in (1, 2)
+    yshape = (N, (H + 1) // 2, (W + 1) // 2, cout) if y_sub == 2 else (N, H, W, cout)
+    if out is None and (x.is_cuda or y_sub == 1):
+        out = empty(*yshape, dtype=torch.bfloat16, device=x.device)
+    assert out is None or tuple(out.shape) == yshape, (tuple(out.shape), yshape)
     if z is None:
         z = empty(N, H, W, nt, dtype=torch.bfloat16, device=x.device)
     if x.is_cuda:
-        _native().conv_tail(x, x2, w, bias, res, out, w1, b1, z, stride2, act, tile)
+        _native().conv_tail(x, x2, w, bias, res, out, w1, b1, z, stride2, act, tile, y_sub)
         return out, z
+    full = out if y_sub == 1 else torch.empty(N, H, W, cout, dtype=torch.bfloat16)
     if x2 is not None:
-        _ref.conv_dual(x, x2, w, bias, act, stride2, out)
+        _ref.conv_dual(x, x2, w, bias, act, stride2, full)
     else:
         spec = ConvSpec.auto(x.shape[3], cout, 1, 1, 0, act)
-        _ref.conv2d(x, spec, w, bias, res, out, 0, 0, 0)
+        _ref.conv2d(x, spec, w, bias, res, full, 0, 0, 0)
     spec1 = ConvSpec.auto(cout, nt, 1, 1, 0, ACT_RELU)
-    _ref.conv2d(out, spec1, w1, b1, None, z, 0, 0, 0)
+    _ref.conv2d(full, spec1, w1, b1, None, z, 0, 0, 0)
+    if y_sub == 2:
+        sub = full[:, ::2, ::2]
+        if out is None:
+            out = sub.contiguous()
+        else:
+            out.copy_(sub)
     return out, z
 
 
 SEAM_SHAPES = {(128, 512, 128), (128, 512, 256), (256, 1024, 256)}
 SEAM_ENABLED = os.environ.get("KVEDGE_SEAM", "1") != "0"
 SEAM_MIN_WGS = int(os.environ.get("KVEDGE_SEAM_MIN_WGS", "256"))
+TAIL_YSUB = os.environ.get("KVEDGE_TAIL_YSUB", "1") != "0"
 
 
 C2F_ENABLED = os.environ.get("KVEDGE_C2F", "1") != "0"
```

Result: no change. 91070 images/sec (median of 3 runs) (+0.3%).
